# bgmanuel99/Super-Resolution-Images-for-3D-Printing-Defect-Detection

Hardware: AMD Instinct MI355X
Metric: 4x-SR MPix/s on 512x512 LR batch (higher is better)
Workload: dtype bf16

## Files before the change

### include/sr355.h

```cpp
#ifndef SR355_H
#define SR355_H
#include <stdint.h>

#ifdef __cplusplus
extern "C" {
#endif

typedef struct sr_ctx sr_ctx;
typedef struct sr_model sr_model;

typedef enum sr_status {
    SR_OK = 0,
    SR_ERR_INVALID = -1,
    SR_ERR_HIP = -2,
    SR_ERR_OOM = -3,
    SR_ERR_STATE = -4,
    SR_ERR_NAME = -5,
    SR_ERR_CAPACITY = -6
} sr_status;

enum { SR_DTYPE_F32 = 0, SR_DTYPE_BF16 = 1, SR_DTYPE_U8 = 2 };
enum { SR_MODEL_SRCNN = 0, SR_MODEL_EDSR = 1, SR_MODEL_ESRGAN_G = 2, SR_MODEL_VGG16 = 3,
       SR_MODEL_ESRGAN_D = 4,
       SR_MODEL_VGG19_FEATURES = 5 };
enum { SR_ACT_LINEAR = 0, SR_ACT_RELU = 1, SR_ACT_LRELU = 2, SR_ACT_TANH = 3 };
enum { SR_WEIGHT_KERNEL = 0, SR_WEIGHT_BIAS = 1 };
enum { SR_ELT_AXPBY = 0, SR_ELT_RELU_BWD = 1, SR_ELT_LRELU_BWD = 2, SR_ELT_CLIP01_BWD = 3, SR_ELT_MUL = 4, SR_ELT_TANH_BWD = 5, SR_ELT_CLIP01 = 6,
       SR_ELT_SIGN_DIFF = 7 };

typedef struct sr_model_cfg {
    int32_t compute_dtype;
    int32_t scale_factor;
    int32_t channels;
    int32_t num_blocks;
    int32_t num_filters;
    int32_t growth_channels;
    float   res_scaling;
    int32_t num_classes;
    int32_t use_attention;
} sr_model_cfg;

int  sr_init(int device_id, sr_ctx** out);
void sr_destroy(sr_ctx* ctx);
const char* sr_last_error(sr_ctx* ctx);
int  sr_mem_info(sr_ctx* ctx, int64_t* current_bytes, int64_t* peak_bytes);
int  sr_last_forward_ms(sr_ctx* ctx, float* ms);

int  sr_measure_clock(sr_ctx* ctx, float* mhz, void* stream);

int  sr_debug_set_stamp_buffer(sr_ctx* ctx, void* device_u64_buffer, int64_t capacity_bytes);
int  sr_debug_set_chain_stamp_buffer(sr_ctx* ctx, void* device_u64_buffer, int64_t capacity_bytes);
int64_t sr_debug_stamp_bytes_needed(int which, int64_t workgroups);
int  sr_debug_set_fused(sr_ctx* ctx, int mask, int max_workgroups);
enum { SR_FUSE_DENSE_TAIL = 1, SR_FUSE_DENSE_MID = 2, SR_FUSE_RGB_TAIL = 4, SR_FUSE_ATTN_PROJ = 8, SR_FUSE_CELLS = 16, SR_FUSE_CONV1_STREAM = 32,
       SR_FUSE_POOL = 64, SR_FUSE_CONV_STREAM = 128, SR_FUSE_SRCNN_1X1 = 256, SR_FUSE_ALL = 511,
       SR_FUSE_TWO_UP = SR_FUSE_DENSE_TAIL | SR_FUSE_DENSE_MID | SR_FUSE_CONV1_STREAM };
int  sr_debug_set_alloc_cap(sr_ctx* ctx, int64_t bytes);
int  sr_debug_conv_routes(sr_ctx* ctx, int enable, char* text, int64_t cap);
int  sr_profile_begin(sr_ctx* ctx);
int  sr_profile_end(sr_ctx* ctx, char* json, int64_t cap);

int  sr_model_create(sr_ctx* ctx, int kind, const sr_model_cfg* cfg, sr_model** out);
void sr_model_destroy(sr_model* m);
int  sr_model_num_params(sr_model* m);
int  sr_model_param_info(sr_model* m, int index, const char** name, int* which, int64_t shape[4], int* ndim);
int  sr_model_set_weight(sr_model* m, const char* keras_layer_name, int which,
                         const float* host, const int64_t* shape, int ndim);
int  sr_model_finalize(sr_model* m);
int  sr_model_release_workspace(sr_model* m);
int  sr_model_num_ops(sr_model* m);
int  sr_model_op_info(sr_model* m, int index, const char** name, int* channels, int* mul, int* shift, int* ceil_halvings);
int  sr_model_set_tap(sr_model* m, int op_index, float* device_dst, int64_t capacity);
int  sr_model_output_shape(sr_model* m, int B, int H, int W, int C, int64_t out_shape[4]);
int  sr_forward(sr_model* m, const void* x, int io_dtype, int B, int H, int W, int C,
                void* y, int64_t y_capacity, void* stream);

int  sr_conv2d(sr_ctx* ctx, const void* x, int dtype, int B, int H, int W, int Cin,
               const float* w_hwio, const float* bias, int KH, int KW, int Cout, int act,
               float alpha, const void* skip1, float beta1, const void* skip2, float beta2,
               int clip01, int d2s_r, void* y, void* stream);
int  sr_self_attention(sr_ctx* ctx, const void* x, int dtype, int B, int H, int W, int C,
                       const float* wf, const float* bf, const float* wg, const float* bg,
                       const float* wh, const float* bh, const float* wv, const float* bv,
                       void* y, void* stream);
int  sr_bicubic(sr_ctx* ctx, const void* x, int dtype, int B, int H, int W, int C,
                int outH, int outW, void* y, void* stream);
int  sr_resize(sr_ctx* ctx, const void* x, int dtype, int B, int H, int W, int C,
               int outH, int outW, int interpolation, void* y, void* stream);
int  sr_psnr(sr_ctx* ctx, const void* a, const void* b, int B, int H, int W, int C, float max_val,
             float* out_B, void* stream);
int  sr_ssim(sr_ctx* ctx, const void* a, const void* b, int B, int H, int W, int C, float max_val,
             float* out_B, void* stream);
int  sr_mse(sr_ctx* ctx, const void* a, const void* b, int64_t n, float* out1, void* stream);
int  sr_l1(sr_ctx* ctx, const void* a, const void* b, int64_t n, float* out1, void* stream);
int  sr_spectral_l1(sr_ctx* ctx, const void* a, const void* b, int B, int H, int W, int C, float* out1, void* stream);
int  sr_conv2d_wgrad(sr_ctx* ctx, const void* x, const void* dy, int B, int H, int W, int Cin, int Cout, int K,
                     float* dw_hwio, float* db, void* stream);
int  sr_conv2d_dev(sr_ctx* ctx, const void* x, int B, int H, int W, int Cin, const float* d_w, const float* d_bias, int K, int Cout,
                   int rot, int act, float alpha, const void* skip1, float beta1, const void* skip2, float beta2, int clip01,
                   int d2s_r, void* y, void* stream);
typedef struct { const void* p; int64_t cs; int32_t coff; } sr_view;
int  sr_conv2d_dev_views(sr_ctx* ctx, const sr_view* x, int B, int H, int W, int Cin, const float* d_w, const float* d_bias, int K, int Cout, int rot,
                         int act, float alpha, const sr_view* skip1, float beta1, const sr_view* y, void* stream);
int  sr_conv2d_wgrad_views(sr_ctx* ctx, const sr_view* x, const sr_view* dy, int B, int H, int W, int Cin, int Cout, int K,
                           float* dw_hwio, float* db, void* stream);
int  sr_eltwise_views(sr_ctx* ctx, int op, const sr_view* a, const sr_view* b, float alpha, float beta, const sr_view* out, int64_t npix, int C, void* stream);
typedef struct { const float* w; const float* bias; int32_t K, Cin, Cout, rot; } sr_pack_desc;
int  sr_conv_prepack(sr_ctx* ctx, const sr_pack_desc* uses, int n, void* stream);
int  sr_eltwise(sr_ctx* ctx, int op, const void* a, const void* b, float alpha, float beta, void* out, int64_t n, void* stream);
int  sr_adam(sr_ctx* ctx, void* w, const void* g, void* m, void* v, int64_t n, float lr_t, float beta1, float one_minus_beta1, float beta2,
             float one_minus_beta2, float epsilon, float grad_scale, void* stream);
int  sr_space_to_depth(sr_ctx* ctx, const void* x, int B, int H, int W, int C, int r, void* y, void* stream);
enum { SR_SP_MAXPOOL2 = 0, SR_SP_GAP = 1, SR_SP_PICK2 = 2, SR_SP_VGG_PREPROCESS = 3 };
int  sr_spatial_op(sr_ctx* ctx, int op, const void* x, int B, int H, int W, int C, void* y, void* stream);
int  sr_matmul(sr_ctx* ctx, const void* A, const void* B, void* C, int batch, int M, int N, int K, int transA, int transB, float alpha, void* stream);
int  sr_softmax_rows(sr_ctx* ctx, void* s, int64_t rows, int cols, void* stream);
int  sr_softmax_bwd(sr_ctx* ctx, const void* p, const void* dp, void* ds, int64_t rows, int cols, void* stream);
int  sr_maxpool2_bwd(sr_ctx* ctx, const void* x, const void* dy, int B, int H, int W, int C, void* dx, void* stream);
int  sr_zero_insert2(sr_ctx* ctx, const void* dy, int B, int H, int W, int C, void* out, void* stream);
int  sr_spectral_l1_bwd(sr_ctx* ctx, const void* a, const void* b, int B, int H, int W, int C, float scale, void* da, void* stream);
int  sr_extract_patches(sr_ctx* ctx, const float* img, int H, int W, int C, int patch, int stride,
                        float mul, float add, int out_dtype, void* out, int64_t out_capacity,
                        int* n_patches, void* stream);
int  sr_overlap_add(sr_ctx* ctx, const void* patches, int in_dtype, int H, int W, int C, int patch,
                    int stride, int scale, float mul, float add, float* out, void* stream);

int  sr_extract_patches_batch(sr_ctx* ctx, const void* imgs, int in_dtype, int F, int H, int W, int C, int patch, int stride,
                              float mul, float add, int out_dtype, void* out, int64_t out_capacity, int* patches_per_image, void* stream);
int  sr_patch_vote(sr_ctx* ctx, const float* probs, int F, int P, int K, int32_t* cls_F, float* conf_F, int32_t* votes_FxK, void* stream);
int  sr_classification_counts(sr_ctx* ctx, const int32_t* y_true_N, const int32_t* preds_AxN, const float* conf_AxN, int A, int N, int K,
                              int64_t* confusion_AxKxK, double* conf_sums_Ax2, void* stream);

int  sr_back_projection(sr_ctx* ctx, const uint8_t* hr_u8, const uint8_t* lr_u8, int B, int H, int W, int h, int w, int iterations,
                        uint8_t* y_u8, float* y_f32, void* stream);
int  sr_noise_sigma(sr_ctx* ctx, const uint8_t* x_u8, int B, int h, int w, double* sigma_f64, void* stream);
int  sr_nl_means(sr_ctx* ctx, const uint8_t* x_u8, int B, int h, int w, int patch, int distance, const double* sigma_f64,
                 double h_scale, float* y_f32, void* stream);
int  sr_edge_guided(sr_ctx* ctx, const uint8_t* x_u8, int B, int h, int w, int H, int W, float weight, uint8_t* y_u8,
                    float* up_e_f32, void* stream);
// ... 93 lines not shown
```

### super-resolution-images-for-3d-printing-defect-detection_amd/csrc/api.hip

```cpp
#include <math.h>
#include <stdio.h>
#include <stdlib.h>
#include <string.h>

#include <memory>

#include "common.h"

void* sr_ctx::dalloc(size_t bytes) {
    void* p = nullptr;
    if (bytes == 0) bytes = 16;
    if (alloc_cap > 0 && cur_bytes + (int64_t)bytes > alloc_cap) {
        err = "allocation of " + std::to_string(bytes) + " bytes exceeds the debug cap (sr_debug_set_alloc_cap)";
        return nullptr;
    }
    hipError_t e = hipMalloc(&p, bytes);
    if (e != hipSuccess) {
        err = std::string("hipMalloc(") + std::to_string(bytes) + "): " + hipGetErrorString(e);
        return nullptr;
    }
    allocs[p] = bytes;
    cur_bytes += (int64_t)bytes;
    if (cur_bytes > peak_bytes) peak_bytes = cur_bytes;
    return p;
// ... 469 lines not shown
            const std::string why = m->ctx->err;
            (void)hipDeviceSynchronize();
            m->free_bufs();
            return m->ctx->fail(SR_ERR_OOM, "workspace for [" + std::to_string(B) + "," + std::to_string(H) + "," + std::to_string(W) + "]: " + why +
                                                " (all workspaces of this model were released)");
        }
        SR_HIP(m->ctx, hipMemsetAsync(m->bufp[i], 0, bytes, st));
        m->bufcap[i] = bytes;
    }
    return SR_OK;
}

enum Route { RT_CHAIN = OP_PREPROC + 1, RT_CHAIN_SECOND, RT_CONV1_STREAM, RT_RGB_TAIL, RT_PW2, RT_IN_EPILOGUE };

bool tapped(const sr_model* m, size_t oi) { return !m->taps.empty() && m->taps.count((int)oi) != 0; }
bool bare_epilogue(const Op& op) { return op.skip1.buf < 0 && op.skip2.buf < 0 && op.d2s == 1 && !op.clip; }

bool chain_fits(const sr_model* m, size_t oi, int w, bool pack2) {
    const Op& op = m->ops[oi];
    if (op.chain < 0 || op.chain_pos != 0) return false;
    const ChainSpec& ch = m->chains[op.chain];
    return !(ch.tail && tapped(m, oi)) && (m->ctx->chain_mask & (ch.tail ? SR_FUSE_DENSE_TAIL : SR_FUSE_DENSE_MID)) && chain_supported(ch.w, m->view(op.in), pack2 ? 48 : w);
}
bool conv1_stream_fits(const sr_model* m, const Op& op, int w, bool pack2) {
    return (m->ctx->chain_mask & SR_FUSE_CONV1_STREAM) && op.chain < 0 && op.act == SR_ACT_RELU && op.alpha == 1.f && bare_epilogue(op) && op.out.buf == op.in.buf &&
           op.in.coff == 0 && op.out.coff == 64 && conv1_stream_supported(m->convs[op.conv].w, m->view(op.in), pack2 ? 48 : w);
}
bool rgb_tail_fits(const sr_model* m, const Op& op, size_t oi, int B, int h, int w) {
    const ConvWeights& cw = m->convs[op.conv].w;
    return op.rgbtail >= 0 && (m->ctx->chain_mask & SR_FUSE_RGB_TAIL) && !tapped(m, oi) && cw.rows && cw.NT == 4 && cw.Cout == 64 && bare_epilogue(op) &&
           op.act != SR_ACT_TANH && op.out.buf >= 0 && (int64_t)m->bufcap[op.out.buf] >= rgbtail_partial_bytes(B, h, w);
}
bool pw2_fits(const sr_model* m, const Op& op, size_t oi) {
    const ConvWeights& cw = m->convs[op.conv].w;
    return op.pw2 >= 0 && (m->ctx->chain_mask & SR_FUSE_SRCNN_1X1) && !tapped(m, oi) && cw.thin && !cw.few && cw.dtype == SR_DTYPE_F32 && bare_epilogue(op);
}
bool pool_fits(const sr_model* m, const Op& op, size_t oi, int h, int w) {
    if (oi + 1 >= m->ops.size() || op.out.buf < 0) return false;
    const Op& pl = m->ops[oi + 1];
    const ConvWeights& cw = m->convs[op.conv].w;
    return (m->ctx->chain_mask & SR_FUSE_POOL) && m->T == SR_DTYPE_BF16 && pl.kind == OP_POOL && pl.in.buf == op.out.buf && pl.out.buf >= 0 && cw.rows && cw.NT == 4 &&
           cw.CoutP == cw.Cout && bare_epilogue(op) && op.act != SR_ACT_TANH && !tapped(m, oi) && !m->grid_now[op.in.buf].gx && !m->grid_now[op.out.buf].gx &&
           h >= 2 && w >= 2 && m->bufs[pl.out.buf].Cbuf % 8 == 0 && m->bufs[pl.out.buf].Cbuf >= cw.Cout;
}
bool proj_fits(const sr_model* m, const Op& op) {
    const ConvWeights& cw = m->convs[op.conv].w;
    return op.proj >= 0 && (m->ctx->chain_mask & SR_FUSE_ATTN_PROJ) && cw.rows && cw.NT == 4 && cw.Cout / (op.d2s * op.d2s) == 64 && cw.CoutP == cw.Cout &&
           op.out.buf >= 0 && !m->bufs[op.out.buf].blk && op.skip2.buf < 0 && !op.clip && op.act != SR_ACT_TANH && m->bufs[op.out.buf].Cbuf % 4 == 0;
}

void plan_routes(sr_model* m, const Layout& L, int B, int H, int W) {
    std::vector<int>& rt = m->routes;
    rt.resize(m->ops.size());
    for (size_t oi = 0; oi < m->ops.size(); ++oi) rt[oi] = m->ops[oi].kind;
    for (size_t oi = 0; oi < m->ops.size(); ++oi) {
        const Op& op = m->ops[oi];
        if (rt[oi] != OP_CONV) continue;
        int h, w;
        buf_hw(m->bufs[op.in.buf], H, W, &h, &w);
        if (chain_fits(m, oi, w, L.pack2)) { rt[oi] = RT_CHAIN; rt[oi + 1] = RT_CHAIN_SECOND; }
        else if (conv1_stream_fits(m, op, w, L.pack2)) rt[oi] = RT_CONV1_STREAM;
        else if (rgb_tail_fits(m, op, oi, B, h, w)) { rt[oi] = RT_RGB_TAIL; rt[oi + 1] = RT_IN_EPILOGUE; }
        else if (pw2_fits(m, op, oi)) { rt[oi] = RT_PW2; rt[oi + 1] = RT_IN_EPILOGUE; }
        else if (pool_fits(m, op, oi, h, w) || proj_fits(m, op)) rt[oi + 1] = RT_IN_EPILOGUE;
    }
}

}

extern "C" {

int sr_init(int device_id, sr_ctx** out) {
    if (!out) return SR_ERR_INVALID;
    *out = nullptr;
    int n = 0;
    if (hipGetDeviceCount(&n) != hipSuccess || device_id < 0 || device_id >= n) return SR_ERR_HIP;
    if (hipSetDevice(device_id) != hipSuccess) return SR_ERR_HIP;
    sr_ctx* c = new sr_ctx();
    c->device = device_id;
    if (hipEventCreate(&c->ev0) != hipSuccess || hipEventCreate(&c->ev1) != hipSuccess) { delete c; return SR_ERR_HIP; }
    c->zero_page = c->dalloc(sr_ctx::ZERO_PAGE_BYTES);
    if (!c->zero_page) { sr_destroy(c); return SR_ERR_OOM; }
    if (hipMemset(c->zero_page, 0, sr_ctx::ZERO_PAGE_BYTES) != hipSuccess) { sr_destroy(c); return SR_ERR_HIP; }
    *out = c;
    return SR_OK;
}

void sr_destroy(sr_ctx* ctx) {
    DeviceGuard dg_(ctx);
    if (!ctx) return;
    (void)hipDeviceSynchronize();
    lpips_release(ctx);
    std::vector<void*> ps;
    for (auto& kv : ctx->allocs) ps.push_back(kv.first);
    for (void* p : ps) ctx->dfree(p);
    if (ctx->ev0) (void)hipEventDestroy(ctx->ev0);
    if (ctx->ev1) (void)hipEventDestroy(ctx->ev1);
    for (auto& r : ctx->prof_recs) { (void)hipEventDestroy(r.e0); (void)hipEventDestroy(r.e1); }
    for (auto& e : ctx->ev_pool) (void)hipEventDestroy(e);
    delete ctx;
}

const char* sr_last_error(sr_ctx* ctx) { return ctx ? ctx->err.c_str() : "null ctx"; }

int sr_mem_info(sr_ctx* ctx, int64_t* current_bytes, int64_t* peak_bytes) {
    if (!ctx) return SR_ERR_INVALID;
    if (current_bytes) *current_bytes = ctx->cur_bytes;
    if (peak_bytes) *peak_bytes = ctx->peak_bytes;
    return SR_OK;
}

int sr_last_forward_ms(sr_ctx* ctx, float* ms) {
    DeviceGuard dg_(ctx);
    if (!ctx || !ms) return SR_ERR_INVALID;
    if (!ctx->timed) return ctx->fail(SR_ERR_STATE, "no forward has run on this ctx");
    SR_HIP(ctx, hipEventSynchronize(ctx->ev1));
    SR_HIP(ctx, hipEventElapsedTime(ms, ctx->ev0, ctx->ev1));
    return SR_OK;
}

int64_t sr_debug_stamp_bytes_needed(int which, int64_t workgroups) {
    if (which == 0) return workgroups < 0 ? -1 : workgroups * 16 * (int64_t)sizeof(unsigned long long);
    if (which == 1) return (int64_t)64 * 4 * 64 * 4 * (int64_t)sizeof(unsigned long long);
    return -1;
}

int sr_debug_set_stamp_buffer(sr_ctx* ctx, void* device_u64_buffer, int64_t capacity_bytes) {
    if (!ctx) return SR_ERR_INVALID;
    if (device_u64_buffer && capacity_bytes < sr_debug_stamp_bytes_needed(0, 1))
        return ctx->fail(SR_ERR_INVALID, "sr_debug_set_stamp_buffer: the buffer does not hold one workgroup's stamps");
    ctx->stamp_buf = static_cast<unsigned long long*>(device_u64_buffer);
    ctx->stamp_cap = device_u64_buffer ? capacity_bytes : 0;
    return SR_OK;
}

int sr_measure_clock(sr_ctx* ctx, float* mhz, void* stream) {
    if (!ctx || !mhz) return SR_ERR_INVALID;
    DeviceGuard dg_(ctx);
    return clock_probe_launch(ctx, mhz, static_cast<hipStream_t>(stream));
}

int sr_debug_set_chain_stamp_buffer(sr_ctx* ctx, void* device_u64_buffer, int64_t capacity_bytes) {
    if (!ctx) return SR_ERR_INVALID;
    if (device_u64_buffer && capacity_bytes < sr_debug_stamp_bytes_needed(1, 0))
        return ctx->fail(SR_ERR_INVALID, "sr_debug_set_chain_stamp_buffer: the buffer is smaller than the stamped kernels write (sr_debug_stamp_bytes_needed(1, 0))");
    ctx->chain_stamp_buf = static_cast<unsigned long long*>(device_u64_buffer);
    const char* skip = getenv("SR355_CHAIN_STAMP_SKIP");
    ctx->chain_stamp_skip = skip ? atoi(skip) : -1;
    return SR_OK;
}

int sr_debug_set_fused(sr_ctx* ctx, int mask, int max_workgroups) {
    if (!ctx) return SR_ERR_INVALID;
    ctx->chain_mask = mask;
    ctx->chain_max_wgs = max_workgroups > 0 ? max_workgroups : 0;
    return SR_OK;
}

int sr_debug_set_alloc_cap(sr_ctx* ctx, int64_t bytes) {
    if (!ctx) return SR_ERR_INVALID;
    ctx->alloc_cap = bytes > 0 ? bytes : 0;
    return SR_OK;
}

int sr_debug_conv_routes(sr_ctx* ctx, int enable, char* text, int64_t cap) {
    if (!ctx) return SR_ERR_INVALID;
    if (text && cap <= (int64_t)ctx->route_text.size()) return ctx->fail(SR_ERR_CAPACITY, "sr_debug_conv_routes: the text buffer is too small");
    if (text) memcpy(text, ctx->route_text.c_str(), ctx->route_text.size() + 1);
    ctx->route_text.clear();
    ctx->route_log = enable != 0;
    return SR_OK;
}

int sr_profile_begin(sr_ctx* ctx) {
    if (!ctx) return SR_ERR_INVALID;
    for (auto& r : ctx->prof_recs) { ctx->ev_pool.push_back(r.e0); ctx->ev_pool.push_back(r.e1); }
    ctx->prof_recs.clear();
    ctx->prof = true;
    return SR_OK;
}

int sr_profile_end(sr_ctx* ctx, char* json, int64_t cap) {
    DeviceGuard dg_(ctx);
    if (!ctx || !json || cap <= 0) return SR_ERR_INVALID;
    ctx->prof = false;
    SR_HIP(ctx, hipDeviceSynchronize());
    struct Agg { int64_t n = 0; double ms = 0, flops = 0, bytes = 0; };
    std::vector<Agg> agg(ctx->prof_names.size());
    for (auto& r : ctx->prof_recs) {
        float ms = 0.f;
        if (hipEventElapsedTime(&ms, r.e0, r.e1) != hipSuccess) continue;
        Agg& a = agg[r.name];
        a.n += 1; a.ms += ms; a.flops += r.flops; a.bytes += r.bytes;
    }
    std::string s = "[";
    bool first = true;
    for (size_t i = 0; i < agg.size(); ++i) {
        if (!agg[i].n) continue;
        char buf[512];
        snprintf(buf, sizeof buf, "%s{\"kernel\": \"%s\", \"launches\": %lld, \"total_ms\": %.6f, \"flops\": %.6e, \"bytes\": %.6e}",
                 first ? "" : ", ", ctx->prof_names[i].c_str(), (long long)agg[i].n, agg[i].ms, agg[i].flops, agg[i].bytes);
        s += buf;
        first = false;
    }
    s += "]";
    for (auto& r : ctx->prof_recs) { ctx->ev_pool.push_back(r.e0); ctx->ev_pool.push_back(r.e1); }
    ctx->prof_recs.clear();
    if ((int64_t)s.size() + 1 > cap) return ctx->fail(SR_ERR_CAPACITY, "profile buffer too small");
    memcpy(json, s.c_str(), s.size() + 1);
    return SR_OK;
}

int sr_model_create(sr_ctx* ctx, int kind, const sr_model_cfg* cfg, sr_model** out) {
    if (!ctx || !cfg || !out) return SR_ERR_INVALID;
    *out = nullptr;
    if (cfg->compute_dtype != SR_DTYPE_F32 && cfg->compute_dtype != SR_DTYPE_BF16)
        return ctx->fail(SR_ERR_INVALID, "compute_dtype must be SR_DTYPE_F32 or SR_DTYPE_BF16");
    std::unique_ptr<sr_model> m(new sr_model());
    m->ctx = ctx; m->kind = kind; m->cfg = *cfg; m->T = cfg->compute_dtype;
    if (m->cfg.channels <= 0) m->cfg.channels = 3;
    if (m->cfg.channels > 16 / dtype_size(m->T))
        return ctx->fail(SR_ERR_INVALID, "channels must fit one 16-byte slice (<= 4 for f32, <= 8 for bf16)");
    int rc;
    switch (kind) {
        case SR_MODEL_SRCNN: rc = build_srcnn(m.get()); break;
        case SR_MODEL_EDSR: rc = build_edsr(m.get()); break;
        case SR_MODEL_ESRGAN_G: rc = build_esrgan(m.get()); break;
        case SR_MODEL_VGG16: rc = build_vgg16(m.get()); break;
        case SR_MODEL_ESRGAN_D: rc = build_discriminator(m.get()); break;
        case SR_MODEL_VGG19_FEATURES: rc = build_vgg19_features(m.get()); break;
        default: return ctx->fail(SR_ERR_INVALID, "unknown model kind");
    }
    if (rc) return rc;
    m->dense_dev.assign(m->params.size(), nullptr);
    *out = m.release();
    return SR_OK;
}

// ... 115 lines not shown
        std::vector<float> k, bias;
        gather(c, k, bias);
        int rc = conv_pack_weights(ctx, k.data(), bias.data(), c.KS, c.Cin, c.Cout, m->T, &c.w, c.rows_head);
        if (rc) return rc;
    }
    for (auto& ch : m->chains) {
        chain_free_weights(ctx, &ch.w);
        const ConvSpec& a = m->convs[ch.conv_a], &bq = m->convs[ch.conv_b];
        std::vector<float> ka, ba, kb, bb;
        gather(a, ka, ba);
        gather(bq, kb, bb);
        int rc = chain_pack_weights(ctx, ka.data(), ba.data(), kb.data(), bb.data(), a.Cin / 32, a.Cout / 16, bq.Cout / 16, &ch.w);
        if (rc) return rc;
    }
    for (auto& rt : m->rgbtails) {
        rgbtail_free_weights(ctx, &rt.w);
        const ConvSpec& c2 = m->convs[rt.conv_b];
        std::vector<float> k, bias;
        gather(c2, k, bias);
        int rc = rgbtail_pack_weights(ctx, k.data(), bias.data(), c2.Cout, &rt.w);
        if (rc) return rc;
    }
    for (auto& pj : m->projs) {
        proj_free_weights(ctx, &pj.w);
        const ConvSpec& c1 = m->convs[pj.conv];
        std::vector<float> k, bias;
        gather(c1, k, bias);
        int rc = proj_pack_weights(ctx, k.data(), bias.data(), c1.Cout, &pj.w);
        if (rc) return rc;
    }
    for (auto& pw : m->pw2s) {
        pw2_free_weights(ctx, &pw.w);
        const ConvSpec& c1 = m->convs[pw.conv];
        std::vector<float> k, bias;
        gather(c1, k, bias);
        int rc = pw2_pack_weights(ctx, k.data(), bias.data(), c1.Cin, c1.Cout, pw.act, &pw.w);
        if (rc) return rc;
    }
    for (auto& op : m->ops) {
        if (op.kind != OP_DENSE) continue;
        for (int pi : {op.dw, op.db}) {
            if (m->dense_dev[pi]) ctx->dfree(m->dense_dev[pi]);
            const Param& p = m->params[pi];
            m->dense_dev[pi] = static_cast<float*>(ctx->dalloc(sizeof(float) * p.count()));
            if (!m->dense_dev[pi]) return SR_ERR_OOM;
            SR_HIP(ctx, hipMemcpy(m->dense_dev[pi], p.host.data(), sizeof(float) * p.count(), hipMemcpyHostToDevice));
        }
    }
    m->finalized = true;
    return SR_OK;
}

int sr_model_output_shape(sr_model* m, int B, int H, int W, int C, int64_t out_shape[4]) {
    if (!m || !out_shape) return SR_ERR_INVALID;
    (void)C;
    if (m->out_vec) { out_shape[0] = B; out_shape[1] = m->out_C; out_shape[2] = 1; out_shape[3] = 1; }
    else { out_shape[0] = B; out_shape[1] = ((int64_t)H * m->out_mul) >> m->out_shift; out_shape[2] = ((int64_t)W * m->out_mul) >> m->out_shift; out_shape[3] = m->out_C; }
    return SR_OK;
}

int sr_forward(sr_model* m, const void* x, int io_dtype, int B, int H, int W, int C, void* y, int64_t y_capacity, void* stream) {
    DeviceGuard dg_(m ? m->ctx : nullptr);
    if (!m) return SR_ERR_INVALID;
    sr_ctx* ctx = m->ctx;
    hipStream_t st = static_cast<hipStream_t>(stream);
    if (!m->finalized) return ctx->fail(SR_ERR_STATE, "sr_model_finalize has not been called");
    if (!x || !y) return ctx->fail(SR_ERR_INVALID, "null tensor");
    if (io_dtype != SR_DTYPE_F32 && io_dtype != SR_DTYPE_BF16) return ctx->fail(SR_ERR_INVALID, "io dtype must be f32 or bf16");
    if (io_dtype == SR_DTYPE_BF16 && m->T == SR_DTYPE_F32) return ctx->fail(SR_ERR_INVALID, "an fp32 model takes fp32 tensors");
    if (C != m->in_C) return ctx->fail(SR_ERR_INVALID, "channel count does not match the model");
    if (B == 0) return SR_OK;
    if (B < 0 || H <= 0 || W <= 0) return ctx->fail(SR_ERR_INVALID, "bad tensor shape");
    int64_t os[4];
    sr_model_output_shape(m, B, H, W, C, os);
    if (y_capacity < os[0] * os[1] * os[2] * os[3]) return ctx->fail(SR_ERR_CAPACITY, "output buffer too small");
    if (m->kind == SR_MODEL_VGG16 && (H < 32 || W < 32)) return ctx->fail(SR_ERR_INVALID, "VGG16 needs H,W >= 32");
    if (m->kind == SR_MODEL_VGG19_FEATURES && (H < 16 || W < 16)) return ctx->fail(SR_ERR_INVALID, "VGG19 features need H,W >= 16");
    const Layout L = choose_layout(m, B, H, W);
    int rc = ensure_workspace(m, L, H, W, st);
    if (rc) return rc;
    plan_routes(m, L, B, H, W);
    SR_HIP(ctx, hipEventRecord(ctx->ev0, st));
    const int T = m->T;
    for (size_t oi = 0; oi < m->ops.size(); ++oi) {
        const Op& op = m->ops[oi];
        const int route = m->routes[oi];
        const Op* nx = oi + 1 < m->ops.size() && m->routes[oi + 1] == RT_IN_EPILOGUE ? &m->ops[oi + 1] : nullptr;
        int h = H, w = W;
        if (op.in.buf >= 0) buf_hw(m->bufs[op.in.buf], H, W, &h, &w);
        const TensorView vi = m->view(op.in), vo = m->view(op.out);
        void* const po = op.out.buf >= 0 ? m->bufp[op.out.buf] : nullptr;
        switch (route) {
            case RT_CHAIN_SECOND: case RT_IN_EPILOGUE:
                break;
            case RT_CHAIN: {
                const ChainSpec& ch = m->chains[op.chain];
                const Op& ob = m->ops[oi + 1];
                TensorView outv{}, so{};
                float bx = 0.f, bo = 0.f;
                if (ch.tail) {
                    outv = m->view(ob.out);
                    for (int k2 = 0; k2 < 2; ++k2) {
                        const Ref& r = k2 ? ob.skip2 : ob.skip1;
                        const float be = k2 ? ob.beta2 : ob.beta1;
                        if (r.buf < 0) continue;
                        if (r.buf == op.in.buf && r.coff == 0) bx = be; else { so = m->view(r); bo = be; }
                    }
                }
                rc = chain_launch(ctx, ch.w, vi, L.pack2 ? (B + 1) / 2 : B, h, L.pack2 ? 48 : w, outv, so, ob.alpha, bx, bo, st, L.pack2);
                break;
            }
            case RT_CONV1_STREAM:
                rc = conv1_stream_launch(ctx, m->convs[op.conv].w, vi, L.pack2 ? (B + 1) / 2 : B, h, L.pack2 ? 48 : w, st, L.pack2);
                break;
            case RT_RGB_TAIL: case RT_PW2: case OP_CONV: {
                const ConvSpec& cs = m->convs[op.conv];
                int in = op.in.buf;
                TensorView xin = vi;
                if (op.pack_alt >= 0 && (L.pack2 || m->grid_now[in].gx)) {
                    void* d = m->bufp[op.pack_alt];
                    const int64_t dC = m->bufs[op.pack_alt].Cbuf;
                    const CellGrid& g = m->grid_now[in];
                    rc = g.gx ? cell_unpack_launch(ctx, vi.p, vi.cs, vi.coff, B, h, w, 64, d, dC, 0, g, st) : unpack_pairs_launch(ctx, vi.p, vi.cs, vi.coff, B, h, w, 64, d, dC, 0, st);
                    if (rc) return rc;
                    in = op.pack_alt;
                    m->grid_now[in] = CellGrid{};
                    xin = m->view({in, 0});
                } else if (L.pack2 && vi.blk) {
                    return ctx->fail(SR_ERR_STATE, "two-up packed dense blocks: a conv outside the fused kernels would read a packed buffer");
                }
                const CellGrid g = m->grid_now[in];
                bool same = g.gx == 0 || op.d2s == 1;
                for (const Ref& r : {op.out, op.skip1, op.skip2})
                    if (r.buf != -1 && !((r.buf >= 0 ? m->grid_now[r.buf] : CellGrid{}) == g)) same = false;
                if (!same) return ctx->fail(SR_ERR_STATE, "packed small-image layout: producer and consumer disagree");
                const int cB = g.gx ? 1 : B;
                if (g.gx) { h = g.Hv; w = g.Wv; }
                ConvEpilogue ep;
                ep.act = op.act; ep.alpha = op.alpha; ep.clip01 = op.clip; ep.d2s_r = op.d2s; ep.cell_h = g.ch; ep.cell_w = g.cw;
                if (op.skip1.buf >= 0) { ep.skip1 = m->view(op.skip1); ep.beta1 = op.beta1; }
                if (op.skip2.buf >= 0) { ep.skip2 = m->view(op.skip2); ep.beta2 = op.beta2; }
                if (route == RT_RGB_TAIL) {
                    const RgbTailWeights& rt = m->rgbtails[op.rgbtail].w;
                    ep.f2 = &rt; ep.f2_part = static_cast<float*>(po);
                    rc = conv_launch(ctx, cs.w, xin, cB, h, w, TensorView{}, ep, st);
                    if (!rc) rc = rgbtail_finish_launch(ctx, rt, ep.f2_part, cB, h, w, nx->act, nx->alpha, nx->clip, y, m->out_C, 0, io_dtype == SR_DTYPE_F32, st);
                    break;
                }
                if (route == RT_PW2) ep.pw2 = &m->pw2s[op.pw2].w;
                else if (nx && nx->kind == OP_POOL) { ep.pool_out = m->view(nx->out); ep.pool_grid = m->grid_now[nx->out.buf]; }
                else if (nx) { ep.pj = &m->projs[op.proj].w; ep.pj_out = m->view(nx->out); }
                if (op.out.buf == -2) {
                    ep.out_f32 = io_dtype == SR_DTYPE_F32;
                    rc = conv_launch(ctx, cs.w, xin, B, h, w, y, m->out_C, 0, ep, st);
                } else {
                    rc = conv_launch(ctx, cs.w, xin, cB, h, w, route == RT_PW2 ? m->view(nx->out) : vo, ep, st);
                }
                break;
            }
            case OP_CONVERT:
                rc = convert_pad_launch(ctx, x, io_dtype, (int64_t)B * H * W, C, po, T, vo.cs, 1.f, 0.f, st);
                break;
            case OP_PREPROC:
                rc = vgg_preproc_launch(ctx, x, io_dtype, (int64_t)B * H * W, po, T, vo.cs, st);
                break;
            case OP_ATTN:
                rc = attention_launch(ctx, T, vi.p, vi.cs,  8,  0,  16, B, h * w, po, vo.cs, 0, st);
                break;
            case OP_SUBSAMPLE:
                rc = subsample2_launch(ctx, T, vi.p, B, h, w, m->bufs[op.in.buf].C, vi.cs, po, vo.cs, st);
                break;
            case OP_TOBLK: {
                const CellGrid& g = m->grid_now[op.out.buf];
                rc = g.gx ? cell_pack_launch(ctx, vi.p, vi.cs, vi.coff, B, h, w, 64, po, vo.cs, vo.coff, g, st)
                   : L.pack2 ? pack_pairs_launch(ctx, vi.p, vi.cs, vi.coff, B, h, w, 64, po, vo.cs, vo.coff, st)
                             : nhwc_to_blocked_launch(ctx, vi.p, vi.cs, vi.coff, B, h, w, 64, po, vo.cs, vo.coff, st);
                break;
            }
            case OP_POOL:
                rc = maxpool2_launch(ctx, T, vi.p, B, h, w, m->bufs[op.in.buf].C, vi.cs, po, vo.cs, st, m->grid_now[op.in.buf], m->grid_now[op.out.buf]);
                break;
            case OP_GAP:
                rc = gap_launch(ctx, T, vi.p, B, h * w, m->bufs[op.in.buf].C, vi.cs, static_cast<float*>(po), st);
                break;
            case OP_DENSE: {
                const bool f32 = op.out.buf != -2 || io_dtype == SR_DTYPE_F32;
                float* yf = static_cast<float*>(op.out.buf == -2 ? y : po);
                rc = dense_launch(ctx, static_cast<const float*>(vi.p), m->dense_dev[op.dw], m->dense_dev[op.db], B, op.In, op.Out, op.act, f32 ? yf : nullptr,
                                  f32 ? 0 : io_dtype, f32 ? nullptr : y, st);
                break;
            }
        }
        if (rc) return rc;
        if (tapped(m, oi)) {
            int C_, mu, sh, th, tw;
            op_out_view(m, op, &C_, &mu, &sh);
            buf_hw(m->bufs[op.out.buf], H, W, &th, &tw);
            const sr_model::Tap& tp = m->taps.at((int)oi);
            if (tp.cap < (int64_t)B * th * tw * C_) return ctx->fail(SR_ERR_CAPACITY, "tap buffer too small");
            rc = tap_copy_launch(ctx, vo.p, T, vo.blk, vo.cs, vo.coff, B, th, tw, C_, tp.dst, st, L.pack2 && vo.blk);
            if (rc) return rc;
        }
    }
    SR_HIP(ctx, hipEventRecord(ctx->ev1, st));
    ctx->timed = true;
    return SR_OK;
}

static ConvEpilogue single_op_epilogue(int act, float alpha, int clip01, int d2s_r, TensorView skip1, float beta1, TensorView skip2, float beta2) {
    ConvEpilogue ep;
    ep.act = act; ep.alpha = alpha; ep.clip01 = clip01; ep.d2s_r = d2s_r < 1 ? 1 : d2s_r;
    ep.allow_splitk = 1;
    if (skip1.p) { ep.skip1 = skip1; ep.beta1 = beta1; }
    if (skip2.p) { ep.skip2 = skip2; ep.beta2 = beta2; }
    return ep;
}

static int padded_cin(const ConvWeights& cw) { return cw.thin ? cw.CinP : round_up(cw.CinP, 32); }

int sr_conv2d(sr_ctx* ctx, const void* x, int dtype, int B, int H, int W, int Cin, const float* w_hwio, const float* bias, int KH, int KW,
              int Cout, int act, float alpha, const void* skip1, float beta1, const void* skip2, float beta2, int clip01, int d2s_r,
              void* y, void* stream) {
    DeviceGuard dg_(ctx);
    if (!ctx) return SR_ERR_INVALID;
    hipStream_t st = static_cast<hipStream_t>(stream);
    if (!x || !w_hwio || !y) return ctx->fail(SR_ERR_INVALID, "null tensor");
    if (KH != KW) return ctx->fail(SR_ERR_INVALID, "square kernels only");
    if (dtype != SR_DTYPE_F32 && dtype != SR_DTYPE_BF16) return ctx->fail(SR_ERR_INVALID, "dtype must be f32 or bf16");
    if (B <= 0 || H <= 0 || W <= 0 || Cin <= 0 || Cout <= 0) return ctx->fail(SR_ERR_INVALID, "bad tensor shape");
    ConvWeights cw;
    int rc = conv_pack_weights(ctx, w_hwio, bias, KH, Cin, Cout, dtype, &cw);
    if (rc) return rc;
    const int esz = dtype_size(dtype);
    const int Cp = padded_cin(cw);
    void* xp = ctx->dalloc((size_t)B * H * W * Cp * esz + 4096);
    if (!xp) { conv_free_weights(ctx, &cw); return SR_ERR_OOM; }
    rc = convert_pad_launch(ctx, x, dtype, (int64_t)B * H * W, Cin, xp, dtype, Cp, 1.f, 0.f, st);
    if (!rc) {
        auto skip_view = [&](const void* s) { return (s == x && Cout == Cin) ? TensorView{xp, Cp, 0} : TensorView{s, Cout, 0}; };
        const ConvEpilogue ep = single_op_epilogue(act, alpha, clip01, d2s_r, skip_view(skip1), beta1, skip_view(skip2), beta2);
        const int r = ep.d2s_r;
        rc = conv_launch(ctx, cw, TensorView{xp, Cp, 0}, B, H, W, y, Cout / (r * r), 0, ep, st);
    }
    hipError_t e = hipStreamSynchronize(st);
    ctx->dfree(xp);
    conv_free_weights(ctx, &cw);
    if (!rc && e != hipSuccess) return ctx->fail(SR_ERR_HIP, std::string("conv2d: ") + hipGetErrorString(e));
    return rc;
}

// ... 278 lines not shown
```

### super-resolution-images-for-3d-printing-defect-detection_amd/csrc/attention.hip

```cpp
#include "common.h"

#include <cstdlib>

namespace {

constexpr int KV_TILE = 64;

template <typename T> struct AT;
template <> struct AT<float>  { static constexpr int PITCH = KV_TILE * 4 + 4; };

struct AttnParams {
    const char* qkv; int64_t cs; int qoff, koff, voff;
    char* o; int64_t o_cs; int o_coff;
    int N;
    const float* knorm;
};

__device__ __forceinline__ float xhalf(float v) { return __shfl_xor(v, 32); }

__global__ void __launch_bounds__(256, 2) attn_f32_kernel(AttnParams p) {
    constexpr int PITCH = AT<float>::PITCH;
    __shared__ __attribute__((aligned(16))) char vt[32 * PITCH];

    const int tid = threadIdx.x, lane = tid & 63, wave = tid >> 6, r = lane & 31, h = lane >> 5;
    const int b = blockIdx.y;
    const int N = p.N;
    const float* base = reinterpret_cast<const float*>(p.qkv) + (int64_t)b * N * p.cs;
    const int q = blockIdx.x * 128 + wave * 32 + r;
    const int qc = q < N ? q : N - 1;

    float qf[4];
    {
        const float* qp = base + (int64_t)qc * p.cs + p.qoff;
#pragma unroll
        for (int j = 0; j < 4; ++j) qf[j] = qp[2 * j + h];
    }

    f32x16 oacc;
#pragma unroll
    for (int e = 0; e < 16; ++e) oacc[e] = 0.f;
    float m_run = -INFINITY, l_run = 0.f;

    const int skey = tid >> 2, soct = tid & 3;

    for (int k0 = 0; k0 < N; k0 += KV_TILE) {
        __syncthreads();
        {
            const int key = k0 + skey;
            const float* vp = base + (int64_t)(key < N ? key : N - 1) * p.cs + p.voff + soct * 8;
            f32x4 v0 = *reinterpret_cast<const f32x4*>(vp), v1 = *reinterpret_cast<const f32x4*>(vp + 4);
#pragma unroll
            for (int e = 0; e < 4; ++e) {
                *reinterpret_cast<float*>(vt + (soct * 8 + e) * PITCH + skey * 4) = v0[e];
                *reinterpret_cast<float*>(vt + (soct * 8 + 4 + e) * PITCH + skey * 4) = v1[e];
            }
        }
        __syncthreads();
#pragma unroll
        for (int sub = 0; sub < KV_TILE / 32; ++sub) {
            const int kb = k0 + sub * 32;
            if (kb >= N) break;
            f32x16 s;
#pragma unroll
            for (int e = 0; e < 16; ++e) s[e] = 0.f;
            {
                const int key = kb + r;
                const float* kp = base + (int64_t)(key < N ? key : N - 1) * p.cs + p.koff;
#pragma unroll
                for (int j = 0; j < 4; ++j) s = __builtin_amdgcn_mfma_f32_32x32x2f32(kp[2 * j + h], qf[j], s, 0, 0, 0);
            }
            float mx = -INFINITY;
#pragma unroll
            for (int i = 0; i < 16; ++i) {
                const int key = kb + (i & 3) + 8 * (i >> 2) + 4 * h;
                if (key >= N) s[i] = -INFINITY;
                mx = fmaxf(mx, s[i]);
            }
            mx = fmaxf(mx, xhalf(mx));
            const float m_new = fmaxf(m_run, mx);
            const float alpha = __expf(m_run - m_new);
            float psum = 0.f;
#pragma unroll
            for (int i = 0; i < 16; ++i) { s[i] = __expf(s[i] - m_new); psum += s[i]; }
            l_run = l_run * alpha + psum;
            m_run = m_new;
#pragma unroll
            for (int e = 0; e < 16; ++e) oacc[e] *= alpha;
#pragma unroll
            for (int i = 0; i < 16; ++i) {
                const int krow = sub * 32 + (i & 3) + 8 * (i >> 2);
                const float va = *reinterpret_cast<const float*>(vt + r * PITCH + (krow + 4 * h) * 4);
                oacc = __builtin_amdgcn_mfma_f32_32x32x2f32(va, s[i], oacc, 0, 0, 0);
            }
        }
    }
    const float l_tot = l_run + xhalf(l_run);
    const float inv = 1.f / l_tot;
    if (q < N) {
        float* op = reinterpret_cast<float*>(p.o) + ((int64_t)b * N + q) * p.o_cs + p.o_coff;
#pragma unroll
        for (int g = 0; g < 4; ++g) {
            const int d0 = 8 * g + 4 * h;
            f32x4 t = {oacc[4 * g] * inv, oacc[4 * g + 1] * inv, oacc[4 * g + 2] * inv, oacc[4 * g + 3] * inv};
            *reinterpret_cast<f32x4*>(op + d0) = t;
        }
    }
}

constexpr int KT2 = 128;
constexpr int PITCH2 = KT2 * 2 + 8;

__global__ void __launch_bounds__(64) attn_knorm_kernel(const bf16_t* qkv, int64_t cs, int koff, int N, int ngroups, float* out) {
    const int g = blockIdx.x % ngroups, b = blockIdx.x / ngroups, lane = threadIdx.x;
    const bf16_t* base = qkv + (int64_t)b * N * cs + koff;
    float m = 0.f;
#pragma unroll
    for (int t = 0; t < 2; ++t) {
        const int key = g * 128 + t * 64 + lane;
        if (key < N) {
            const bf16x8 k = *reinterpret_cast<const bf16x8*>(base + (int64_t)key * cs);
            float n2 = 0.f;
#pragma unroll
            for (int e = 0; e < 8; ++e) n2 += (float)k[e] * (float)k[e];
            m = fmaxf(m, n2);
        }
    }
#pragma unroll
    for (int o = 32; o > 0; o >>= 1) m = fmaxf(m, __shfl_xor(m, o));
    if (lane == 0) out[(int64_t)b * ngroups + g] = sqrtf(m);
}

template <int QB>
__global__ void __launch_bounds__(256, 3) attn_bf16_kernel(AttnParams p) {
    __shared__ __attribute__((aligned(16))) char vt[32 * PITCH2];
    const int tid = threadIdx.x, lane = tid & 63, wave = tid >> 6, r = lane & 31, h = lane >> 5;
    const int N = p.N;
    constexpr int QW = 64 * QB * 2;
    const int nqt = (N + QW - 1) / QW;
    const int b = blockIdx.x / nqt, qt = blockIdx.x - b * nqt;
    const bf16_t* base = reinterpret_cast<const bf16_t*>(p.qkv) + (int64_t)b * N * p.cs;
    const int cs = (int)p.cs;
    int qi[QB];
    bf16x8 qb[QB];
#pragma unroll
    for (int j = 0; j < QB; ++j) {
        qi[j] = qt * QW + wave * (32 * QB) + j * 32 + r;
        const int qc = qi[j] < N ? qi[j] : N - 1;
        bf16x8 z = {};
        qb[j] = z;
        if (h == 0) qb[j] = *reinterpret_cast<const bf16x8*>(base + (int64_t)qc * cs + p.qoff);
    }
    float qn2 = 0.f;
#pragma unroll
    for (int j = 0; j < QB; ++j) {
        float n2 = 0.f;
#pragma unroll
        for (int e = 0; e < 8; ++e) n2 += (float)qb[j][e] * (float)qb[j][e];
        qn2 = fmaxf(qn2, n2);
    }
#pragma unroll
    for (int o = 32; o > 0; o >>= 1) qn2 = fmaxf(qn2, __shfl_xor(qn2, o));
    const float qmaxv = sqrtf(qn2) * 1.0009765625f;
    const int* knorm_bits = reinterpret_cast<const int*>(p.knorm) + (int64_t)b * ((N + KT2 - 1) / KT2);
    f32x16 oacc[QB];
    bf16x8 sel = {};
    {
        const int m = lane & 15, kg = lane >> 4;
        const bf16_t one = (bf16_t)1.f;
        if ((m == 0 && (kg & 1) == 0) || (m == 1 && (kg & 1) == 1)) sel = bf16x8{one, one, one, one, one, one, one, one};
    }
    f32x4 lacc[QB];
    float m_run[QB];
#pragma unroll
    for (int j = 0; j < QB; ++j) {
        m_run[j] = 0.f; lacc[j] = f32x4{0.f, 0.f, 0.f, 0.f};
#pragma unroll
        for (int e = 0; e < 16; ++e) oacc[j][e] = 0.f;
    }

    const int kp = tid >> 2, oct = tid & 3;
    bf16x8 kneg = {};
    kneg[0] = (bf16_t)-1.f; kneg[1] = (bf16_t)-1.f; kneg[2] = (bf16_t)-1.f;
    auto load_k = [&](int kb) {
        int l;
        asm volatile("v_mbcnt_lo_u32_b32 %0, -1, 0\n\tv_mbcnt_hi_u32_b32 %0, -1, %0" : "=v"(l));
        bf16x8 kf = kneg;
        const int key = kb + (l & 31);
        if (l < 32) kf = *reinterpret_cast<const bf16x8*>(base + (int64_t)(key < N ? key : N - 1) * cs + p.koff);
        return kf;
    };
    bf16x8 knext = load_k(0);
    f32x16 zero16;
#pragma unroll
    for (int e = 0; e < 16; ++e) zero16[e] = 0.f;
    struct { } false_c; struct { int x; } true_c{0};
    auto hmax = [](float v) {
        const unsigned u = __builtin_bit_cast(unsigned, v);
        const auto sw = __builtin_amdgcn_permlane32_swap(u, u, false, false);
        return fmaxf(__builtin_bit_cast(float, (unsigned)sw[0]), __builtin_bit_cast(float, (unsigned)sw[1]));
    };
    auto tile = [&](const bf16x8 kf, const int sub, const int kb, auto ragged_tag, const bool first) {
        constexpr bool RAGGED = sizeof(ragged_tag) > 1;
        f32x16 s[QB];
        float mx[QB];
#pragma unroll
        for (int j = 0; j < QB; ++j) {
            s[j] = __builtin_amdgcn_mfma_f32_32x32x16_bf16(kf, qb[j], zero16, 0, 0, 0);
            if constexpr (RAGGED) {
#pragma unroll
                for (int i = 0; i < 16; ++i)
                    if (kb + (i & 3) + 8 * (i >> 2) + 4 * h >= N) s[j][i] = -INFINITY;
            }
// ... 85 lines not shown
                lacc[j] = __builtin_amdgcn_mfma_f32_16x16x32_bf16(sel, pf, lacc[j], 0, 0, 0);
            }
        }
        return true;
    };
    auto thresh_of_wave = [&]() -> int {
        float m = m_run[0];
#pragma unroll
        for (int j = 1; j < QB; ++j) m = fminf(m, m_run[j]);
#pragma unroll
        for (int o = 32; o > 0; o >>= 1) m = fminf(m, __shfl_xor(m, o));
        const float lim = GROW_OK + m;
        const float th = !(lim >= 0.f) ? -1.f : (qmaxv > 0.f ? lim / qmaxv * 0.9990234375f : INFINITY);
        return __builtin_amdgcn_readfirstlane(__builtin_bit_cast(int, th));
    };
    int thresh_bits = __builtin_amdgcn_readfirstlane(__builtin_bit_cast(int, -1.f));
    auto stage_v = [&](const int k0) {
        __syncthreads();
#pragma unroll
        for (int part = 0; part < KT2 / 128; ++part) {
            const int ka = k0 + part * 128 + 2 * kp, kbb = ka + 1;
            if (ka - 2 * kp >= N) break;
            const bf16x8 va = *reinterpret_cast<const bf16x8*>(base + (int64_t)(ka < N ? ka : N - 1) * cs + p.voff + oct * 8);
            const bf16x8 vb = *reinterpret_cast<const bf16x8*>(base + (int64_t)(kbb < N ? kbb : N - 1) * cs + p.voff + oct * 8);
#pragma unroll
            for (int e = 0; e < 8; ++e) {
                typedef bf16_t bf16x2 __attribute__((ext_vector_type(2)));
                bf16x2 pr = {va[e], vb[e]};
                *reinterpret_cast<bf16x2*>(vt + (oct * 8 + e) * PITCH2 + (part * 64 + kp) * 4) = pr;
            }
        }
        __syncthreads();
    };
    auto slow_tiles = [&](const int k0, const int sub0, bf16x8 kf) {
        for (int sub = sub0; sub < KT2 / 32; ++sub) {
            const int kb = k0 + sub * 32;
            if (kb >= N) break;
            if (sub != sub0) { kf = knext; knext = load_k(kb + 32); }
            if (kb + 32 <= N) tile(kf, sub, kb, false_c, kb == 0);
            else tile(kf, sub, kb, true_c, kb == 0);
        }
    };

    for (int k0 = 0; k0 < N; k0 += KT2) {
        stage_v(k0);
        int sub = 0;
        bf16x8 kf = knext;
        const bool full = k0 != 0 && k0 + KT2 <= N;
        if (full) {
            const bool guard = !(knorm_bits[k0 / KT2] <= thresh_bits);
#pragma unroll
            for (; sub < KT2 / 32; ++sub) {
                kf = knext;
                knext = load_k(k0 + sub * 32 + 32);
                if (!tile_fast(kf, sub, guard)) break;
            }
        } else {
            knext = load_k(k0 + 32);
        }
        if (sub < KT2 / 32) {
            slow_tiles(k0, sub, kf);
            thresh_bits = thresh_of_wave();
        }
    }
#pragma unroll
    for (int j = 0; j < QB; ++j) {
        const float l0 = __shfl(lacc[j][0], r & 15), l1 = __shfl(lacc[j][1], r & 15);
        const float inv = 1.f / ((r >> 4) ? l1 : l0);
        if (qi[j] < N) {
            bf16_t* op = reinterpret_cast<bf16_t*>(p.o) + ((int64_t)b * N + qi[j]) * p.o_cs + p.o_coff;
#pragma unroll
            for (int g = 0; g < 4; ++g) {
                bf16x4 t = {(bf16_t)(oacc[j][4 * g] * inv), (bf16_t)(oacc[j][4 * g + 1] * inv), (bf16_t)(oacc[j][4 * g + 2] * inv),
                            (bf16_t)(oacc[j][4 * g + 3] * inv)};
                *reinterpret_cast<bf16x4*>(op + 8 * g + 4 * h) = t;
            }
        }
    }
}

}

int attention_launch(sr_ctx* ctx, int dtype, const void* qkv, int64_t cs, int qoff, int koff, int voff, int B, int N,
                     void* o, int64_t o_cs, int o_coff, hipStream_t st) {
    if (B <= 0 || N <= 0) return ctx->fail(SR_ERR_INVALID, "attention: empty tensor");
    const int esz = dtype_size(dtype);
    if ((cs * esz) % 16 || (qoff * esz) % 16 || (koff * esz) % 16 || (voff * esz) % 16 || (o_cs * esz) % 16 || (o_coff * esz) % 16)
        return ctx->fail(SR_ERR_INVALID, "attention: views must be 16-byte aligned");
    AttnParams p{static_cast<const char*>(qkv), cs, qoff, koff, voff, static_cast<char*>(o), o_cs, o_coff, N, nullptr};
    dim3 grid((unsigned)((N + 127) / 128), (unsigned)B);
    if (dtype != SR_DTYPE_BF16 && dtype != SR_DTYPE_F32) return ctx->fail(SR_ERR_INVALID, "attention: dtype must be f32 or bf16");
    const int rec = ctx->prof_open(dtype == SR_DTYPE_BF16 ? "attn<bf16>" : "attn<f32>", 2.0 * B * (double)N * N * 40.0,
                                   (double)B * N * 80.0 * esz, st);
    if (dtype == SR_DTYPE_BF16) {
        constexpr int QBr = 2;
        const int64_t nwg = (int64_t)B * ((N + 128 * QBr - 1) / (128 * QBr));
        const int ngroups = (N + KT2 - 1) / KT2;
        if (nwg >= (1ll << 31) || (int64_t)B * ngroups >= (1ll << 31)) { ctx->prof_close(rec, st); return ctx->fail(SR_ERR_INVALID, "attention: too many workgroups for one launch"); }
        float* kn = static_cast<float*>(ctx->arena(ctx->attn_kn, sizeof(float) * (size_t)B * ngroups, st));
        if (!kn) { ctx->prof_close(rec, st); return SR_ERR_OOM; }
        p.knorm = kn;
        hipLaunchKernelGGL(attn_knorm_kernel, dim3((unsigned)((int64_t)B * ngroups)), dim3(64), 0, st, reinterpret_cast<const bf16_t*>(qkv) + 0, cs, koff, N, ngroups, kn);
        hipLaunchKernelGGL(attn_bf16_kernel<QBr>, dim3((unsigned)nwg), dim3(256), 0, st, p);
    }
    else hipLaunchKernelGGL(attn_f32_kernel, grid, dim3(256), 0, st, p);
    ctx->prof_close(rec, st);
    SR_HIP(ctx, hipGetLastError());
    return SR_OK;
}
```

### super-resolution-images-for-3d-printing-defect-detection_amd/csrc/common.h

```cpp
#pragma once
#include <hip/hip_runtime.h>
#include <stdint.h>
#include <string.h>
#include <string>
#include <unordered_map>
#include <unordered_set>
#include <vector>

#include "../../include/sr355.h"

typedef __bf16 bf16_t;
typedef __bf16 bf16x8 __attribute__((ext_vector_type(8)));
typedef __bf16 bf16x4 __attribute__((ext_vector_type(4)));
typedef float f32x4 __attribute__((ext_vector_type(4)));
typedef float f32x16 __attribute__((ext_vector_type(16)));

struct sr_ctx {
    int device = 0;
    std::string err;
    int64_t cur_bytes = 0, peak_bytes = 0;
    std::unordered_map<void*, size_t> allocs;
    hipEvent_t ev0 = nullptr, ev1 = nullptr;
    bool timed = false;

    void* scratch_buf = nullptr;
    size_t scratch_cap = 0;
    unsigned long long* stamp_buf = nullptr;
    int64_t stamp_cap = 0;
    int chain_stamp_skip = -1;
    unsigned long long* chain_stamp_buf = nullptr;

    struct ProfRec { int name; hipEvent_t e0, e1; double flops, bytes; };
    bool prof = false;
    std::vector<std::string> prof_names;
    std::vector<ProfRec> prof_recs;
    std::vector<hipEvent_t> ev_pool;
    int prof_open(const std::string& name, double flops, double bytes, hipStream_t st);
    void prof_close(int rec, hipStream_t st);

    static constexpr int MAX_LDS_BYTES = 160 * 1024;
    std::unordered_map<const void*, int> lds_attr_done;
    int ensure_dyn_lds(const void* kernel, int bytes);
    void* tab_buf = nullptr; size_t tab_cap = 0;
    struct Arena { void* p = nullptr; size_t cap = 0; };
    Arena attn_kn;
    Arena dev_w, dev_b, dev_x;
    Arena cls_tab, cls_work, cls_fft;
    std::unordered_map<int64_t, double*> dft_ops;
    Arena met_work, met_fft;
    Arena eda_work, eda_dct;
    Arena deg_work;
    Arena crop_work;
    Arena sn_work, sn_tab, dhead_work;
    std::vector<char> sn_tab_host;
    void* sn_tab_dev = nullptr;
    struct LpipsState* lpips = nullptr;
    Arena lpips_work;
    int* deg_status = nullptr;
    void* arena(Arena& a, size_t bytes, hipStream_t st);
    struct PackKey {
        const void* w; const void* b; int K, Cin, Cout, rot;
        bool operator==(const PackKey& o) const { return w == o.w && b == o.b && K == o.K && Cin == o.Cin && Cout == o.Cout && rot == o.rot; }
    };
    struct PackKeyHash {
        size_t operator()(const PackKey& k) const {
            return std::hash<const void*>()(k.w) ^ (std::hash<const void*>()(k.b) * 31u) ^ ((size_t)k.rot << 1) ^ ((size_t)k.Cin << 20) ^ ((size_t)k.Cout << 36) ^ ((size_t)k.K << 52);
        }
    };
    std::unordered_map<PackKey, std::pair<void*, float*>, PackKeyHash> pack_cache;
    Arena pack_w, pack_b, pack_tab;
    std::vector<char> pack_tab_host;
    void* pack_tab_dev = nullptr;
    static constexpr int ZERO_PAGE_BYTES = 32768;
    void* zero_page = nullptr;
    int num_cus = 0;
    int cu_count();
    int chain_mask = 511;
    int chain_max_wgs = 0;
    int64_t alloc_cap = 0;
    bool route_log = false;
    std::string route_text;

    void* dalloc(size_t bytes);
    void dfree(void* p);
    void* scratch(size_t bytes);
    int fail(int code, const std::string& msg) { err = msg; return code; }
};
static_assert(511 == SR_FUSE_ALL && SR_FUSE_ALL == (SR_FUSE_DENSE_TAIL | SR_FUSE_DENSE_MID | SR_FUSE_RGB_TAIL | SR_FUSE_ATTN_PROJ | SR_FUSE_CELLS | SR_FUSE_CONV1_STREAM |
                                             SR_FUSE_POOL | SR_FUSE_CONV_STREAM | SR_FUSE_SRCNN_1X1), "sr_ctx::chain_mask's default is every SR_FUSE_* bit");

struct DeviceGuard {
    int prev = -1; bool switched = false;
    explicit DeviceGuard(const sr_ctx* c) {
        if (c && hipGetDevice(&prev) == hipSuccess && prev != c->device) switched = hipSetDevice(c->device) == hipSuccess;
    }
    ~DeviceGuard() { if (switched) (void)hipSetDevice(prev); }
    DeviceGuard(const DeviceGuard&) = delete;
    DeviceGuard& operator=(const DeviceGuard&) = delete;
};

#define SR_HIP(ctx, call)                                                                        \
    do {                                                                                         \
        hipError_t e_ = (call);                                                                  \
        if (e_ != hipSuccess)                                                                    \
            return (ctx)->fail(SR_ERR_HIP, std::string(#call) + ": " + hipGetErrorString(e_));   \
    } while (0)

void lpips_release(sr_ctx* ctx);

__device__ inline int gray_bgr(int b, int g, int r) { return (1868 * b + 9617 * g + 4899 * r + 8192) >> 14; }

static inline int dtype_size(int dt) { return dt == SR_DTYPE_F32 ? 4 : (dt == SR_DTYPE_BF16 ? 2 : 1); }
static inline int round_up(int a, int b) { return (a + b - 1) / b * b; }
static inline uint16_t f32_to_bf16_host(float f) {
    uint32_t u;
    memcpy(&u, &f, 4);
    if ((u & 0x7fffffffu) > 0x7f800000u) return (uint16_t)((u >> 16) | 0x40);
    u += 0x7fffu + ((u >> 16) & 1u);
    return (uint16_t)(u >> 16);
}

int weights_upload(sr_ctx* ctx, const void* packed, size_t bytes, const float* bias, int n, int npad, void** d_w, float** d_bias);
template <typename P> static inline void weights_free(sr_ctx* ctx, P*& w, float*& bias) {
    if (w) ctx->dfree(w);
    if (bias) ctx->dfree(bias);
    w = nullptr; bias = nullptr;
}

struct ConvWeights {
    void* w = nullptr;
    float* bias = nullptr;
    int dtype = SR_DTYPE_BF16;
    int KS = 3, Cin = 0, Cout = 0;
    int CinP = 0, CoutP = 0;
    int thin = 0;
    int KGPT = 2;
    int NT = 1;
    int rows = 0;
    int few = 0;
    int pw = 0;
    int nchunks = 1;
    size_t bytes = 0;
};

struct TensorView {
    const void* p = nullptr;
    int64_t cs = 0;
    int coff = 0;
    int blk = 0;
};

struct RgbTailWeights {
    void* a = nullptr;
    float* bias = nullptr;
    int c2 = 0;
};

struct ProjWeights {
    void* a = nullptr;
    float* bias = nullptr;
    int nblk = 0;
};

struct Pw2Weights {
    float* a = nullptr;
    float* bias = nullptr;
    int cin = 0, cout = 0, act = 0;
};

struct CellGrid {
    int gx = 0, ch = 0, cw = 0, Hv = 0, Wv = 0;
    bool operator==(const CellGrid& o) const { return gx == o.gx && ch == o.ch && cw == o.cw && Hv == o.Hv && Wv == o.Wv; }
};

struct ConvEpilogue {
    TensorView pool_out;
    CellGrid pool_grid;
    int cell_h = 0, cell_w = 0;
    const ProjWeights* pj = nullptr;
    TensorView pj_out;
    const Pw2Weights* pw2 = nullptr;
    const RgbTailWeights* f2 = nullptr;
    float* f2_part = nullptr;
    int act = SR_ACT_LINEAR;
    float alpha = 1.f;
    TensorView skip1, skip2;
    float beta1 = 0.f, beta2 = 0.f;
    int clip01 = 0;
    int d2s_r = 1;
    int out_f32 = 0;
    int allow_splitk = 0;
};

int conv_pack_weights_dev(sr_ctx* ctx, const float* d_hwio, const float* d_bias, int KS, int Cin, int Cout, int rot, ConvWeights* out, hipStream_t st);
int conv_prepack_dev(sr_ctx* ctx, const sr_pack_desc* descs, int n, hipStream_t st);
int conv_pack_weights(sr_ctx* ctx, const float* hwio, const float* bias, int KS, int Cin, int Cout,
                      int dtype, ConvWeights* out, int rows_head = 0);
static inline void conv_free_weights(sr_ctx* ctx, ConvWeights* w) { weights_free(ctx, w->w, w->bias); }
int conv_launch(sr_ctx* ctx, const ConvWeights& w, TensorView x, int B, int H, int W,
                void* y, int64_t y_cs, int y_coff, const ConvEpilogue& ep, hipStream_t st);
int conv_launch(sr_ctx* ctx, const ConvWeights& w, TensorView x, int B, int H, int W, TensorView y, const ConvEpilogue& ep, hipStream_t st);

int proj_pack_weights(sr_ctx* ctx, const float* w_hwio, const float* bias, int cout, ProjWeights* out);
int pw2_pack_weights(sr_ctx* ctx, const float* w_hwio, const float* bias, int cin, int cout, int act, Pw2Weights* out);
static inline void pw2_free_weights(sr_ctx* ctx, Pw2Weights* w) { weights_free(ctx, w->a, w->bias); *w = Pw2Weights{}; }
static inline void proj_free_weights(sr_ctx* ctx, ProjWeights* w) { weights_free(ctx, w->a, w->bias); }
int rgbtail_pack_weights(sr_ctx* ctx, const float* w2_hwio, const float* bias2, int c2, RgbTailWeights* out);
static inline void rgbtail_free_weights(sr_ctx* ctx, RgbTailWeights* w) { weights_free(ctx, w->a, w->bias); }
int64_t rgbtail_partial_bytes(int B, int H, int W);
int rgbtail_finish_launch(sr_ctx* ctx, const RgbTailWeights& w, const float* part, int B, int H, int W, int act, float alpha, int clip01, void* y,
                          int64_t y_cs, int y_coff, int out_f32, hipStream_t st);

struct ChainWeights {
    void* w = nullptr; float* bias = nullptr;
    int ext = 0, nb0 = 0, nb1 = 0;
    size_t bytes = 0;
};
int chain_pack_weights(sr_ctx* ctx, const float* wa_hwio, const float* ba, const float* wb_hwio, const float* bb, int ext, int nb0, int nb1, ChainWeights* out);
static inline void chain_free_weights(sr_ctx* ctx, ChainWeights* w) { weights_free(ctx, w->w, w->bias); }
bool chain_supported(const ChainWeights& w, const TensorView& in, int W);
bool conv1_stream_supported(const ConvWeights& w, const TensorView& in, int W);
int conv1_stream_launch(sr_ctx* ctx, const ConvWeights& w, TensorView in, int B, int H, int W, hipStream_t st, bool seam = false);
int pack_pairs_launch(sr_ctx* ctx, const void* src, int64_t src_cs, int src_coff, int B, int H, int W, int C, void* dst, int64_t dst_C, int dst_coff, hipStream_t st);
int unpack_pairs_launch(sr_ctx* ctx, const void* src, int64_t src_C, int src_coff, int B, int H, int W, int C, void* dst, int64_t dst_C, int dst_coff, hipStream_t st);
int cell_pack_launch(sr_ctx* ctx, const void* src, int64_t src_cs, int src_coff, int B, int H, int W, int C, void* dst, int64_t dst_C, int dst_coff, const CellGrid& g, hipStream_t st);
int cell_unpack_launch(sr_ctx* ctx, const void* src, int64_t src_C, int src_coff, int B, int H, int W, int C, void* dst, int64_t dst_C, int dst_coff, const CellGrid& g, hipStream_t st);
int chain_launch(sr_ctx* ctx, const ChainWeights& w, TensorView in, int B, int H, int W, TensorView out, TensorView skip_o, float alpha, float beta_x,
                 float beta_o, hipStream_t st, bool seam = false);

int attention_launch(sr_ctx* ctx, int dtype, const void* qkv, int64_t cs, int qoff, int koff, int voff,
                     int B, int N, void* o, int64_t o_cs, int o_coff, hipStream_t st);

int nhwc_to_blocked_launch(sr_ctx* ctx, const void* src, int64_t src_cs, int src_coff, int B, int H, int W, int C, void* dst, int64_t dst_C,
                           int dst_coff, hipStream_t st);
int clock_probe_launch(sr_ctx* ctx, float* mhz_out, hipStream_t st);
int tap_copy_launch(sr_ctx* ctx, const void* src, int dtype, int blk, int64_t cs, int coff, int B, int H, int W, int C, float* dst, hipStream_t st, bool pairs = false);
int convert_pad_launch(sr_ctx* ctx, const void* x, int in_dtype, int64_t npix, int C, void* y, int out_dtype,
                       int Cp, float mul, float add, hipStream_t st);
int maxpool2_launch(sr_ctx* ctx, int dtype, const void* x, int B, int H, int W, int C, int64_t x_cs, void* y,
                    int64_t y_cs, hipStream_t st, CellGrid in_grid = CellGrid{}, CellGrid out_grid = CellGrid{});
int gap_launch(sr_ctx* ctx, int dtype, const void* x, int B, int HW, int C, int64_t x_cs, float* y, hipStream_t st);
int dense_launch(sr_ctx* ctx, const float* x, const float* w, const float* bias, int B, int In, int Out, int act,
                 float* y, int y_dtype, void* y_typed, hipStream_t st);
int bicubic_launch(sr_ctx* ctx, const void* x, int dtype, int B, int H, int W, int C, int outH, int outW,
                   void* y, int out_dtype, int64_t y_cs, hipStream_t st);
int subsample2_launch(sr_ctx* ctx, int dtype, const void* x, int B, int H, int W, int C, int64_t x_cs, void* y, int64_t y_cs, hipStream_t st);
int vgg_preproc_launch(sr_ctx* ctx, const void* x, int in_dtype, int64_t npix, void* y, int out_dtype, int Cp, hipStream_t st);
int l1_launch(sr_ctx* ctx, const float* a, const float* b, int64_t n, float* out, hipStream_t st);
int spectral_l1_launch(sr_ctx* ctx, const float* a, const float* b, int B, int H, int W, int C, float* out, hipStream_t st);
int wgrad_launch(sr_ctx* ctx, const float* x, const float* dy, int B, int H, int W, int Cin, int Cout, int KS, float* dw, float* db, hipStream_t st);
int wgrad_launch_views(sr_ctx* ctx, const float* x, int64_t x_cs, const float* dy, int64_t dy_cs, int B, int H, int W, int Cin, int Cout, int KS, float* dw, float* db,
                       hipStream_t st);
int eltwise_views_launch(sr_ctx* ctx, int op, const float* a, int64_t a_cs, const float* b, int64_t b_cs, float alpha, float beta, float* out, int64_t o_cs, int64_t npix, int C,
                         hipStream_t st);
int adam_launch(sr_ctx* ctx, float* w, const float* g, float* m, float* v, int64_t n, float lr_t, float b1, float omb1, float b2, float omb2, float eps,
                float gscale, hipStream_t st);
int eltwise_launch(sr_ctx* ctx, int op, const float* a, const float* b, float alpha, float beta, float* out, int64_t n, hipStream_t st);
int space_to_depth_launch(sr_ctx* ctx, const float* x, int B, int H, int W, int C, int r, float* y, hipStream_t st);
int matmul_launch(sr_ctx* ctx, const float* A, const float* B, float* C, int batch, int M, int N, int K, int tA, int tB, float alpha, hipStream_t st);
int softmax_rows_launch(sr_ctx* ctx, float* s, int64_t rows, int cols, hipStream_t st);
int softmax_bwd_launch(sr_ctx* ctx, const float* p, const float* dp, float* ds, int64_t rows, int cols, hipStream_t st);
int maxpool2_bwd_launch(sr_ctx* ctx, const float* x, const float* dy, int B, int H, int W, int C, float* dx, hipStream_t st);
int zero_insert2_launch(sr_ctx* ctx, const float* dy, int B, int H, int W, int C, float* out, hipStream_t st);
int spectral_l1_bwd_launch(sr_ctx* ctx, const float* a, const float* b, int B, int H, int W, int C, float scale, float* da, hipStream_t st);
int resize_launch(sr_ctx* ctx, const void* x, int dtype, int B, int H, int W, int C, int outH, int outW, int interp, void* y, hipStream_t st);
int psnr_launch(sr_ctx* ctx, const float* a, const float* b, int B, int64_t n_per_image, float max_val, float* out,
                hipStream_t st);
int ssim_launch(sr_ctx* ctx, const float* a, const float* b, int B, int H, int W, int C, float max_val, float* out,
                hipStream_t st);
int mse_launch(sr_ctx* ctx, const float* a, const float* b, int64_t n, float* out, hipStream_t st);
int extract_patches_launch(sr_ctx* ctx, const float* img, int H, int W, int C, int patch, int stride, float mul,
                           float add, int out_dtype, void* out, int ny, int nx, hipStream_t st);
int overlap_add_launch(sr_ctx* ctx, const void* patches, int in_dtype, int H, int W, int C, int patch, int stride,
                       int scale, float mul, float add, int ny, int nx, float* out, hipStream_t st);

static inline int pad_amount(int n, int patch, int stride) {
    int pad = (n % stride != 0) ? (patch - (n % stride)) % stride : 0;
    int extra = patch - stride;
    return pad > extra ? pad : extra;
}
```

### super-resolution-images-for-3d-printing-defect-detection_amd/csrc/conv.hip

```cpp
#include <type_traits>

#include "conv_common.h"
#include "conv_pack.h"

#include <cstdio>
#include <cstdlib>
#include <cstring>

namespace {

using namespace convk;

template <typename T> struct TT;
template <> struct TT<bf16_t> { static constexpr int E = 8; typedef bf16x8 frag; };
template <> struct TT<float>  { static constexpr int E = 4; typedef f32x4 frag; };

__device__ __forceinline__ f32x16 mma(bf16x8 a, bf16x8 b, f32x16 c) {
    return __builtin_amdgcn_mfma_f32_32x32x16_bf16(a, b, c, 0, 0, 0);
}
__device__ __forceinline__ f32x16 mma(f32x4 a, f32x4 b, f32x16 c) {
#pragma unroll
    for (int j = 0; j < 4; ++j) c = __builtin_amdgcn_mfma_f32_32x32x2f32(a[j], b[j], c, 0, 0, 0);
    return c;
}
// ... 718 lines not shown
    std::vector<PackJob> jobs((size_t)n);
    std::vector<sr_ctx::PackKey> keys((size_t)n);
    size_t wbytes = 0, bbytes = 0;
    int64_t blocks = 0;
    std::vector<size_t> woff((size_t)n), boff((size_t)n);
    for (int i = 0; i < n; ++i) {
        const sr_pack_desc& d = descs[i];
        if (!d.w || d.Cin <= 0 || d.Cout <= 0) return ctx->fail(SR_ERR_INVALID, "conv prepack: null kernel or bad shape");
        ConvWeights w;
        PackJob& jb = jobs[(size_t)i];
        const int rc = conv_plan(ctx, SR_DTYPE_F32, d.K, d.Cin, d.Cout, 0, d.rot ? 1 : 0, &w, &jb.q, &jb.n);
        if (rc) return rc;
        jb.src = d.w; jb.bias = d.bias; jb.blk0 = (int)blocks;
        blocks += (jb.n + PACK_JOB_ELEMS - 1) / PACK_JOB_ELEMS;
        woff[(size_t)i] = wbytes; boff[(size_t)i] = bbytes;
        wbytes += (w.bytes + 255) & ~(size_t)255;
        bbytes += (sizeof(float) * (size_t)round_up(w.CoutP, 64) + 255) & ~(size_t)255;
        keys[(size_t)i] = sr_ctx::PackKey{d.w, d.bias, d.K, d.Cin, d.Cout, d.rot ? 1 : 0};
    }
    if (blocks > 0x7fffffff) return ctx->fail(SR_ERR_INVALID, "conv prepack: too many elements for one launch");
    char* wb = static_cast<char*>(ctx->arena(ctx->pack_w, wbytes, st));
    char* bb = static_cast<char*>(ctx->arena(ctx->pack_b, bbytes, st));
    const size_t tbytes = sizeof(PackJob) * (size_t)n;
    void* tab = ctx->arena(ctx->pack_tab, tbytes, st);
    if (!wb || !bb || !tab) return SR_ERR_OOM;
    for (int i = 0; i < n; ++i) {
        jobs[(size_t)i].dst = reinterpret_cast<float*>(wb + woff[(size_t)i]);
        jobs[(size_t)i].bias_out = reinterpret_cast<float*>(bb + boff[(size_t)i]);
    }
    if (ctx->pack_tab_host.size() != tbytes || ctx->pack_tab_dev != tab || memcmp(ctx->pack_tab_host.data(), jobs.data(), tbytes) != 0) {
        SR_HIP(ctx, hipStreamSynchronize(st));
        SR_HIP(ctx, hipMemcpy(tab, jobs.data(), tbytes, hipMemcpyHostToDevice));
        ctx->pack_tab_host.assign(reinterpret_cast<const char*>(jobs.data()), reinterpret_cast<const char*>(jobs.data()) + tbytes);
        ctx->pack_tab_dev = tab;
    }
    hipLaunchKernelGGL(pack_weights_f32_many_kernel, dim3((unsigned)blocks), dim3(256), 0, st, static_cast<const PackJob*>(tab), n);
    SR_HIP(ctx, hipGetLastError());
    for (int i = 0; i < n; ++i) ctx->pack_cache[keys[(size_t)i]] = {jobs[(size_t)i].dst, jobs[(size_t)i].bias_out};
    return SR_OK;
}

int conv_launch(sr_ctx* ctx, const ConvWeights& w, TensorView x, int B, int H, int W, void* y, int64_t y_cs, int y_coff,
                const ConvEpilogue& ep, hipStream_t st) {
    return conv_launch(ctx, w, x, B, H, W, TensorView{y, y_cs, y_coff}, ep, st);
}

int conv_launch(sr_ctx* ctx, const ConvWeights& w, TensorView x, int B, int H, int W, TensorView yv, const ConvEpilogue& ep, hipStream_t st) {
    void* y = const_cast<void*>(yv.p);
    const int64_t y_cs = yv.cs;
    const int y_coff = yv.coff;
    if (B <= 0 || H <= 0 || W <= 0) return ctx->fail(SR_ERR_INVALID, "conv: empty tensor");
    const int esz = dtype_size(w.dtype);
    if ((x.cs * esz) % 16 != 0 || (x.coff * esz) % 16 != 0 || ((uintptr_t)x.p % 16) != 0)
        return ctx->fail(SR_ERR_INVALID, "conv: input view must be 16-byte aligned per pixel");
    if (x.cs - x.coff < w.CinP) return ctx->fail(SR_ERR_INVALID, "conv: input view exposes fewer channels than the packed Cin");
    if ((int64_t)H * W * x.cs >= (int64_t)1 << 31) return ctx->fail(SR_ERR_INVALID, "conv: image too large for 32-bit offsets");
    const int r = ep.d2s_r < 1 ? 1 : ep.d2s_r;
    if (w.Cout % (r * r) != 0) return ctx->fail(SR_ERR_INVALID, "conv: Cout not divisible by d2s block^2");
    auto strides = [&](const TensorView& v, int width, int64_t* cs, int* ps, int* rs) {
        if (v.blk) { *cs = 32; *ps = width * 32; *rs = (int)(width * v.cs); }
        else { *cs = v.cs; *ps = 32; *rs = (int)(width * v.cs); }
    };
    for (const TensorView* v : {(const TensorView*)&x, (const TensorView*)&yv, &ep.skip1, &ep.skip2})
        if (v->p && v->blk && (v->cs % 32 != 0 || v->coff % (v == &yv ? 4 : 32) != 0))
            return ctx->fail(SR_ERR_INVALID, "conv: a row-blocked view needs 32-channel granularity (4 for the output's first channel)");
    const bool any_blk = x.blk || yv.blk || (ep.skip1.p && ep.skip1.blk) || (ep.skip2.p && ep.skip2.blk);
    if (w.pw && r > 1) return ctx->fail(SR_ERR_INVALID, "conv: 1x1 with depth_to_space is not built");
    if (any_blk && !w.rows) return ctx->fail(SR_ERR_INVALID, "conv: only the bf16 3x3 kernel handles row-blocked views");
    if (yv.blk && r > 1) return ctx->fail(SR_ERR_INVALID, "conv: depth_to_space writes NHWC only");
    ConvParams p;
    p.in = static_cast<const char*>(x.p); p.in_coff = x.coff; strides(x, W, &p.in_cs, &p.in_ps, &p.in_rs);
    p.w = static_cast<const char*>(w.w); p.bias = w.bias;
    p.out = static_cast<char*>(y); p.out_coff = y_coff; strides(yv, W * r, &p.out_cs, &p.out_ps, &p.out_rs);
    p.out_f32 = (ep.out_f32 || w.dtype == SR_DTYPE_F32) ? 1 : 0;
    p.s1 = static_cast<const char*>(ep.skip1.p); p.s1_coff = ep.skip1.coff; p.beta1 = ep.beta1; strides(ep.skip1, W, &p.s1_cs, &p.s1_ps, &p.s1_rs);
    p.s2 = static_cast<const char*>(ep.skip2.p); p.s2_coff = ep.skip2.coff; p.beta2 = ep.beta2; strides(ep.skip2, W, &p.s2_cs, &p.s2_ps, &p.s2_rs);
    if (!p.s1 && p.s2) {
        p.s1 = p.s2; p.s1_cs = p.s2_cs; p.s1_coff = p.s2_coff; p.s1_ps = p.s2_ps; p.s1_rs = p.s2_rs; p.beta1 = p.beta2; p.s2 = nullptr;
    }
    p.alpha = ep.alpha; p.act = ep.act; p.clip = ep.clip01; p.r = r; p.Cd = w.Cout / (r * r);
    p.B = B; p.H = H; p.W = W; p.Cout = w.Cout; p.nchunks = w.nchunks; p.tilesX = p.tilesY = 0;
    p.dbg = ctx->stamp_buf;
    p.f2w = nullptr; p.f2part = nullptr; p.f2c = 0;
    p.pjw = nullptr; p.pjbias = nullptr; p.pjout = nullptr; p.pj_cs = 0; p.pj_coff = 0; p.pj_rs = 0; p.pj_nblk = 0;
    p.cell_h = ep.cell_h; p.cell_w = ep.cell_w;
    p.splitk_ok = ep.allow_splitk;
    p.pw2w = nullptr; p.pw2bias = nullptr; p.pw2_cout = 0; p.pw2_act = 0;
    p.plout = nullptr; p.pl_cs = 0; p.pl_coff = 0; p.pl_gx = p.pl_ch = p.pl_cw = p.pl_Wv = 0;
    const int osz = p.out_f32 ? 4 : esz;
    bool vec = (y_cs % 4 == 0) && (y_coff % 4 == 0) && ((uintptr_t)y % (4 * osz) == 0) && (p.Cd % 4 == 0);
    if (p.s1) vec = vec && (p.s1_cs % 4 == 0) && (p.s1_coff % 4 == 0) && ((uintptr_t)p.s1 % (4 * esz) == 0);
    if (p.s2) vec = vec && (p.s2_cs % 4 == 0) && (p.s2_coff % 4 == 0) && ((uintptr_t)p.s2 % (4 * esz) == 0);
    p.vec = vec ? 1 : 0;
    if (any_blk && !(vec && w.Cout % 4 == 0 && ep.act != SR_ACT_TANH))
        return ctx->fail(SR_ERR_INVALID, "conv: row-blocked views need the vector epilogue (aligned views, Cout % 4 == 0, no tanh)");
    p.skip_lds = 0; p.skip_scale = 0.f;
    if (w.rows && w.NT == 4 && w.Cout % 16 == 0 && w.Cin >= w.Cout && ep.act == SR_ACT_LINEAR && ep.alpha != 0.f && r == 1 && vec) {
        if (p.s2 && p.s2 == p.in && p.s2_cs == p.in_cs && p.s2_ps == p.in_ps && p.s2_coff == p.in_coff) { p.skip_lds = 2; p.skip_scale = p.beta2 / p.alpha; }
        else if (p.s1 && p.s1 == p.in && p.s1_cs == p.in_cs && p.s1_ps == p.in_ps && p.s1_coff == p.in_coff) { p.skip_lds = 1; p.skip_scale = p.beta1 / p.alpha; }
    }
    if ((ep.cell_h || ep.cell_w) && !(w.rows && vec && w.Cout % 4 == 0 && ep.act != SR_ACT_TANH && r == 1 && !ep.pj && !ep.f2 && ep.cell_h >= 2 && ep.cell_w >= 2))
        return ctx->fail(SR_ERR_INVALID, "conv: separator masks need the bf16 3x3 kernel's vector epilogue");
    if (ep.pool_out.p) {
        if (!(w.rows && w.NT == 4 && w.CoutP == w.Cout && r == 1 && !p.s1 && !p.s2 && !ep.clip01 && ep.act != SR_ACT_TANH && !ep.pj && !ep.f2 && !ep.cell_h && !ep.cell_w && !ep.pool_out.blk &&
              ep.pool_out.cs % 8 == 0 && ep.pool_out.coff % 8 == 0 && ((uintptr_t)ep.pool_out.p % 16) == 0 && ep.pool_out.cs - ep.pool_out.coff >= w.Cout && H >= 2 && W >= 2))
            return ctx->fail(SR_ERR_INVALID, "conv: the fused max-pool follows a bf16 3x3 conv in 64-cout tiles without skips");
        p.plout = static_cast<char*>(const_cast<void*>(ep.pool_out.p)); p.pl_cs = ep.pool_out.cs; p.pl_coff = ep.pool_out.coff;
        p.pl_gx = ep.pool_grid.gx; p.pl_ch = ep.pool_grid.ch; p.pl_cw = ep.pool_grid.cw; p.pl_Wv = ep.pool_grid.Wv;
    }
    if (ep.pj) {
        if (!(w.rows && w.NT == 4 && p.Cd == 64 && w.CoutP == w.Cout && !yv.blk && !p.s2 && !ep.clip01 && ep.act != SR_ACT_TANH && vec && !ep.f2 && ep.pj->a &&
              ep.pj->nblk >= 1 && ep.pj->nblk <= 3 && ep.pj_out.p && !ep.pj_out.blk && ep.pj_out.cs - ep.pj_out.coff >= 16 * ep.pj->nblk && ep.pj_out.cs % 4 == 0 &&
              ep.pj_out.coff % 4 == 0 && (int64_t)H * r * W * r * ep.pj_out.cs < ((int64_t)1 << 31)))
            return ctx->fail(SR_ERR_INVALID, "conv: the fused 1x1 projection follows a bf16 3x3 conv whose output pixels have 64 channels (NHWC, at most one skip)");
        p.pjw = static_cast<const char*>(ep.pj->a); p.pjbias = ep.pj->bias; p.pj_nblk = ep.pj->nblk;
        p.skip_lds = 0; p.skip_scale = 0.f;
        p.pjout = static_cast<char*>(const_cast<void*>(ep.pj_out.p)); p.pj_cs = ep.pj_out.cs; p.pj_coff = ep.pj_out.coff; p.pj_rs = (int)(W * r * ep.pj_out.cs);
    }
    if (ep.pw2) {
        if (!(w.dtype == SR_DTYPE_F32 && w.thin && !w.few && w.NT == 1 && w.CoutP == 96 && ep.pw2->a && ep.pw2->cin == w.Cout && ep.pw2->cout >= 1 && ep.pw2->cout <= 32 && r == 1 &&
              !p.s1 && !p.s2 && !ep.clip01 && !ep.pj && !ep.f2 && !ep.pool_out.p && !yv.blk && yv.cs - yv.coff >= ep.pw2->cout))
            return ctx->fail(SR_ERR_INVALID, "conv: the fused 1x1 follows an fp32 thin conv that owns all its couts in one workgroup, without skips");
        p.pw2w = ep.pw2->a; p.pw2bias = ep.pw2->bias; p.pw2_cout = ep.pw2->cout; p.pw2_act = ep.pw2->act;
        p.Cd = ep.pw2->cout;
    }
    if (ep.f2) {
        if (!(w.rows && w.NT == 4 && w.Cout == 64 && w.CoutP == 64 && r == 1 && !p.s1 && !p.s2 && !ep.clip01 && ep.act != SR_ACT_TANH && ep.f2->a && ep.f2_part))
            return ctx->fail(SR_ERR_INVALID, "conv: the fused RGB tail follows a bf16 3x3 conv to 64 channels without skips");
        p.f2w = static_cast<const char*>(ep.f2->a); p.f2part = ep.f2_part; p.f2c = ep.f2->c2;
    }
    const int nct = w.CoutP / 32 / w.NT;
    const ConvRoute rt = conv_route(ctx, w, p, nct);
    const bool stream = rt.fam == CF_STREAM;
    if (ctx->route_log) ctx->route_text += conv_route_name(rt) + "\n";
    int rec = -1;
    if (ctx->prof && ep.f2) {
        const double px = (double)B * H * W;
        rec = ctx->prof_open("conv_rows_rgbtail<bf16,64->64->rgb>", 2.0 * px * 9 * w.Cin * (w.Cout + ep.f2->c2),
                             px * w.Cin * esz + (double)rgbtail_partial_bytes(B, H, W), st);
    } else if (ctx->prof && ep.pool_out.p) {
        const double px = (double)B * H * W;
        rec = ctx->prof_open("conv_rows_pool<bf16,k3,nt4+maxpool2>", 2.0 * px * 9.0 * w.Cin * w.Cout, px * ((double)w.Cin * esz + 0.25 * w.Cout * esz), st);
    } else if (ctx->prof && ep.pj) {
        const double px = (double)B * H * W;
        rec = ctx->prof_open("conv_rows_proj<bf16,k3,nt4+1x1>", 2.0 * px * (9.0 * w.Cin * w.Cout + (double)w.Cout * 16 * ep.pj->nblk),
                             px * ((double)w.Cin * esz + (double)w.Cout * osz + (p.s1 ? (double)w.Cout * esz : 0.0) + (double)r * r * 16 * ep.pj->nblk * esz), st);
    } else if (ctx->prof && ep.pw2) {
        const double px = (double)B * H * W;
        rec = ctx->prof_open("conv_thin_pw2<f32,k9,3->96->32>", 2.0 * px * ((double)w.KS * w.KS * w.Cin * w.Cout + (double)w.Cout * ep.pw2->cout),
                             px * ((double)w.CinP * esz + (double)ep.pw2->cout * osz), st);
    } else if (ctx->prof) {
        char nm[96];
        snprintf(nm, sizeof nm, "conv_%s<%s,k%d,kg%d,nt%d>", w.few ? "few" : stream ? "stream" : w.rows ? "rows" : (w.pw ? "pw" : (w.thin ? "thin" : "wide")),
                 w.dtype == SR_DTYPE_BF16 ? "bf16" : "f32", w.KS, w.KGPT, w.NT);
        const double px = (double)B * H * W;
        double bytes = px * ((double)w.Cin * esz + (double)w.Cout * osz);
        if (p.s1) bytes += px * w.Cout * esz;
        if (p.s2) bytes += px * w.Cout * esz;
        rec = ctx->prof_open(nm, 2.0 * px * w.KS * w.KS * w.Cin * w.Cout, bytes, st);
    }
    int rc;
    switch (rt.fam) {
        case CF_FEW: rc = w.KS == 3 ? launch_fewcout<3>(ctx, p, rt.sub, st) : launch_fewcout<5>(ctx, p, rt.sub, st); break;
        case CF_STREAM: rc = conv_stream_launch(ctx, w, p, st); break;
        case CF_ROWS: rc = conv_rows_launch(ctx, w, p, st); break;
        case CF_PW: rc = conv_pw_launch(ctx, w, p, st); break;
        default: rc = (w.dtype == SR_DTYPE_BF16) ? dispatch<bf16_t>(ctx, rt, p, nct, st) : dispatch<float>(ctx, rt, p, nct, st); break;
    }
    ctx->prof_close(rec, st);
    return rc;
}

int pw2_pack_weights(sr_ctx* ctx, const float* w, const float* bias, int cin, int cout, int act, Pw2Weights* out) {
    if (cin < 32 || cin % 32 != 0 || cin > 96 || cout < 1 || cout > 32) return ctx->fail(SR_ERR_INVALID, "fused 1x1: 32, 64 or 96 input and 1..32 output channels");
    const int NT = cin / 32;
    std::vector<float> host((size_t)NT * 16 * 64, 0.f);
    for (int n = 0; n < NT; ++n)
        for (int i = 0; i < 16; ++i)
            for (int l = 0; l < 64; ++l) {
                const int c = 32 * n + 8 * (i >> 2) + 4 * (l >> 5) + (i & 3), co = l & 31;
                if (co < cout) host[((size_t)n * 16 + i) * 64 + l] = w[(size_t)c * cout + co];
            }
    Pw2Weights pw;
    pw.cin = cin; pw.cout = cout; pw.act = act;
    void* a = nullptr;
    if (int rc = weights_upload(ctx, host.data(), host.size() * sizeof(float), bias, cout, 32, &a, &pw.bias)) return rc;
    pw.a = static_cast<float*>(a);
    *out = pw;
    return SR_OK;
}
```

### super-resolution-images-for-3d-printing-defect-detection_amd/csrc/conv_common.h

```cpp
#pragma once
#include "common.h"

namespace convk {

struct ConvParams {
    const char* in; int64_t in_cs; int in_coff; int in_ps; int in_rs;
    const char* w; const float* bias;
    char* out; int64_t out_cs; int out_coff; int out_ps; int out_rs; int out_f32;
    const char* s1; int64_t s1_cs; int s1_coff; int s1_ps; int s1_rs; float beta1;
    const char* s2; int64_t s2_cs; int s2_coff; int s2_ps; int s2_rs; float beta2;
    float alpha; int act; int clip; int r; int Cd;
    int B, H, W, Cout;
    int nchunks;
    int tilesX, tilesY;
    int vec;
    int skip_lds;
    float skip_scale;
    unsigned long long* dbg;
    const char* f2w;
    float* f2part;
    int f2c;
    const char* pjw;
    const float* pjbias;
    char* pjout; int64_t pj_cs; int pj_coff; int pj_rs; int pj_nblk;
    const float* pw2w; const float* pw2bias; int pw2_cout, pw2_act;
    int splitk_ok;
    int cell_h, cell_w;
    char* plout; int64_t pl_cs; int pl_coff; int pl_gx, pl_ch, pl_cw, pl_Wv;
};

__device__ __forceinline__ int choff(int c, int ps) { return (c >> 5) * ps + (c & 31); }
__device__ __forceinline__ float act_apply(float v, int act) {
    switch (act) {
        case SR_ACT_RELU: return fmaxf(v, 0.f);
        case SR_ACT_LRELU: return v > 0.f ? v : 0.2f * v;
        case SR_ACT_TANH: return tanhf(v);
        default: return v;
    }
}

template <typename T> __device__ __forceinline__ void load4(const char* base, int64_t eoff, bool vec, int n, float v[4]);
template <> __device__ __forceinline__ void load4<float>(const char* base, int64_t eoff, bool vec, int n, float v[4]) {
    const float* p = reinterpret_cast<const float*>(base) + eoff;
    if (vec) { f32x4 t = *reinterpret_cast<const f32x4*>(p); v[0] = t[0]; v[1] = t[1]; v[2] = t[2]; v[3] = t[3]; }
    else { for (int e = 0; e < 4; ++e) v[e] = e < n ? p[e] : 0.f; }
}
template <> __device__ __forceinline__ void load4<bf16_t>(const char* base, int64_t eoff, bool vec, int n, float v[4]) {
    const bf16_t* p = reinterpret_cast<const bf16_t*>(base) + eoff;
    if (vec) { bf16x4 t = *reinterpret_cast<const bf16x4*>(p); for (int e = 0; e < 4; ++e) v[e] = (float)t[e]; }
    else { for (int e = 0; e < 4; ++e) v[e] = e < n ? (float)p[e] : 0.f; }
}
template <typename T> __device__ __forceinline__ void store4(char* base, int64_t eoff, bool vec, int n, const float v[4], bool f32);
template <> __device__ __forceinline__ void store4<float>(char* base, int64_t eoff, bool vec, int n, const float v[4], bool) {
    float* p = reinterpret_cast<float*>(base) + eoff;
    if (vec) { f32x4 t = {v[0], v[1], v[2], v[3]}; *reinterpret_cast<f32x4*>(p) = t; }
    else { for (int e = 0; e < n; ++e) p[e] = v[e]; }
}
template <> __device__ __forceinline__ void store4<bf16_t>(char* base, int64_t eoff, bool vec, int n, const float v[4], bool f32) {
    if (f32) { store4<float>(base, eoff, vec, n, v, true); return; }
    bf16_t* p = reinterpret_cast<bf16_t*>(base) + eoff;
    if (vec) { bf16x4 t = {(bf16_t)v[0], (bf16_t)v[1], (bf16_t)v[2], (bf16_t)v[3]}; *reinterpret_cast<bf16x4*>(p) = t; }
    else { for (int e = 0; e < n; ++e) p[e] = (bf16_t)v[e]; }
}


template <typename T>
__device__ __forceinline__ void epilogue4(const ConvParams& p, int b, int oy, int ox, int c0, const float a[4]) {
    if (c0 >= p.Cout) return;
    const bool vec = p.vec != 0;
    const int64_t pix = ((int64_t)b * p.H + oy) * p.W + ox;
    const int nv = min(4, p.Cout - c0);
    const bool v4 = vec && nv == 4;
    float v[4];
#pragma unroll
    for (int e = 0; e < 4; ++e) v[e] = act_apply(a[e] + p.bias[c0 + e], p.act) * p.alpha;
    if (p.s1) {
        float s[4];
        load4<T>(p.s1, pix * p.s1_cs + p.s1_coff + c0, v4, nv, s);
#pragma unroll
        for (int e = 0; e < 4; ++e) v[e] += p.beta1 * s[e];
    }
    if (p.s2) {
        float s[4];
        load4<T>(p.s2, pix * p.s2_cs + p.s2_coff + c0, v4, nv, s);
#pragma unroll
        for (int e = 0; e < 4; ++e) v[e] += p.beta2 * s[e];
    }
    if (p.clip) {
#pragma unroll
        for (int e = 0; e < 4; ++e) v[e] = fminf(fmaxf(v[e], 0.f), 1.f);
    }
    if (p.r <= 1) {
        store4<T>(p.out, pix * p.out_cs + p.out_coff + c0, v4, nv, v, p.out_f32 != 0);
    } else if (v4) {
        const int sub = c0 / p.Cd, c = c0 - sub * p.Cd;
        const int i = sub / p.r, j = sub - i * p.r;
        const int64_t dst = (((int64_t)b * p.H * p.r + (int64_t)oy * p.r + i) * ((int64_t)p.W * p.r) + (int64_t)ox * p.r + j) * p.out_cs + p.out_coff + c;
        store4<T>(p.out, dst, true, 4, v, p.out_f32 != 0);
    } else {
        for (int e = 0; e < nv; ++e) {
            const int co = c0 + e, sub = co / p.Cd, c = co - sub * p.Cd;
            const int i = sub / p.r, j = sub - i * p.r;
            const int64_t dst = (((int64_t)b * p.H * p.r + (int64_t)oy * p.r + i) * ((int64_t)p.W * p.r) + (int64_t)ox * p.r + j) * p.out_cs + p.out_coff + c;
            store4<T>(p.out, dst, false, 1, v + e, p.out_f32 != 0);
        }
    }
}
// ... 8 lines not shown
```

### super-resolution-images-for-3d-printing-defect-detection_amd/csrc/conv_rows.hip

```cpp
#include <stdlib.h>
#include <string.h>

#include <vector>

#include "conv_rows_epi.h"

namespace {

using namespace convk;

__device__ __forceinline__ f32x4 mma16(bf16x8 a, bf16x8 b, f32x4 c) {
    return __builtin_amdgcn_mfma_f32_16x16x32_bf16(a, b, c, 0, 0, 0);
}

#define STAMP_AT(i) do { if (STAMP && tid == 0) p.dbg[(size_t)blockIdx.x * 16 + (i)] = __builtin_amdgcn_s_memtime(); } while (0)

template <int R>
__device__ __forceinline__ void rows_fuse2(const ConvParams& p, f32x4 (&acc)[R][4], const f32x4 (&biasv)[4], char* smem, int64_t tile, int y0, int x0,
                                           int wave, int lane, int px, int q, int tid) {
    constexpr int TH = 4 * R, RW = 18, ZS = 36;
    const float slope = p.act == SR_ACT_RELU ? 0.f : (p.act == SR_ACT_LRELU ? 0.2f : 1.f);
    const float alpha = p.alpha;
    bf16x8 wa[2][2];
#pragma unroll
    for (int tb = 0; tb < 2; ++tb)
#pragma unroll
        for (int hf = 0; hf < 2; ++hf) wa[tb][hf] = *reinterpret_cast<const bf16x8*>(p.f2w + ((tb * 2 + hf) * 64 + lane) * 16);
    const int ox = x0 + px;
    f32x4 z[R][2];
#pragma unroll
    for (int r = 0; r < R; ++r) {
        const bool live = y0 + wave * R + r < p.H && ox < p.W;
        bf16x8 hb[2], lb[2];
#pragma unroll
        for (int hf = 0; hf < 2; ++hf)
#pragma unroll
            for (int u = 0; u < 2; ++u)
#pragma unroll
                for (int e = 0; e < 4; ++e) {
                    float v = acc[r][2 * hf + u][e] + biasv[2 * hf + u][e];
                    v = fmaxf(v, v * slope) * alpha;
                    const bf16_t hi = (bf16_t)v;
                    hb[hf][4 * u + e] = live ? hi : (bf16_t)0.f;
                    lb[hf][4 * u + e] = live ? (bf16_t)(v - (float)hi) : (bf16_t)0.f;
                }
#pragma unroll
        for (int tb = 0; tb < 2; ++tb) {
            z[r][tb] = mma16(wa[tb][0], lb[0], f32x4{0.f, 0.f, 0.f, 0.f});
            z[r][tb] = mma16(wa[tb][1], lb[1], z[r][tb]);
            z[r][tb] = mma16(wa[tb][0], hb[0], z[r][tb]);
            z[r][tb] = mma16(wa[tb][1], hb[1], z[r][tb]);
        }
    }
    __syncthreads();
    float* zl = reinterpret_cast<float*>(smem);
#pragma unroll
    for (int r = 0; r < R; ++r)
#pragma unroll
        for (int tb = 0; tb < 2; ++tb) *reinterpret_cast<f32x4*>(zl + ((wave * R + r) * 16 + px) * ZS + 16 * tb + 4 * q) = z[r][tb];
    __syncthreads();
    if (tid < (TH + 2) * RW) {
        const int ry = tid / RW, rx = tid - ry * RW, c2 = p.f2c;
        float s[3] = {0.f, 0.f, 0.f};
#pragma unroll
        for (int ky = 0; ky < 3; ++ky) {
            const int sy = ry + ky - 2;
#pragma unroll
            for (int kx = 0; kx < 3; ++kx) {
                const int sx = rx + kx - 2;
                if ((unsigned)sy < (unsigned)TH && (unsigned)sx < 16u) {
                    const float* zp = zl + (sy * 16 + sx) * ZS + (ky * 3 + kx) * c2;
#pragma unroll
                    for (int co = 0; co < 3; ++co)
                        if (co < c2) s[co] += zp[co];
                }
            }
        }
        float* dst = p.f2part + (tile * ((TH + 2) * RW) + tid) * 3;
        dst[0] = s[0]; dst[1] = s[1]; dst[2] = s[2];
    }
}

template <int R, bool HAS1>
__device__ __forceinline__ void rows_epilogue_proj(const ConvParams& p, f32x4 (&acc)[R][4], const f32x4 (&biasv)[4], int b, int y0, int x0, int ct,
                                                   int wave, int lane, int px, int q) {
    typedef unsigned u32x2 __attribute__((ext_vector_type(2)));
    typedef unsigned u32x4 __attribute__((ext_vector_type(4)));
    const int H = p.H, W = p.W, ox = x0 + px, oyw = y0 + wave * R;
    const int rows = min(R, H - oyw);
    if (rows <= 0) return;
    const bool col_ok = ox < W;
    const int oxc = col_ok ? ox : 0;
    const float slope = p.act == SR_ACT_RELU ? 0.f : (p.act == SR_ACT_LRELU ? 0.2f : 1.f);
    const float alpha = p.alpha, beta1 = p.beta1;
    const int rr = p.r, nblk = p.pj_nblk;
    const int si = rr > 1 ? ct / rr : 0, sj = rr > 1 ? ct - si * rr : 0;
    const int lane_c = (q & 1) * 16 + 4 * (q & ~1);
    const int64_t orow0 = ((int64_t)b * H + oyw) * rr + si;
    const int ooff = (ox * rr + sj) * (int)p.out_cs + p.out_coff + (rr > 1 ? 0 : ct * 64) + lane_c;
    const int poff = (ox * rr + sj) * (int)p.pj_cs + p.pj_coff + 4 * q;
    bf16x4 k1[HAS1 ? R : 1][4];
    if (HAS1) {
#pragma unroll
        for (int r = 0; r < R; ++r) {
            const int64_t row = (int64_t)b * H + (oyw + (r < rows ? r : 0));
#pragma unroll
            for (int n = 0; n < 4; ++n)
                k1[r][n] = *reinterpret_cast<const bf16x4*>(reinterpret_cast<const bf16_t*>(p.s1) + row * p.s1_rs + (oxc * (int)p.s1_cs + choff(p.s1_coff + ct * 64 + n * 16 + 4 * q, p.s1_ps)));
        }
    }
    bf16x8 wa[3][2];
    f32x4 pjb[3];
#pragma unroll
    for (int nb = 0; nb < 3; ++nb) {
        const int nbc = nb < nblk ? nb : 0;
#pragma unroll
        for (int hf = 0; hf < 2; ++hf) wa[nb][hf] = *reinterpret_cast<const bf16x8*>(p.pjw + ((nbc * 2 + hf) * 64 + lane) * 16);
        pjb[nb] = *reinterpret_cast<const f32x4*>(p.pjbias + nbc * 16 + 4 * q);
    }
#pragma unroll
    for (int r = 0; r < R; ++r) {
        if (r >= rows) break;
        bf16x4 o[4];
#pragma unroll
        for (int n = 0; n < 4; ++n) {
            f32x4 v = acc[r][n] + biasv[n];
#pragma unroll
            for (int e = 0; e < 4; ++e) v[e] = fmaxf(v[e], v[e] * slope) * alpha;
            if (HAS1) {
#pragma unroll
                for (int e = 0; e < 4; ++e) v[e] += beta1 * (float)k1[r][n][e];
            }
            o[n] = bf16x4{(bf16_t)v[0], (bf16_t)v[1], (bf16_t)v[2], (bf16_t)v[3]};
        }
        bf16_t* const orow = reinterpret_cast<bf16_t*>(p.out) + (orow0 + (int64_t)r * rr) * p.out_rs;
#pragma unroll
        for (int s = 0; s < 2; ++s) {
            const u32x2 au = __builtin_bit_cast(u32x2, o[2 * s]), cu = __builtin_bit_cast(u32x2, o[2 * s + 1]);
            const auto s0 = __builtin_amdgcn_permlane16_swap(au[0], cu[0], false, false);
            const auto s1 = __builtin_amdgcn_permlane16_swap(au[1], cu[1], false, false);
            const u32x4 ov = {(unsigned)s0[0], (unsigned)s1[0], (unsigned)s0[1], (unsigned)s1[1]};
            if (col_ok) *reinterpret_cast<u32x4*>(orow + ooff + 32 * s) = ov;
        }
        bf16x8 hb[2];
#pragma unroll
        for (int hf = 0; hf < 2; ++hf)
#pragma unroll
            for (int e = 0; e < 4; ++e) { hb[hf][e] = o[2 * hf][e]; hb[hf][4 + e] = o[2 * hf + 1][e]; }
        bf16_t* const prow = reinterpret_cast<bf16_t*>(p.pjout) + (orow0 + (int64_t)r * rr) * p.pj_rs;
#pragma unroll
        for (int nb = 0; nb < 3; ++nb) {
            if (nb >= nblk) break;
            f32x4 z = mma16(wa[nb][0], hb[0], pjb[nb]);
            z = mma16(wa[nb][1], hb[1], z);
            const bf16x4 zo = {(bf16_t)z[0], (bf16_t)z[1], (bf16_t)z[2], (bf16_t)z[3]};
            if (col_ok) *reinterpret_cast<bf16x4*>(prow + poff + 16 * nb) = zo;
        }
        __builtin_amdgcn_sched_barrier(0);
    }
}

template <int R>
__device__ __forceinline__ void rows_pool2(const ConvParams& p, f32x4 (&acc)[R][4], const f32x4 (&biasv)[4], char* smem, int b, int y0, int x0, int ct, int wave,
                                           int px, int q, int tid) {
    constexpr int TH = 4 * R, PB = 128 + 16;
    const float slope = p.act == SR_ACT_RELU ? 0.f : (p.act == SR_ACT_LRELU ? 0.2f : 1.f);
    const float alpha = p.alpha;
    __syncthreads();
#pragma unroll
    for (int r = 0; r < R; ++r)
#pragma unroll
        for (int n = 0; n < 4; ++n) {
            f32x4 v = acc[r][n] + biasv[n];
#pragma unroll
            for (int e = 0; e < 4; ++e) v[e] = fmaxf(v[e], v[e] * slope) * alpha;
            *reinterpret_cast<bf16x4*>(smem + ((wave * R + r) * 16 + px) * PB + (16 * n + 4 * q) * 2) = bf16x4{(bf16_t)v[0], (bf16_t)v[1], (bf16_t)v[2], (bf16_t)v[3]};
        }
    __syncthreads();
    const int Ho = p.H >> 1, Wo = p.W >> 1;
#pragma unroll
    for (int it = 0; it < 2; ++it) {
        const int v = tid + 256 * it;
        if (v >= (TH / 2) * 8 * 8) break;
        const int cv = v & 7, ppx = (v >> 3) & 7, pr = v >> 6;
        const int oy = (y0 >> 1) + pr, ox = (x0 >> 1) + ppx;
        if (oy >= Ho || ox >= Wo) continue;
        const char* s = smem + ((2 * pr) * 16 + 2 * ppx) * PB + cv * 16;
        const bf16x8 v00 = *reinterpret_cast<const bf16x8*>(s), v01 = *reinterpret_cast<const bf16x8*>(s + PB);
        const bf16x8 v10 = *reinterpret_cast<const bf16x8*>(s + 16 * PB), v11 = *reinterpret_cast<const bf16x8*>(s + 17 * PB);
        bf16x8 o;
#pragma unroll
        for (int e = 0; e < 8; ++e) o[e] = (bf16_t)fmaxf(fmaxf((float)v00[e], (float)v01[e]), fmaxf((float)v10[e], (float)v11[e]));
        const int64_t pix = p.pl_gx == 0 ? ((int64_t)b * Ho + oy) * Wo + ox : ((int64_t)(b / p.pl_gx) * p.pl_ch + oy) * p.pl_Wv + (b % p.pl_gx) * p.pl_cw + ox;
        *reinterpret_cast<bf16x8*>(reinterpret_cast<bf16_t*>(p.plout) + pix * p.pl_cs + p.pl_coff + ct * 64 + cv * 8) = o;
    }
}

template <int NB16, int R, bool STAMP, int FUSE2 = 0>
__global__ void __launch_bounds__(256, NB16 == 4 ? (R > 3 ? 2 : 3) : 4) conv3_rows_kernel(ConvParams p) {
    constexpr int TH = 4 * R, TW = 16, PH = TH + 2, PW = TW + 2;
    constexpr int NPIX = PH * PW;
    constexpr int NIN = NPIX * 4;
    constexpr int NINT = (NIN + 255) / 256;
    constexpr int LIN_BYTES = NPIX * 64;
    constexpr int WUNITS = 9 * NB16 * 64;
    constexpr int NWT = (WUNITS + 255) / 256;
    constexpr bool WPRE = NB16 <= 1;
    extern __shared__ __attribute__((aligned(16))) char smem[];
    char* lin = smem;
    char* lw = smem + LIN_BYTES;
    float* lbias = reinterpret_cast<float*>(smem + LIN_BYTES + WUNITS * 16);

    const int tid = threadIdx.x, lane = tid & 63, wave = tid >> 6, px = lane & 15, q = lane >> 4;
    STAMP_AT(0);
    int t;
    {
        const int total = gridDim.x, xcd = blockIdx.x & 7, k = blockIdx.x >> 3;
        const int qn = total >> 3, rn = total & 7;
        t = (xcd < rn ? xcd * (qn + 1) : rn * (qn + 1) + (xcd - rn) * qn) + k;
    }
    const int nct = p.tilesX >> 16;
    const int tilesX = p.tilesX & 0xffff;
    const int ct = t % nct; t /= nct;
    const int tx = t % tilesX; t /= tilesX;
    const int ty = t % p.tilesY;
    const int b = t / p.tilesY;
    const int y0 = ty * TH, x0 = tx * TW;
    const int H = p.H, W = p.W, in_cs = (int)p.in_cs, in_rs = p.in_rs, in_ps = p.in_ps;
    const bf16_t* inb = reinterpret_cast<const bf16_t*>(p.in) + (int64_t)b * H * in_rs + choff(p.in_coff, in_ps);

    int soff[NINT], doff[NINT];
#pragma unroll
    for (int i = 0; i < NINT; ++i) {
        const int u = tid + 256 * i;
        const int pix = u >> 2, sl = u & 3;
        const int py = pix / PW, pxx = pix - py * PW;
        const int gy = y0 + py - 1, gx = x0 + pxx - 1;
        const bool live = u < NIN;
        const bool inside = live && (unsigned)gy < (unsigned)H && (unsigned)gx < (unsigned)W;
        doff[i] = live ? pix * 64 + ((sl * 16) ^ ((pix & 4) << 3)) : -1;
        soff[i] = inside ? gy * in_rs + gx * in_cs + sl * 8 : -1;
// ... 73 lines not shown
        if constexpr (WDMA) {
            dma_w(chunk);
            asm volatile("s_waitcnt vmcnt(%0)" ::"n"(DMA_PER_WAVE) : "memory");
#pragma unroll
            for (int i = 0; i < NINT; ++i) asm volatile("" : "+v"(pre[i]));
        } else {
            land_all();
        }
#pragma unroll
        for (int i = 0; i < NINT; ++i)
            if (doff[i] >= 0) {
                bf16x8 z = {};
                *reinterpret_cast<bf16x8*>(lin + doff[i]) = soff[i] >= 0 ? pre[i] : z;
            }
        if constexpr (WDMA) asm volatile("s_waitcnt vmcnt(0)" ::: "memory");
        else write_w();
        __syncthreads();
        if (chunk < 6) STAMP_AT(3 + 2 * chunk);
        if (chunk + 1 < nch) {
            issue(chunk + 1);
            if (WPRE) issue_w(chunk + 1);
        }
        bf16x8 xcur = *reinterpret_cast<const bf16x8*>(lin + xaddr(0, 0));
#pragma unroll
        for (int kx = 0; kx < 3; ++kx) {
            bf16x8 wf[3][NB16];
#pragma unroll
            for (int ky = 0; ky < 3; ++ky)
#pragma unroll
                for (int n = 0; n < NB16; ++n)
                    wf[ky][n] = *reinterpret_cast<const bf16x8*>(lw + ((ky * 3 + kx) * NB16 + n) * 1024 + lane * 16);
#pragma unroll
            for (int yi = 0; yi < R + 2; ++yi) {
                const bf16x8 xf = xcur;
                if (yi + 1 < R + 2) xcur = *reinterpret_cast<const bf16x8*>(lin + xaddr(yi + 1, kx));
                else if (kx + 1 < 3) xcur = *reinterpret_cast<const bf16x8*>(lin + xaddr(0, kx + 1));
#pragma unroll
                for (int ky = 0; ky < 3; ++ky) {
                    const int yo = yi - ky;
                    if (yo >= 0 && yo < R) {
#pragma unroll
                        for (int n = 0; n < NB16; ++n) acc[yo][n] = mma16(wf[ky][n], xf, acc[yo][n]);
                    }
                }
            }
        }
        if constexpr (SKIP_LDS_OK) if (skip_lds) {
            const float sc = p.skip_scale;
#pragma unroll
            for (int n = 0; n < NB16; ++n) {
                const int g = ct * NB16 + n;
                if ((g >> 1) != chunk) continue;
                const int slice = (g & 1) * 2 + (q >> 1);
#pragma unroll
                for (int r = 0; r < R; ++r) {
                    const int tt = (wave * R + r + 1) * PW + px + 1;
                    const bf16x4 xk = *reinterpret_cast<const bf16x4*>(lin + tt * 64 + ((slice * 16) ^ ((tt & 4) << 3)) + (q & 1) * 8);
#pragma unroll
                    for (int e = 0; e < 4; ++e) acc[r][n][e] += sc * (float)xk[e];
                }
            }
        }
    }
    asm volatile("s_waitcnt vmcnt(0)" ::: "memory");
    STAMP_AT(14);

    f32x4 biasv[NB16];
#pragma unroll
    for (int n = 0; n < NB16; ++n) biasv[n] = *reinterpret_cast<const f32x4*>(lbias + n * 16 + 4 * q);
    if constexpr (FUSE2 == 2) {
        static_assert(FUSE2 != 2 || NB16 == 4, "the fused max-pool is built for 64-cout workgroups");
        rows_pool2<R>(p, acc, biasv, smem, b, y0, x0, ct, wave, px, q, tid);
        STAMP_AT(15);
        return;
    }
    if constexpr (FUSE2 == 1) {
        static_assert(FUSE2 != 1 || NB16 == 4, "the fused RGB tail needs all 64 channels of a pixel in one workgroup");
        rows_fuse2<R>(p, acc, biasv, smem, ((int64_t)b * p.tilesY + ty) * tilesX + tx, y0, x0, wave, lane, px, q, tid);
        STAMP_AT(15);
        return;
    }
    if constexpr (NB16 == 4) {
        if (p.pjw) {
            if (p.s1) rows_epilogue_proj<R, true>(p, acc, biasv, b, y0, x0, ct, wave, lane, px, q);
            else rows_epilogue_proj<R, false>(p, acc, biasv, b, y0, x0, ct, wave, lane, px, q);
            STAMP_AT(15);
            return;
        }
    }
    if constexpr (SKIP_LDS_OK) if (skip_lds) {
        ConvParams pe = p;
        if (p.skip_lds == 1) { pe.s1 = p.s2; pe.s1_cs = p.s2_cs; pe.s1_coff = p.s2_coff; pe.s1_ps = p.s2_ps; pe.s1_rs = p.s2_rs; pe.beta1 = p.beta2; }
        pe.s2 = nullptr;
        rows_epilogue<NB16, R>(pe, acc, biasv, b, y0, x0, ct, wave, px, q);
        STAMP_AT(15);
        return;
    }
    rows_epilogue<NB16, R>(p, acc, biasv, b, y0, x0, ct, wave, px, q);
    STAMP_AT(15);
}

template <int NB16, int R = (NB16 == 4 ? 3 : 4)>
int launch_rows(sr_ctx* ctx, const ConvParams& p0, int nct, hipStream_t st) {
    constexpr int lds = (4 * R + 2) * 18 * 64 + 9 * NB16 * 1024 + NB16 * 64;
    static_assert(NB16 != 4 || 4 * R * 16 * 36 * 4 <= lds, "rows_fuse2 parks its tap channels in the tile's LDS");
    ConvParams p = p0;
    const int tilesX = (p.W + 15) / 16;
    p.tilesY = (p.H + 4 * R - 1) / (4 * R);
    if (tilesX > 0xffff || nct > 0x7fff) return ctx->fail(SR_ERR_INVALID, "conv_rows: image too wide / too many cout tiles");
    const int64_t nwg = (int64_t)tilesX * p.tilesY * p.B * nct;
    if (nwg >= (1ll << 31)) return ctx->fail(SR_ERR_INVALID, "conv_rows: too many workgroups for one launch");
    p.tilesX = (nct << 16) | tilesX;
    dim3 grid((unsigned)nwg, 1u);
    if (p.dbg && !p.f2w && !p.plout) {
        if (nwg * 16 * (int64_t)sizeof(unsigned long long) > ctx->stamp_cap)
            return ctx->fail(SR_ERR_INVALID, "conv_rows: the stamp buffer is too small for this launch (sr_debug_stamp_bytes_needed(0, workgroups))");
        auto kd = conv3_rows_kernel<NB16, R, true>;
        if (int rc = ctx->ensure_dyn_lds(reinterpret_cast<const void*>(kd), lds)) return rc;
        hipLaunchKernelGGL(kd, grid, dim3(256), lds, st, p);
        SR_HIP(ctx, hipGetLastError());
        return SR_OK;
    }
    if constexpr (NB16 == 4 && R == 3) {
        if (p.f2w) {
            if (nct != 1) return ctx->fail(SR_ERR_INVALID, "conv_rows: the fused RGB tail needs a 64-cout conv");
            auto kf = conv3_rows_kernel<NB16, R, false, 1>;
            if (int rc = ctx->ensure_dyn_lds(reinterpret_cast<const void*>(kf), lds)) return rc;
            hipLaunchKernelGGL(kf, grid, dim3(256), lds, st, p);
            SR_HIP(ctx, hipGetLastError());
            return SR_OK;
        }
    }
    if (p.f2w) return ctx->fail(SR_ERR_INVALID, "conv_rows: the fused RGB tail needs a 64-cout conv");
    if constexpr (NB16 == 4 && R == 3) {
        if (p.plout) {
            static_assert(NB16 != 4 || 12 * 16 * 144 <= lds, "rows_pool2 parks the tile's outputs in its LDS");
            auto kp = conv3_rows_kernel<NB16, R, false, 2>;
            if (int rc = ctx->ensure_dyn_lds(reinterpret_cast<const void*>(kp), lds)) return rc;
            hipLaunchKernelGGL(kp, grid, dim3(256), lds, st, p);
            SR_HIP(ctx, hipGetLastError());
            return SR_OK;
        }
    }
    if (p.plout) return ctx->fail(SR_ERR_INVALID, "conv_rows: the fused max-pool needs 64-cout workgroups");
    auto kern = conv3_rows_kernel<NB16, R, false>;
    if (int rc = ctx->ensure_dyn_lds(reinterpret_cast<const void*>(kern), lds)) return rc;
    hipLaunchKernelGGL(kern, grid, dim3(256), lds, st, p);
    SR_HIP(ctx, hipGetLastError());
    return SR_OK;
}

}

namespace {

constexpr int F2_TH = 12, F2_TW = 16, F2_REGION = (F2_TH + 2) * (F2_TW + 2);

__global__ void __launch_bounds__(256) rgbtail_finish_kernel(const float* __restrict__ part, int64_t npix, int H, int W, int tilesY, int tilesX,
                                                             const float* __restrict__ bias, int c2, int act, float alpha, int clip, char* out,
                                                             int64_t out_cs, int out_coff, int out_f32) {
    const int64_t i = (int64_t)blockIdx.x * 256 + threadIdx.x;
    if (i >= npix) return;
    const int x = (int)(i % W);
    const int64_t row = i / W;
    const int y = (int)(row % H);
    const int64_t b = row / H;
    const int ty = y / F2_TH, ry = y - ty * F2_TH + 1, tx = x / F2_TW, rx = x - tx * F2_TW + 1;
    float s[3] = {0.f, 0.f, 0.f};
// ... 89 lines not shown
```

### super-resolution-images-for-3d-printing-defect-detection_amd/csrc/conv_rows_epi.h

```cpp
#pragma once
#include "conv_common.h"

namespace convk {

template <int NB16, int R, bool HAS1, bool HAS2, bool PAIR>
__device__ __forceinline__ void rows_epilogue_fast(const ConvParams& p, f32x4 (&acc)[R][NB16], const f32x4 (&biasv)[NB16], int b, int y0,
                                                   int x0, int ct, int wave, int px, int q) {
    typedef unsigned u32x2 __attribute__((ext_vector_type(2)));
    typedef unsigned u32x4 __attribute__((ext_vector_type(4)));
    const int H = p.H, W = p.W;
    const int ox = x0 + px;
    const int oyw = y0 + wave * R;
    const int rows = min(R, H - oyw);
    if (rows <= 0) return;
    const int cell_h = p.cell_h, cell_w = p.cell_w;
    const bool col_ok = ox < W && (cell_w == 0 || ox % cell_w != cell_w - 1);
    const int oxc = ox < W ? ox : 0;
    const float slope = p.act == SR_ACT_RELU ? 0.f : (p.act == SR_ACT_LRELU ? 0.2f : 1.f);
    const float alpha = p.alpha, beta1 = p.beta1, beta2 = p.beta2;
    const bool clip = p.clip != 0, of32 = p.out_f32 != 0;

    constexpr int RG = (HAS1 && HAS2 && NB16 <= 2 && R >= 2) ? R / 2 : R;
    int cc[NB16];
#pragma unroll
// ... 4 lines not shown
    int loff[NS];
    int64_t rb[NS];
    bool live[NS];
    const int64_t rstep = rr_ <= 1 ? (int64_t)p.out_rs : (int64_t)rr_ * p.out_rs;
#pragma unroll
    for (int s = 0; s < NS; ++s) {
        const int blk = (ct * NB16 + (PAIR ? 2 * s : s)) * 16;
        const int lane_c = PAIR ? (q & 1) * 16 + 4 * (q & ~1) : 4 * q;
        live[s] = col_ok && (PAIR || blk + lane_c < p.Cout);
        if (rr_ <= 1) {
            rb[s] = ((int64_t)b * H + oyw) * p.out_rs;
            loff[s] = ox * (int)p.out_cs + choff(p.out_coff + blk + lane_c, p.out_ps);
        } else {
            const int sub = blk / Cd, cb = blk - sub * Cd;
            const int i = sub / rr_, j = sub - i * rr_;
            rb[s] = (((int64_t)b * H + oyw) * rr_ + i) * p.out_rs;
            loff[s] = (ox * rr_ + j) * (int)p.out_cs + p.out_coff + cb + lane_c;
        }
    }

#pragma unroll
    for (int r0 = 0; r0 < R; r0 += RG) {
    if (r0 >= rows) break;
    bf16x4 k1[HAS1 ? RG : 1][NB16], k2[HAS2 ? RG : 1][NB16];
    if (HAS1 || HAS2) {
#pragma unroll
        for (int g = 0; g < RG; ++g) {
            const int64_t row = (int64_t)b * H + (oyw + (r0 + g < rows ? r0 + g : 0));
#pragma unroll
            for (int n = 0; n < NB16; ++n) {
                if (HAS1) k1[g][n] = *reinterpret_cast<const bf16x4*>(reinterpret_cast<const bf16_t*>(p.s1) + row * p.s1_rs + (oxc * (int)p.s1_cs + choff(p.s1_coff + cc[n], p.s1_ps)));
                if (HAS2) k2[g][n] = *reinterpret_cast<const bf16x4*>(reinterpret_cast<const bf16_t*>(p.s2) + row * p.s2_rs + (oxc * (int)p.s2_cs + choff(p.s2_coff + cc[n], p.s2_ps)));
            }
        }
    }
#pragma unroll
    for (int g = 0; g < RG; ++g) {
        const int r = r0 + g;
        if (r >= rows) break;
        const bool row_ok = cell_h == 0 || (oyw + r) % cell_h != cell_h - 1;
        f32x4 v[NB16];
#pragma unroll
        for (int n = 0; n < NB16; ++n) {
            v[n] = acc[r][n] + biasv[n];
#pragma unroll
            for (int e = 0; e < 4; ++e) v[n][e] = fmaxf(v[n][e], v[n][e] * slope) * alpha;
            if (HAS1) {
#pragma unroll
                for (int e = 0; e < 4; ++e) v[n][e] += beta1 * (float)k1[g][n][e];
            }
            if (HAS2) {
#pragma unroll
                for (int e = 0; e < 4; ++e) v[n][e] += beta2 * (float)k2[g][n][e];
            }
            if (clip) {
#pragma unroll
                for (int e = 0; e < 4; ++e) v[n][e] = fminf(fmaxf(v[n][e], 0.f), 1.f);
            }
        }
#pragma unroll
        for (int s = 0; s < NS; ++s) {
            const int64_t base = rb[s] + r * rstep;
            if (PAIR) {
                const int n = 2 * s;
                const bf16x4 a = {(bf16_t)v[n][0], (bf16_t)v[n][1], (bf16_t)v[n][2], (bf16_t)v[n][3]};
                const bf16x4 c = {(bf16_t)v[n + 1][0], (bf16_t)v[n + 1][1], (bf16_t)v[n + 1][2], (bf16_t)v[n + 1][3]};
                const u32x2 au = __builtin_bit_cast(u32x2, a), cu = __builtin_bit_cast(u32x2, c);
                const auto s0 = __builtin_amdgcn_permlane16_swap(au[0], cu[0], false, false);
                const auto s1 = __builtin_amdgcn_permlane16_swap(au[1], cu[1], false, false);
                const u32x4 o = {(unsigned)s0[0], (unsigned)s1[0], (unsigned)s0[1], (unsigned)s1[1]};
                if (live[s] && row_ok) *reinterpret_cast<u32x4*>(reinterpret_cast<bf16_t*>(p.out) + base + loff[s]) = o;
            } else if (of32) {
                if (live[s] && row_ok) *reinterpret_cast<f32x4*>(reinterpret_cast<float*>(p.out) + base + loff[s]) = v[s];
            } else {
                const bf16x4 o = {(bf16_t)v[s][0], (bf16_t)v[s][1], (bf16_t)v[s][2], (bf16_t)v[s][3]};
                if (live[s] && row_ok) *reinterpret_cast<bf16x4*>(reinterpret_cast<bf16_t*>(p.out) + base + loff[s]) = o;
            }
        }
        __builtin_amdgcn_sched_barrier(0);
    }
    }
}

template <int NB16>
__device__ __forceinline__ int rows_epilogue_kind(const ConvParams& p) {
    const int Cd = p.Cd, rr_ = p.r;
    const bool has1 = p.s1 != nullptr, has2 = p.s2 != nullptr;
    const bool fast = p.vec != 0 && (p.Cout & 3) == 0 && p.act != SR_ACT_TANH && (rr_ <= 1 || (Cd & 15) == 0) && (has1 || !has2);
    if (!fast) return -1;
    const bool pair_ok = NB16 >= 2 && p.out_f32 == 0 && (rr_ <= 1 || (Cd & 31) == 0) && (p.Cout & 31) == 0;
    return 2 * (has2 ? 2 : (has1 ? 1 : 0)) + (pair_ok ? 1 : 0);
}

template <int NB16, int R, int KIND>
__device__ __forceinline__ void rows_epilogue_as(const ConvParams& p, f32x4 (&acc)[R][NB16], const f32x4 (&biasv)[NB16], int b, int y0, int x0,
                                                 int ct, int wave, int px, int q) {
    if constexpr (KIND < 0) {
        const int H = p.H, W = p.W;
        const int ox = x0 + px;
        const int oyw = y0 + wave * R;
        if (ox < W) {
#pragma unroll
            for (int r = 0; r < R; ++r) {
                const int oy = oyw + r;
                if (oy >= H) continue;
#pragma unroll
                for (int n = 0; n < NB16; ++n) {
                    const float a[4] = {acc[r][n][0], acc[r][n][1], acc[r][n][2], acc[r][n][3]};
                    epilogue4<bf16_t>(p, b, oy, ox, (ct * NB16 + n) * 16 + 4 * q, a);
                }
            }
        }
    } else {
        constexpr bool PAIR = (KIND & 1) != 0 && NB16 >= 2;
        rows_epilogue_fast<NB16, R, (KIND >> 1) >= 1, (KIND >> 1) >= 2, PAIR>(p, acc, biasv, b, y0, x0, ct, wave, px, q);
    }
}

template <int NB16, int R>
__device__ __forceinline__ void rows_epilogue(const ConvParams& p, f32x4 (&acc)[R][NB16], const f32x4 (&biasv)[NB16], int b, int y0, int x0,
                                              int ct, int wave, int px, int q) {
    switch (rows_epilogue_kind<NB16>(p)) {
        case -1: rows_epilogue_as<NB16, R, -1>(p, acc, biasv, b, y0, x0, ct, wave, px, q); break;
        case 0: rows_epilogue_as<NB16, R, 0>(p, acc, biasv, b, y0, x0, ct, wave, px, q); break;
        case 1: rows_epilogue_as<NB16, R, 1>(p, acc, biasv, b, y0, x0, ct, wave, px, q); break;
        case 2: rows_epilogue_as<NB16, R, 2>(p, acc, biasv, b, y0, x0, ct, wave, px, q); break;
        case 3: rows_epilogue_as<NB16, R, 3>(p, acc, biasv, b, y0, x0, ct, wave, px, q); break;
        case 4: rows_epilogue_as<NB16, R, 4>(p, acc, biasv, b, y0, x0, ct, wave, px, q); break;
        default: rows_epilogue_as<NB16, R, 5>(p, acc, biasv, b, y0, x0, ct, wave, px, q); break;
    }
}

}
```

### super-resolution-images-for-3d-printing-defect-detection_amd/csrc/conv_stream.hip

```cpp
#include <stdlib.h>

#include <algorithm>
#include <type_traits>

#include "conv_rows_epi.h"

namespace {

using namespace convk;

__device__ __forceinline__ f32x4 mma16s(bf16x8 a, bf16x8 b, f32x4 c) { return __builtin_amdgcn_mfma_f32_16x16x32_bf16(a, b, c, 0, 0, 0); }

constexpr int S_NCOMP = 8, S_NLOAD = 4, S_R = 3;
constexpr int S_TH = S_NCOMP * S_R, S_TW = 16, S_PH = S_TH + 2, S_PW = S_TW + 2, S_NPIX = S_PH * S_PW;
constexpr int S_BUF = S_NPIX * 64;
constexpr int S_NBUF = 3;
constexpr int S_WB = 2 * 9 * 4 * 1024;
constexpr int S_LDS = S_WB + S_NBUF * S_BUF + 64 * 4;
constexpr int S_PIECES = (S_NPIX + 15) / 16;
static_assert(S_LDS <= 160 * 1024, "LDS budget");

template <int N> __device__ __forceinline__ void wait_vm() {
    static_assert(N >= 0 && N < 64, "vmcnt is a 6-bit counter");
    asm volatile("s_waitcnt vmcnt(%0)" ::"n"(N) : "memory");
}

struct StreamParams {
    ConvParams c;
    const char* zero;
    int nct, tilesX, tilesY;
    int tiles_per_wg;
    int ntiles;
};

__global__ void __launch_bounds__((S_NCOMP + S_NLOAD) * 64, (S_NCOMP + S_NLOAD + 3) / 4) conv64_stream_kernel(StreamParams sp) {
    extern __shared__ __attribute__((aligned(16))) char smem[];
    char* const lw = smem;
    char* const stg = smem + S_WB;
    float* const lbias = reinterpret_cast<float*>(stg + S_NBUF * S_BUF);
    constexpr int NTHR = (S_NCOMP + S_NLOAD) * 64;
    const ConvParams& p = sp.c;
    const int tid = threadIdx.x, lane = tid & 63, px = lane & 15, q = lane >> 4;
    const int wave = __builtin_amdgcn_readfirstlane(tid >> 6);
    const int ct = blockIdx.x % sp.nct, wgs = blockIdx.x / sp.nct;
    const int t0 = wgs * sp.tiles_per_wg, t1 = min(sp.ntiles, t0 + sp.tiles_per_wg);
    if (t0 >= t1) return;
    const int nunits = 2 * (t1 - t0);
    const int H = p.H, W = p.W;

    {
        const char* wsrc = p.w + (int64_t)ct * S_WB;
        for (int u = tid; u < S_WB / 16; u += NTHR) *reinterpret_cast<f32x4*>(lw + u * 16) = *reinterpret_cast<const f32x4*>(wsrc + u * 16);
        if (tid < 64) lbias[tid] = p.bias[ct * 64 + tid];
    }
    auto tile_of = [&](int tt, int& b, int& y0, int& x0) {
        const int tx = tt % sp.tilesX;
        const int r = tt / sp.tilesX;
        const int ty = r % sp.tilesY;
        b = r / sp.tilesY;
        y0 = ty * S_TH; x0 = tx * S_TW;
    };
    if (wave >= S_NCOMP) {
        asm volatile("s_waitcnt vmcnt(0) lgkmcnt(0)" ::: "memory");
        const int lwr = wave - S_NCOMP;
        auto loader = [&](auto LWc) {
            constexpr int LW = decltype(LWc)::value;
            constexpr int NP = (S_PIECES - LW + 3) / 4;
            int rel[NP];
#pragma unroll
            for (int i = 0; i < NP; ++i) {
                const int t = 16 * (LW + 4 * i) + (lane >> 2);
                rel[i] = t < S_NPIX ? ((t / S_PW) << 16) | (t % S_PW) : -1;
            }
            const int slot = lane & 3;
            auto stage_unit = [&](int k) {
                const int c = k & 1;
                int b, y0, x0;
                tile_of(min(t0 + (k >> 1), t1 - 1), b, y0, x0);
                const char* const img = p.in + ((int64_t)b * H * W * p.in_cs + p.in_coff) * 2 + c * 64;
                char* const dst = stg + (k % S_NBUF) * S_BUF;
#pragma unroll
                for (int i = 0; i < NP; ++i) {
                    const int t = 16 * (LW + 4 * i) + (lane >> 2);
                    const int gy = y0 + (rel[i] >> 16) - 1, gx = x0 + (rel[i] & 0xffff) - 1;
                    const bool inside = rel[i] >= 0 && (unsigned)gy < (unsigned)H && (unsigned)gx < (unsigned)W;
                    const int sl = slot ^ ((t & 4) >> 1);
                    const char* src = inside ? img + ((int64_t)gy * W + gx) * (p.in_cs * 2) + sl * 16 : sp.zero + sl * 16;
                    if (rel[i] >= 0)
                        __builtin_amdgcn_global_load_lds((const __attribute__((address_space(1))) void*)src,
                                                         (__attribute__((address_space(3))) void*)(dst + (LW + 4 * i) * 1024), 16, 0, 0);
                }
            };
            stage_unit(0); stage_unit(1);
            for (int k = 0; k < nunits; ++k) {
                if (k == 0) wait_vm<NP>();
                __builtin_amdgcn_s_barrier();
                stage_unit(k + 2);
                wait_vm<NP>();
            }
            asm volatile("s_waitcnt vmcnt(0)" ::: "memory");
        };
        if (lwr == 0) loader(std::integral_constant<int, 0>{});
        else if (lwr == 1) loader(std::integral_constant<int, 1>{});
        else if (lwr == 2) loader(std::integral_constant<int, 2>{});
        else loader(std::integral_constant<int, 3>{});
        return;
    }
    asm volatile("s_waitcnt vmcnt(0) lgkmcnt(0)" ::: "memory");
    const int tbase = wave * S_R * S_PW + px;
    auto xaddr = [&](int yi, int kx) {
        const int tt = tbase + yi * S_PW + kx;
        return tt * 64 + ((q * 16) ^ ((tt & 4) << 3));
    };
    auto tiles = [&](auto KINDc) {
    constexpr int KIND = decltype(KINDc)::value;
    for (int ti = t0; ti < t1; ++ti) {
        f32x4 acc[S_R][4];
#pragma unroll
        for (int r = 0; r < S_R; ++r)
#pragma unroll
            for (int n = 0; n < 4; ++n) acc[r][n] = f32x4{0.f, 0.f, 0.f, 0.f};
#pragma unroll
        for (int c = 0; c < 2; ++c) {
            const int k = 2 * (ti - t0) + c;
            asm volatile("s_waitcnt lgkmcnt(0)" ::: "memory");
            __builtin_amdgcn_s_barrier();
            const char* const lin = stg + (k % S_NBUF) * S_BUF;
            const char* const lwc = lw + c * (9 * 4 * 1024);
            bf16x8 xcur = *reinterpret_cast<const bf16x8*>(lin + xaddr(0, 0));
#pragma unroll
            for (int kx = 0; kx < 3; ++kx) {
                bf16x8 wf[3][4];
#pragma unroll
                for (int ky = 0; ky < 3; ++ky)
#pragma unroll
                    for (int n = 0; n < 4; ++n) wf[ky][n] = *reinterpret_cast<const bf16x8*>(lwc + ((ky * 3 + kx) * 4 + n) * 1024 + lane * 16);
#pragma unroll
                for (int yi = 0; yi < S_R + 2; ++yi) {
                    const bf16x8 xf = xcur;
                    if (yi + 1 < S_R + 2) xcur = *reinterpret_cast<const bf16x8*>(lin + xaddr(yi + 1, kx));
                    else if (kx + 1 < 3) xcur = *reinterpret_cast<const bf16x8*>(lin + xaddr(0, kx + 1));
#pragma unroll
                    for (int ky = 0; ky < 3; ++ky) {
                        const int yo = yi - ky;
                        if (yo >= 0 && yo < S_R) {
#pragma unroll
                            for (int n = 0; n < 4; ++n) acc[yo][n] = mma16s(wf[ky][n], xf, acc[yo][n]);
                        }
                    }
                }
            }
        }
        int b, y0, x0;
        tile_of(ti, b, y0, x0);
        f32x4 biasv[4];
#pragma unroll
        for (int n = 0; n < 4; ++n) biasv[n] = *reinterpret_cast<const f32x4*>(lbias + n * 16 + 4 * q);
        rows_epilogue_as<4, S_R, KIND>(p, acc, biasv, b, y0, x0, ct, wave, px, q);
    }
    };
    switch (rows_epilogue_kind<4>(p)) {
        case 0: tiles(std::integral_constant<int, 0>{}); break;
        case 1: tiles(std::integral_constant<int, 1>{}); break;
        case 2: tiles(std::integral_constant<int, 2>{}); break;
        default: tiles(std::integral_constant<int, 3>{}); break;
    }
}

}

bool conv_stream_supported(const ConvWeights& w, const convk::ConvParams& p) {
    return w.rows && w.dtype == SR_DTYPE_BF16 && w.NT == 4 && w.nchunks == 2 && w.Cin == 64 && w.CoutP == w.Cout && p.in_ps == 32 && p.in_cs >= 64 && p.in_cs % 8 == 0 &&
           p.in_coff % 8 == 0 && p.H % S_TH == 0 && p.W % S_TW == 0 && p.skip_lds == 0 && !p.f2w && !p.pjw && !p.plout && !p.dbg && p.cell_h == 0 && p.cell_w == 0 &&
           p.vec != 0 && (p.Cout & 3) == 0 && p.act != SR_ACT_TANH && (p.r <= 1 || (p.Cd & 15) == 0) && !p.s2;
}

int conv_stream_launch(sr_ctx* ctx, const ConvWeights& w, const convk::ConvParams& p0, hipStream_t st) {
    if (!ctx->zero_page) return ctx->fail(SR_ERR_STATE, "context has no zero page");
    StreamParams sp;
    sp.c = p0;
    sp.zero = static_cast<const char*>(ctx->zero_page);
    sp.nct = w.CoutP / 64;
    sp.tilesX = p0.W / S_TW; sp.tilesY = p0.H / S_TH;
    sp.c.tilesX = sp.tilesX; sp.c.tilesY = sp.tilesY;
    const int64_t ntiles = (int64_t)p0.B * sp.tilesX * sp.tilesY;
    if (ntiles >= (1ll << 30)) return ctx->fail(SR_ERR_INVALID, "conv_stream: too many tiles for one launch");
    sp.ntiles = (int)ntiles;
    const int ncu = ctx->cu_count();
    const int groups = (int)std::max<int64_t>(1, std::min<int64_t>(ntiles, ncu / sp.nct > 0 ? ncu / sp.nct : 1));
    sp.tiles_per_wg = (int)((ntiles + groups - 1) / groups);
    const int ngroups = (int)((ntiles + sp.tiles_per_wg - 1) / sp.tiles_per_wg);
    auto k = conv64_stream_kernel;
    if (int rc = ctx->ensure_dyn_lds(reinterpret_cast<const void*>(k), S_LDS)) return rc;
    hipLaunchKernelGGL(k, dim3(ngroups * sp.nct), dim3((S_NCOMP + S_NLOAD) * 64), S_LDS, st, sp);
    SR_HIP(ctx, hipGetLastError());
    return SR_OK;
}
```

### super-resolution-images-for-3d-printing-defect-detection_amd/sr355/_lib.py

```python
import ctypes as C
import os

_HERE = os.path.dirname(os.path.abspath(__file__))
LIB_PATH = os.path.join(_HERE, "libsr355.so")

SR_OK = 0
SR_ERR_INVALID, SR_ERR_HIP, SR_ERR_OOM, SR_ERR_STATE, SR_ERR_NAME, SR_ERR_CAPACITY = -1, -2, -3, -4, -5, -6
DTYPE_F32, DTYPE_BF16, DTYPE_U8 = 0, 1, 2
MODEL_SRCNN, MODEL_EDSR, MODEL_ESRGAN_G, MODEL_VGG16, MODEL_ESRGAN_D, MODEL_VGG19_FEATURES = 0, 1, 2, 3, 4, 5
ACT_LINEAR, ACT_RELU, ACT_LRELU, ACT_TANH = 0, 1, 2, 3
WEIGHT_KERNEL, WEIGHT_BIAS = 0, 1
SP_MAXPOOL2, SP_GAP, SP_PICK2, SP_VGG_PREPROCESS = 0, 1, 2, 3
ELT_AXPBY, ELT_RELU_BWD, ELT_LRELU_BWD, ELT_CLIP01_BWD, ELT_MUL, ELT_TANH_BWD, ELT_CLIP01, ELT_SIGN_DIFF = 0, 1, 2, 3, 4, 5, 6, 7
FUSE_DENSE_TAIL, FUSE_DENSE_MID, FUSE_RGB_TAIL, FUSE_ATTN_PROJ, FUSE_CELLS, FUSE_CONV1_STREAM, FUSE_POOL, FUSE_CONV_STREAM, FUSE_SRCNN_1X1 = \
    1, 2, 4, 8, 16, 32, 64, 128, 256
FUSE_ALL = 511
FUSE_TWO_UP = FUSE_DENSE_TAIL | FUSE_DENSE_MID | FUSE_CONV1_STREAM


class ModelCfg(C.Structure):
    _fields_ = [("compute_dtype", C.c_int32), ("scale_factor", C.c_int32), ("channels", C.c_int32),
                ("num_blocks", C.c_int32), ("num_filters", C.c_int32), ("growth_channels", C.c_int32),
                ("res_scaling", C.c_float), ("num_classes", C.c_int32), ("use_attention", C.c_int32)]


class View(C.Structure):
    _fields_ = [("p", C.c_void_p), ("cs", C.c_int64), ("coff", C.c_int32)]


class PackDesc(C.Structure):
    _fields_ = [("w", C.c_void_p), ("bias", C.c_void_p), ("K", C.c_int32), ("Cin", C.c_int32), ("Cout", C.c_int32), ("rot", C.c_int32)]


class SnDesc(C.Structure):
    _fields_ = [("koff", C.c_int64), ("K", C.c_int32), ("Cout", C.c_int32), ("uoff", C.c_int64)]


class PatchSide(C.Structure):
    _fields_ = [("src", C.c_void_p), ("out", C.c_void_p), ("dtype", C.c_int32), ("N", C.c_int32), ("H", C.c_int32), ("W", C.c_int32),
                ("pad_h", C.c_int32), ("pad_w", C.c_int32), ("swap_rb", C.c_int32), ("mul", C.c_float), ("add", C.c_float)]


_vp, _i, _f, _i64 = C.c_void_p, C.c_int, C.c_float, C.c_int64
_vw = C.POINTER(View)
_fp = C.POINTER(C.c_float)
_i64p = C.POINTER(C.c_int64)

SIGNATURES = {
    "sr_init": (_i, [_i, C.POINTER(_vp)]),
    "sr_destroy": (None, [_vp]),
    "sr_last_error": (C.c_char_p, [_vp]),
    "sr_mem_info": (_i, [_vp, _i64p, _i64p]),
    "sr_last_forward_ms": (_i, [_vp, _fp]),
    "sr_debug_set_stamp_buffer": (_i, [_vp, _vp, _i64]),
    "sr_debug_stamp_bytes_needed": (_i64, [_i, _i64]),
    "sr_measure_clock": (_i, [_vp, _fp, _vp]),
    "sr_debug_set_chain_stamp_buffer": (_i, [_vp, _vp, _i64]),
    "sr_debug_set_fused": (_i, [_vp, _i, _i]),
    "sr_debug_set_alloc_cap": (_i, [_vp, _i64]),
    "sr_debug_conv_routes": (_i, [_vp, _i, C.c_char_p, _i64]),
    "sr_profile_begin": (_i, [_vp]),
    "sr_profile_end": (_i, [_vp, C.c_char_p, _i64]),
    "sr_model_create": (_i, [_vp, _i, C.POINTER(ModelCfg), C.POINTER(_vp)]),
    "sr_model_destroy": (None, [_vp]),
    "sr_model_release_workspace": (_i, [_vp]),
    "sr_model_num_ops": (_i, [_vp]),
    "sr_model_op_info": (_i, [_vp, _i, C.POINTER(C.c_char_p), C.POINTER(_i), C.POINTER(_i), C.POINTER(_i), C.POINTER(_i)]),
    "sr_model_set_tap": (_i, [_vp, _i, _vp, _i64]),
    "sr_model_num_params": (_i, [_vp]),
    "sr_model_param_info": (_i, [_vp, _i, C.POINTER(C.c_char_p), C.POINTER(_i), _i64p, C.POINTER(_i)]),
    "sr_model_set_weight": (_i, [_vp, C.c_char_p, _i, _fp, _i64p, _i]),
    "sr_model_finalize": (_i, [_vp]),
    "sr_model_output_shape": (_i, [_vp, _i, _i, _i, _i, _i64p]),
    "sr_forward": (_i, [_vp, _vp, _i, _i, _i, _i, _i, _vp, _i64, _vp]),
    "sr_conv2d": (_i, [_vp, _vp, _i, _i, _i, _i, _i, _fp, _fp, _i, _i, _i, _i, _f, _vp, _f, _vp, _f, _i, _i, _vp, _vp]),
    "sr_self_attention": (_i, [_vp, _vp, _i, _i, _i, _i, _i, _fp, _fp, _fp, _fp, _fp, _fp, _fp, _fp, _vp, _vp]),
    "sr_bicubic": (_i, [_vp, _vp, _i, _i, _i, _i, _i, _i, _i, _vp, _vp]),
    "sr_resize": (_i, [_vp, _vp, _i, _i, _i, _i, _i, _i, _i, _i, _vp, _vp]),
    "sr_psnr": (_i, [_vp, _vp, _vp, _i, _i, _i, _i, _f, _vp, _vp]),
    "sr_ssim": (_i, [_vp, _vp, _vp, _i, _i, _i, _i, _f, _vp, _vp]),
    "sr_mse": (_i, [_vp, _vp, _vp, _i64, _vp, _vp]),
    "sr_conv2d_dev": (_i, [_vp, _vp, _i, _i, _i, _i, _vp, _vp, _i, _i, _i, _i, _f, _vp, _f, _vp, _f, _i, _i, _vp, _vp]),
    "sr_conv2d_wgrad": (_i, [_vp, _vp, _vp, _i, _i, _i, _i, _i, _i, _vp, _vp, _vp]),
    "sr_conv2d_dev_views": (_i, [_vp, _vw, _i, _i, _i, _i, _vp, _vp, _i, _i, _i, _i, _f, _vw, _f, _vw, _vp]),
    "sr_conv_prepack": (_i, [_vp, C.POINTER(PackDesc), _i, _vp]),
    "sr_conv2d_wgrad_views": (_i, [_vp, _vw, _vw, _i, _i, _i, _i, _i, _i, _vp, _vp, _vp]),
    "sr_eltwise_views": (_i, [_vp, _i, _vw, _vw, _f, _f, _vw, _i64, _i, _vp]),
    "sr_eltwise": (_i, [_vp, _i, _vp, _vp, _f, _f, _vp, _i64, _vp]),
    "sr_adam": (_i, [_vp, _vp, _vp, _vp, _vp, _i64, _f, _f, _f, _f, _f, _f, _f, _vp]),
    "sr_space_to_depth": (_i, [_vp, _vp, _i, _i, _i, _i, _i, _vp, _vp]),
    "sr_spatial_op": (_i, [_vp, _i, _vp, _i, _i, _i, _i, _vp, _vp]),
    "sr_matmul": (_i, [_vp, _vp, _vp, _vp, _i, _i, _i, _i, _i, _i, _f, _vp]),
    "sr_softmax_rows": (_i, [_vp, _vp, _i64, _i, _vp]),
    "sr_softmax_bwd": (_i, [_vp, _vp, _vp, _vp, _i64, _i, _vp]),
    "sr_maxpool2_bwd": (_i, [_vp, _vp, _vp, _i, _i, _i, _i, _vp, _vp]),
    "sr_zero_insert2": (_i, [_vp, _vp, _i, _i, _i, _i, _vp, _vp]),
    "sr_spectral_l1_bwd": (_i, [_vp, _vp, _vp, _i, _i, _i, _i, _f, _vp, _vp]),
    "sr_l1": (_i, [_vp, _vp, _vp, _i64, _vp, _vp]),
    "sr_spectral_l1": (_i, [_vp, _vp, _vp, _i, _i, _i, _i, _vp, _vp]),
    "sr_extract_patches": (_i, [_vp, _vp, _i, _i, _i, _i, _i, _f, _f, _i, _vp, _i64, C.POINTER(_i), _vp]),
    "sr_overlap_add": (_i, [_vp, _vp, _i, _i, _i, _i, _i, _i, _i, _f, _f, _vp, _vp]),
    "sr_extract_patches_batch": (_i, [_vp, _vp, _i, _i, _i, _i, _i, _i, _i, _f, _f, _i, _vp, _i64, C.POINTER(_i), _vp]),
    "sr_patch_vote": (_i, [_vp, _vp, _i, _i, _i, _vp, _vp, _vp, _vp]),
    "sr_classification_counts": (_i, [_vp, _vp, _vp, _vp, _i, _i, _i, _vp, _vp, _vp]),
    "sr_back_projection": (_i, [_vp, _vp, _vp, _i, _i, _i, _i, _i, _i, _vp, _vp, _vp]),
    "sr_noise_sigma": (_i, [_vp, _vp, _i, _i, _i, _vp, _vp]),
    "sr_nl_means": (_i, [_vp, _vp, _i, _i, _i, _i, _i, _vp, C.c_double, _vp, _vp]),
    "sr_edge_guided": (_i, [_vp, _vp, _i, _i, _i, _i, _i, _f, _vp, _vp, _vp]),
    "sr_freq_extrapolate": (_i, [_vp, _vp, _i, _i, _i, _i, _i, _vp, _vp]),
    "sr_classic_scores": (_i, [_vp, _vp, _i, _vp, _i, _i, _i, _i, _i, _vp, C.c_double, _vp, _vp, _vp, _vp, _vp, _vp]),
    "sr_rgb2gray_u8": (_i, [_vp, _vp, _i, _i, _i, _vp, _vp]),
    "sr_freq_to_u8": (_i, [_vp, _vp, _i, _i, _i, _vp, _vp, _vp]),
    "sr_ssim_map": (_i, [_vp, _vp, _i, _vp, _i, _i, _i, _i, _i, _vp, _vp, _vp, _vp]),
    "sr_eda_pair_stats": (_i, [_vp, _vp, _vp, _i, _i, _i, _i, _i, _vp, _vp, _vp, _vp, _vp, _vp, _vp, _vp, _vp, _vp]),
    "sr_eda_accumulate": (_i, [_vp, _vp, _vp, _i, _i, _i, _vp, _vp, _vp, _vp, _vp, _vp]),
    "sr_eda_pair_panels": (_i, [_vp, _vp, _vp, _i, _i, _i, _vp, _vp, _vp, _vp, _vp, _vp, _vp, _vp, _vp]),
    "sr_degrade_gauss": (_i, [_vp, _vp, _i, _i, _i, _vp, _vp, _vp]),
    "sr_degrade_motion": (_i, [_vp, _vp, _i, _i, _i, _vp, _vp, _vp]),
    "sr_degrade_noise": (_i, [_vp, _vp, _i, _i, _i, _vp, _vp, C.c_uint64, _vp, _vp, _vp]),
    "sr_degrade_jpeg": (_i, [_vp, _vp, _i, _i, _i, _vp, _vp, _vp, _vp, _vp, _vp, _vp, _vp, _vp]),
    "sr_degrade_status": (_i, [_vp, _vp]),
    "sr_object_boxes": (_i, [_vp, _vp, _i, _i, _i, _vp, _vp, _vp, _vp, _vp]),
    "sr_square_crop": (_i, [_vp, _vp, _i, _i, _i, _vp, _vp, _vp]),
    "sr_affine_warp": (_i, [_vp, _vp, _i, _i, _i, _i, _vp, _i, _vp, _vp, _vp]),
    "sr_dense_head_workspace_bytes": (_i64, [_i, _i]),
    "sr_dense_head_step": (_i, [_vp, _vp, _i, _i, _i, _i, _vp, _vp, _vp, _f, _vp, _f, _vp, _vp, _vp, _i64, _vp]),
    "sr_spectral_norm_bucket": (_i, [_vp, _vp, _i64, _vp, _i64, C.POINTER(SnDesc), _i, _vp]),
    "sr_disc_head_step": (_i, [_vp, _vp, _i, _i, _i, _i, _i, _i, _vp, _f, _vp, _vp, _vp, _vp, _i, _vp]),
    "sr_lpips_shapes": (_i, [_i, _i, C.POINTER(_i)]),
    "sr_lpips_input_table": (_i, [_fp]),
    "sr_lpips_set_weights": (_i, [_vp, C.POINTER(_fp), C.POINTER(_fp), C.POINTER(_fp)]),
    "sr_lpips": (_i, [_vp, _vp, _vp, _i, _i, _i, _i, _vp, _vp, C.POINTER(_vp), _vp]),
    "sr_gather_patch_pairs": (_i, [_vp, C.POINTER(PatchSide), C.POINTER(PatchSide), _vp, _i, _vp, _i64, _i64, _i, _i, _i, _i, _vp]),
    "sr_gather_warp_patches": (_i, [_vp, _vp, _i, _i, _i, _i, _vp, _i, _vp, _i64, _i64, _i, _i, _i, _i, _vp, _vp, _vp]),
    "sr_clip_by_norm_bucket": (_i, [_vp, _vp, _i64, _vp, _i, C.c_double, _vp, _vp]),
}

SCORE_NAMES = ("psnr", "ssim", "mae", "rmse", "grad_mse", "epi", "hf_ratio", "kl_luma", "kl_color")

EDA_STAT_NAMES = (("psnr", "ssim", "glcm_contrast", "glcm_homogeneity", "glcm_correlation")
                  + tuple(f"{k}_{s}" for k in ("rms_noise", "lap_var", "blocking", "color_noise", "ringing", "saturation_mean", "brightness_mean")
                          for s in ("lr", "hr"))
# ... 42 lines not shown
```

### super-resolution-images-for-3d-printing-defect-detection_amd/sr355/runtime.py

```python
import ctypes as C

import numpy as np
import torch

from . import _lib as L


class Sr355Error(RuntimeError):
    pass


_EXC = {L.SR_ERR_INVALID: ValueError, L.SR_ERR_HIP: Sr355Error, L.SR_ERR_OOM: MemoryError,
        L.SR_ERR_STATE: RuntimeError, L.SR_ERR_NAME: KeyError, L.SR_ERR_CAPACITY: ValueError}

_TORCH2DT = {torch.float32: L.DTYPE_F32, torch.bfloat16: L.DTYPE_BF16, torch.uint8: L.DTYPE_U8}
_DT2TORCH = {v: k for k, v in _TORCH2DT.items()}


def dtype_code(dt):
    if isinstance(dt, str):
        dt = {"f32": torch.float32, "float32": torch.float32, "bf16": torch.bfloat16, "bfloat16": torch.bfloat16,
              "u8": torch.uint8}[dt]
    return _TORCH2DT[dt]

# ... 16 lines not shown
    if not t.is_contiguous():
        raise ValueError(f"{name}: tensor must be contiguous")
    return t


def gauss_taps(ksize, sigma):
    if ksize not in (3, 5, 7) or not sigma > 0:
        raise ValueError(f"gauss_taps: ksize must be 3, 5 or 7 and sigma positive, got {ksize!r}, {sigma!r}")
    r = ksize // 2
    g = np.exp(-((np.arange(ksize, dtype=np.float64) - r) ** 2) / (2.0 * float(sigma) ** 2))
    t = np.floor(256.0 * g / g.sum() + 0.5).astype(np.int64)
    t[r] += 256 - int(t.sum())
    return t.astype(np.int32)


class Context:
    _instances = {}

    @classmethod
    def get(cls, device=None):
        if device is None:
            if not torch.cuda.is_available():
                raise RuntimeError("sr355 needs an MI355X: torch.cuda.is_available() is False and there is no CPU path")
            device = torch.cuda.current_device()
        if isinstance(device, torch.device):
            device = device.index if device.index is not None else torch.cuda.current_device()
        if device not in cls._instances:
            cls._instances[device] = cls(device)
        return cls._instances[device]

    def __init__(self, device):
        self.lib = L.load()
        self.device = int(device)
        h = C.c_void_p()
        rc = self.lib.sr_init(self.device, C.byref(h))
        if rc != L.SR_OK:
            raise Sr355Error(f"sr_init(device={device}) failed with {rc} (no usable GPU?)")
        self.h = h
        self.torch_device = torch.device("cuda", self.device)

    def check(self, rc):
        if rc != L.SR_OK:
            msg = self.lib.sr_last_error(self.h).decode("utf-8", "replace")
            raise _EXC.get(rc, Sr355Error)(msg)

    def stream(self):
        return C.c_void_p(torch.cuda.current_stream(self.torch_device).cuda_stream)

    def to_device(self, a, dtype=None):
        t = a if isinstance(a, torch.Tensor) else torch.from_numpy(np.ascontiguousarray(a))
        if dtype is not None and t.dtype != dtype:
            t = t.to(dtype)
        return t.to(self.torch_device, non_blocking=False).contiguous()

    def empty(self, shape, dtype=torch.float32):
        return torch.empty(tuple(int(s) for s in shape), dtype=dtype, device=self.torch_device)

    def mem_info(self):
        cur, peak = C.c_int64(), C.c_int64()
        self.check(self.lib.sr_mem_info(self.h, C.byref(cur), C.byref(peak)))
        return {"current": cur.value, "peak": peak.value}

    def last_forward_ms(self):
        ms = C.c_float()
        self.check(self.lib.sr_last_forward_ms(self.h, C.byref(ms)))
        return ms.value

    def measure_clock_mhz(self):
        mhz = C.c_float()
        self.check(self.lib.sr_measure_clock(self.h, C.byref(mhz), self.stream()))
        return mhz.value

    FUSED_ALL = 511
    FUSED_DENSE_TAIL, FUSED_DENSE_MID, FUSED_RGB_TAIL = L.FUSE_DENSE_TAIL, L.FUSE_DENSE_MID, L.FUSE_RGB_TAIL
    FUSED_ATTN_PROJ, FUSED_CELLS, FUSED_CONV1_STREAM = L.FUSE_ATTN_PROJ, L.FUSE_CELLS, L.FUSE_CONV1_STREAM
    FUSED_POOL, FUSED_CONV_STREAM, FUSED_SRCNN_1X1 = L.FUSE_POOL, L.FUSE_CONV_STREAM, L.FUSE_SRCNN_1X1
    FUSED_TWO_UP = L.FUSE_TWO_UP

    def set_fused(self, mask=511, max_workgroups=0):
        self.check(self.lib.sr_debug_set_fused(self.h, int(mask), int(max_workgroups)))

    def set_alloc_cap(self, nbytes):
        self.check(self.lib.sr_debug_set_alloc_cap(self.h, int(nbytes)))

    def conv_routes(self, enable=True):
        buf = C.create_string_buffer(1 << 16)
        self.check(self.lib.sr_debug_conv_routes(self.h, int(bool(enable)), buf, len(buf)))
        return buf.value.decode().split()

    def profile_begin(self):
        self.check(self.lib.sr_profile_begin(self.h))

    def profile_end(self):
        import json
        buf = C.create_string_buffer(1 << 16)
        self.check(self.lib.sr_profile_end(self.h, buf, len(buf)))
        return json.loads(buf.value.decode())

    def conv2d(self, x, w, b=None, act="linear", alpha=1.0, skip1=None, beta1=0.0, skip2=None, beta2=0.0,
               clip01=False, d2s=1):
        w = _np32(w)
        b = _np32(b)
        kh, kw, cin, cout = w.shape
        _check_tensor(self, x, "conv2d input", (torch.float32, torch.bfloat16))
        for nm, sk in (("skip1", skip1), ("skip2", skip2)):
            if sk is not None:
                _check_tensor(self, sk, f"conv2d {nm}", (x.dtype,))
        B, H, W, Cx = x.shape
        if Cx != cin:
            raise ValueError("conv2d: input channels do not match the kernel")
        r = max(1, int(d2s))
        y = self.empty((B, H * r, W * r, cout // (r * r)), x.dtype)
        actc = {"linear": L.ACT_LINEAR, None: L.ACT_LINEAR, "relu": L.ACT_RELU, "lrelu": L.ACT_LRELU, "tanh": L.ACT_TANH}[act]
        self.check(self.lib.sr_conv2d(self.h, x.data_ptr(), dtype_code(x.dtype), B, H, W, cin, _fptr(w), _fptr(b), kh, kw, cout,
                                      actc, float(alpha), None if skip1 is None else skip1.data_ptr(), float(beta1),
                                      None if skip2 is None else skip2.data_ptr(), float(beta2), int(bool(clip01)), r,
                                      y.data_ptr(), self.stream()))
        return y

    def conv2d_dev(self, x, w_dev, b_dev, cout, rot=False, act="linear", d2s=1, alpha=1.0, skip1=None, beta1=0.0):
        _check_tensor(self, x, "conv2d_dev input")
        _check_tensor(self, w_dev, "conv2d_dev kernel")
        if b_dev is not None:
            _check_tensor(self, b_dev, "conv2d_dev bias")
        if skip1 is not None:
            _check_tensor(self, skip1, "conv2d_dev skip1")
        B, H, W, Cx = x.shape
        k = w_dev.shape[0]
        want = (k, k, cout, Cx) if rot else (k, k, Cx, cout)
        if tuple(w_dev.shape) != want:
            raise ValueError(f"conv2d_dev: kernel shape {tuple(w_dev.shape)} does not match {want}")
        r = max(1, int(d2s))
        y = self.empty((B, H * r, W * r, cout // (r * r)), torch.float32)
        actc = {"linear": L.ACT_LINEAR, None: L.ACT_LINEAR, "relu": L.ACT_RELU, "lrelu": L.ACT_LRELU, "tanh": L.ACT_TANH}[act]
        self.check(self.lib.sr_conv2d_dev(self.h, x.data_ptr(), B, H, W, Cx, w_dev.data_ptr(), None if b_dev is None else b_dev.data_ptr(), k,
                                          int(cout), int(bool(rot)), actc, float(alpha), None if skip1 is None else skip1.data_ptr(), float(beta1),
                                          None, 0.0, 0, r, y.data_ptr(), self.stream()))
        return y

    def self_attention(self, x, wf, bf, wg, bg, wh, bh, wv, bv):
        _check_tensor(self, x, "self_attention input", (torch.float32, torch.bfloat16))
        B, H, W, Cx = x.shape
        arrs = [_np32(a) for a in (wf, bf, wg, bg, wh, bh, wv, bv)]
        y = torch.empty_like(x)
        self.check(self.lib.sr_self_attention(self.h, x.data_ptr(), dtype_code(x.dtype), B, H, W, Cx, *[_fptr(a) for a in arrs],
                                              y.data_ptr(), self.stream()))
        return y

    def bicubic(self, x, out_h, out_w):
        _check_tensor(self, x, "bicubic input", (torch.float32, torch.uint8))
        B, H, W, Cx = x.shape
        y = self.empty((B, out_h, out_w, Cx), x.dtype)
        self.check(self.lib.sr_bicubic(self.h, x.data_ptr(), dtype_code(x.dtype), B, H, W, Cx, int(out_h), int(out_w), y.data_ptr(),
                                       self.stream()))
        return y

    INTERPOLATIONS = {"INTER_NEAREST": 0, "INTER_LINEAR": 1, "INTER_CUBIC": 2, "INTER_AREA": 3, "INTER_LANCZOS4": 4, "INTER_LINEAR_EXACT": 5}

    def resize(self, x, out_h, out_w, interpolation="INTER_CUBIC"):
        code = self.INTERPOLATIONS.get(interpolation, interpolation)
        _check_tensor(self, x, "resize input", (torch.float32, torch.uint8))
        if code == 5 and x.dtype == torch.float32:
            code = 1
        if isinstance(code, bool) or not isinstance(code, (int, np.integer)) or int(code) not in (0, 1, 2, 3, 4):
            raise ValueError(f"unsupported interpolation {interpolation!r}")
        B, H, W, Cx = x.shape
# ... 977 lines not shown
```

Measured before the change: 112.5.

## Fuse attention key-norm computation into conv projection epilogue and stream kernel

The conv epilogue that computes the fused QKV projection now also writes each pixel's squared key norm to a side buffer. The attention launch can then reduce those per-key values into group max norms with a light kernel, instead of rereading the key channels of the QKV tensor. The projection epilogue is moved into a shared header so the streaming conv kernel can use it, and that kernel gains a grouped workgroup-to-tile mapping and support for planar-blocked inputs. The cost is extra epilogue arithmetic and stores, plus a new arena buffer and a debug API.

```diff
diff --git a/include/sr355.h b/include/sr355.h
--- a/include/sr355.h
+++ b/include/sr355.h
@@ -55,6 +55,7 @@
 enum { SR_FUSE_DENSE_TAIL = 1, SR_FUSE_DENSE_MID = 2, SR_FUSE_RGB_TAIL = 4, SR_FUSE_ATTN_PROJ = 8, SR_FUSE_CELLS = 16, SR_FUSE_CONV1_STREAM = 32,
        SR_FUSE_POOL = 64, SR_FUSE_CONV_STREAM = 128, SR_FUSE_SRCNN_1X1 = 256, SR_FUSE_ALL = 511,
        SR_FUSE_TWO_UP = SR_FUSE_DENSE_TAIL | SR_FUSE_DENSE_MID | SR_FUSE_CONV1_STREAM };
+int  sr_debug_attn_key_norms(sr_ctx* ctx, float* device_dst, int64_t capacity, int64_t* count);
 int  sr_debug_set_alloc_cap(sr_ctx* ctx, int64_t bytes);
 int  sr_debug_conv_routes(sr_ctx* ctx, int enable, char* text, int64_t cap);
 int  sr_profile_begin(sr_ctx* ctx);
diff --git a/super-resolution-images-for-3d-printing-defect-detection_amd/csrc/api.hip b/super-resolution-images-for-3d-printing-defect-detection_amd/csrc/api.hip
--- a/super-resolution-images-for-3d-printing-defect-detection_amd/csrc/api.hip
+++ b/super-resolution-images-for-3d-printing-defect-detection_amd/csrc/api.hip
@@ -575,6 +575,8 @@
     c->zero_page = c->dalloc(sr_ctx::ZERO_PAGE_BYTES);
     if (!c->zero_page) { sr_destroy(c); return SR_ERR_OOM; }
     if (hipMemset(c->zero_page, 0, sr_ctx::ZERO_PAGE_BYTES) != hipSuccess) { sr_destroy(c); return SR_ERR_HIP; }
+    const char* kp = getenv("SR355_KNORM_PASS");
+    c->knorm_pass = kp && atoi(kp) != 0;
     *out = c;
     return SR_OK;
 }
@@ -647,6 +649,17 @@
     if (!ctx) return SR_ERR_INVALID;
     ctx->chain_mask = mask;
     ctx->chain_max_wgs = max_workgroups > 0 ? max_workgroups : 0;
+    return SR_OK;
+}
+
+int sr_debug_attn_key_norms(sr_ctx* ctx, float* device_dst, int64_t capacity, int64_t* count) {
+    DeviceGuard dg_(ctx);
+    if (!ctx || !count) return SR_ERR_INVALID;
+    *count = ctx->attn_key_n2.p ? ctx->attn_key_n2_count : 0;
+    if (*count == 0 || !device_dst) return SR_OK;
+    if (capacity < *count) return ctx->fail(SR_ERR_CAPACITY, "sr_debug_attn_key_norms: destination too small");
+    SR_HIP(ctx, hipDeviceSynchronize());
+    SR_HIP(ctx, hipMemcpy(device_dst, ctx->attn_key_n2.p, sizeof(float) * (size_t)*count, hipMemcpyDeviceToDevice));
     return SR_OK;
 }
 
@@ -928,6 +941,8 @@
     plan_routes(m, L, B, H, W);
     SR_HIP(ctx, hipEventRecord(ctx->ev0, st));
     const int T = m->T;
+    const void* kn_qkv = nullptr;
+    const float* kn_n2 = nullptr;
     for (size_t oi = 0; oi < m->ops.size(); ++oi) {
         const Op& op = m->ops[oi];
         const int route = m->routes[oi];
@@ -995,7 +1010,16 @@
                 }
                 if (route == RT_PW2) ep.pw2 = &m->pw2s[op.pw2].w;
                 else if (nx && nx->kind == OP_POOL) { ep.pool_out = m->view(nx->out); ep.pool_grid = m->grid_now[nx->out.buf]; }
-                else if (nx) { ep.pj = &m->projs[op.proj].w; ep.pj_out = m->view(nx->out); }
+                else if (nx) {
+                    ep.pj = &m->projs[op.proj].w; ep.pj_out = m->view(nx->out);
+                    const Op* at = oi + 2 < m->ops.size() ? &m->ops[oi + 2] : nullptr;
+                    if (at && at->kind == OP_ATTN && at->in.buf == nx->out.buf && at->in.coff == 0 && T == SR_DTYPE_BF16 && !g.gx && !ctx->knorm_pass) {
+                        const size_t nkey = (size_t)cB * h * op.d2s * w * op.d2s;
+                        float* kn = static_cast<float*>(ctx->arena(ctx->attn_key_n2, nkey * sizeof(float), st));
+                        if (!kn) return SR_ERR_OOM;
+                        ep.pj_kn = kn; kn_qkv = ep.pj_out.p; kn_n2 = kn; ctx->attn_key_n2_count = (int64_t)nkey;
+                    }
+                }
                 if (op.out.buf == -2) {
                     ep.out_f32 = io_dtype == SR_DTYPE_F32;
                     rc = conv_launch(ctx, cs.w, xin, B, h, w, y, m->out_C, 0, ep, st);
@@ -1011,7 +1035,8 @@
                 rc = vgg_preproc_launch(ctx, x, io_dtype, (int64_t)B * H * W, po, T, vo.cs, st);
                 break;
             case OP_ATTN:
-                rc = attention_launch(ctx, T, vi.p, vi.cs,  8,  0,  16, B, h * w, po, vo.cs, 0, st);
+                rc = attention_launch(ctx, T, vi.p, vi.cs,  8,  0,  16, B, h * w, po, vo.cs, 0, st, kn_qkv == vi.p ? kn_n2 : nullptr);
+                kn_qkv = nullptr;
                 break;
             case OP_SUBSAMPLE:
                 rc = subsample2_launch(ctx, T, vi.p, B, h, w, m->bufs[op.in.buf].C, vi.cs, po, vo.cs, st);
diff --git a/super-resolution-images-for-3d-printing-defect-detection_amd/csrc/attention.hip b/super-resolution-images-for-3d-printing-defect-detection_amd/csrc/attention.hip
--- a/super-resolution-images-for-3d-printing-defect-detection_amd/csrc/attention.hip
+++ b/super-resolution-images-for-3d-printing-defect-detection_amd/csrc/attention.hip
@@ -1,5 +1,6 @@
 #include "common.h"
 
+#include <algorithm>
 #include <cstdlib>
 
 namespace {
@@ -128,6 +129,22 @@
 #pragma unroll
     for (int o = 32; o > 0; o >>= 1) m = fmaxf(m, __shfl_xor(m, o));
     if (lane == 0) out[(int64_t)b * ngroups + g] = sqrtf(m);
+}
+
+__global__ void __launch_bounds__(256) attn_knorm_reduce_kernel(const float* __restrict__ n2, int N, int ngroups, int64_t total, float* __restrict__ out) {
+    const int lane = threadIdx.x & 63;
+    for (int64_t i = (int64_t)blockIdx.x * 4 + (threadIdx.x >> 6); i < total; i += (int64_t)gridDim.x * 4) {
+        const int g = (int)(i % ngroups);
+        const int64_t b = i / ngroups;
+        const int key = g * 128 + 2 * lane;
+        const float* src = n2 + b * N + key;
+        float m = 0.f;
+        if (key + 1 < N && (N & 1) == 0) { const float2 v = *reinterpret_cast<const float2*>(src); m = fmaxf(v.x, v.y); }
+        else { if (key < N) m = src[0]; if (key + 1 < N) m = fmaxf(m, src[1]); }
+#pragma unroll
+        for (int o = 32; o > 0; o >>= 1) m = fmaxf(m, __shfl_xor(m, o));
+        if (lane == 0) out[i] = sqrtf(m);
+    }
 }
 
 template <int QB>
@@ -379,7 +396,7 @@
 }
 
 int attention_launch(sr_ctx* ctx, int dtype, const void* qkv, int64_t cs, int qoff, int koff, int voff, int B, int N,
-                     void* o, int64_t o_cs, int o_coff, hipStream_t st) {
+                     void* o, int64_t o_cs, int o_coff, hipStream_t st, const float* key_n2) {
     if (B <= 0 || N <= 0) return ctx->fail(SR_ERR_INVALID, "attention: empty tensor");
     const int esz = dtype_size(dtype);
     if ((cs * esz) % 16 || (qoff * esz) % 16 || (koff * esz) % 16 || (voff * esz) % 16 || (o_cs * esz) % 16 || (o_coff * esz) % 16)
@@ -397,7 +414,12 @@
         float* kn = static_cast<float*>(ctx->arena(ctx->attn_kn, sizeof(float) * (size_t)B * ngroups, st));
         if (!kn) { ctx->prof_close(rec, st); return SR_ERR_OOM; }
         p.knorm = kn;
-        hipLaunchKernelGGL(attn_knorm_kernel, dim3((unsigned)((int64_t)B * ngroups)), dim3(64), 0, st, reinterpret_cast<const bf16_t*>(qkv) + 0, cs, koff, N, ngroups, kn);
+        if (key_n2) {
+            const int64_t total = (int64_t)B * ngroups;
+            hipLaunchKernelGGL(attn_knorm_reduce_kernel, dim3((unsigned)std::min<int64_t>((total + 3) / 4, 4096)), dim3(256), 0, st, key_n2, N, ngroups, total, kn);
+        } else {
+            hipLaunchKernelGGL(attn_knorm_kernel, dim3((unsigned)((int64_t)B * ngroups)), dim3(64), 0, st, reinterpret_cast<const bf16_t*>(qkv) + 0, cs, koff, N, ngroups, kn);
+        }
         hipLaunchKernelGGL(attn_bf16_kernel<QBr>, dim3((unsigned)nwg), dim3(256), 0, st, p);
     }
     else hipLaunchKernelGGL(attn_f32_kernel, grid, dim3(256), 0, st, p);
diff --git a/super-resolution-images-for-3d-printing-defect-detection_amd/csrc/common.h b/super-resolution-images-for-3d-printing-defect-detection_amd/csrc/common.h
--- a/super-resolution-images-for-3d-printing-defect-detection_amd/csrc/common.h
+++ b/super-resolution-images-for-3d-printing-defect-detection_amd/csrc/common.h
@@ -44,6 +44,9 @@
     void* tab_buf = nullptr; size_t tab_cap = 0;
     struct Arena { void* p = nullptr; size_t cap = 0; };
     Arena attn_kn;
+    Arena attn_key_n2;
+    int64_t attn_key_n2_count = 0;
+    bool knorm_pass = false;
     Arena dev_w, dev_b, dev_x;
     Arena cls_tab, cls_work, cls_fft;
     std::unordered_map<int64_t, double*> dft_ops;
@@ -179,6 +182,7 @@
     int cell_h = 0, cell_w = 0;
     const ProjWeights* pj = nullptr;
     TensorView pj_out;
+    float* pj_kn = nullptr;
     const Pw2Weights* pw2 = nullptr;
     const RgbTailWeights* f2 = nullptr;
     float* f2_part = nullptr;
@@ -229,7 +233,7 @@
                  float beta_o, hipStream_t st, bool seam = false);
 
 int attention_launch(sr_ctx* ctx, int dtype, const void* qkv, int64_t cs, int qoff, int koff, int voff,
-                     int B, int N, void* o, int64_t o_cs, int o_coff, hipStream_t st);
+                     int B, int N, void* o, int64_t o_cs, int o_coff, hipStream_t st, const float* key_n2 = nullptr);
 
 int nhwc_to_blocked_launch(sr_ctx* ctx, const void* src, int64_t src_cs, int src_coff, int B, int H, int W, int C, void* dst, int64_t dst_C,
                            int dst_coff, hipStream_t st);
diff --git a/super-resolution-images-for-3d-printing-defect-detection_amd/csrc/conv.hip b/super-resolution-images-for-3d-printing-defect-detection_amd/csrc/conv.hip
--- a/super-resolution-images-for-3d-printing-defect-detection_amd/csrc/conv.hip
+++ b/super-resolution-images-for-3d-printing-defect-detection_amd/csrc/conv.hip
@@ -824,7 +824,7 @@
     p.B = B; p.H = H; p.W = W; p.Cout = w.Cout; p.nchunks = w.nchunks; p.tilesX = p.tilesY = 0;
     p.dbg = ctx->stamp_buf;
     p.f2w = nullptr; p.f2part = nullptr; p.f2c = 0;
-    p.pjw = nullptr; p.pjbias = nullptr; p.pjout = nullptr; p.pj_cs = 0; p.pj_coff = 0; p.pj_rs = 0; p.pj_nblk = 0;
+    p.pjw = nullptr; p.pjbias = nullptr; p.pjout = nullptr; p.pj_cs = 0; p.pj_coff = 0; p.pj_rs = 0; p.pj_nblk = 0; p.pjkn = nullptr;
     p.cell_h = ep.cell_h; p.cell_w = ep.cell_w;
     p.splitk_ok = ep.allow_splitk;
     p.pw2w = nullptr; p.pw2bias = nullptr; p.pw2_cout = 0; p.pw2_act = 0;
@@ -858,6 +858,7 @@
         p.pjw = static_cast<const char*>(ep.pj->a); p.pjbias = ep.pj->bias; p.pj_nblk = ep.pj->nblk;
         p.skip_lds = 0; p.skip_scale = 0.f;
         p.pjout = static_cast<char*>(const_cast<void*>(ep.pj_out.p)); p.pj_cs = ep.pj_out.cs; p.pj_coff = ep.pj_out.coff; p.pj_rs = (int)(W * r * ep.pj_out.cs);
+        p.pjkn = ep.pj_kn;
     }
     if (ep.pw2) {
         if (!(w.dtype == SR_DTYPE_F32 && w.thin && !w.few && w.NT == 1 && w.CoutP == 96 && ep.pw2->a && ep.pw2->cin == w.Cout && ep.pw2->cout >= 1 && ep.pw2->cout <= 32 && r == 1 &&
diff --git a/super-resolution-images-for-3d-printing-defect-detection_amd/csrc/conv_common.h b/super-resolution-images-for-3d-printing-defect-detection_amd/csrc/conv_common.h
--- a/super-resolution-images-for-3d-printing-defect-detection_amd/csrc/conv_common.h
+++ b/super-resolution-images-for-3d-printing-defect-detection_amd/csrc/conv_common.h
@@ -23,6 +23,7 @@
     const char* pjw;
     const float* pjbias;
     char* pjout; int64_t pj_cs; int pj_coff; int pj_rs; int pj_nblk;
+    float* pjkn;
     const float* pw2w; const float* pw2bias; int pw2_cout, pw2_act;
     int splitk_ok;
     int cell_h, cell_w;
diff --git a/super-resolution-images-for-3d-printing-defect-detection_amd/csrc/conv_rows.hip b/super-resolution-images-for-3d-printing-defect-detection_amd/csrc/conv_rows.hip
--- a/super-resolution-images-for-3d-printing-defect-detection_amd/csrc/conv_rows.hip
+++ b/super-resolution-images-for-3d-printing-defect-detection_amd/csrc/conv_rows.hip
@@ -78,85 +78,6 @@
         }
         float* dst = p.f2part + (tile * ((TH + 2) * RW) + tid) * 3;
         dst[0] = s[0]; dst[1] = s[1]; dst[2] = s[2];
-    }
-}
-
-template <int R, bool HAS1>
-__device__ __forceinline__ void rows_epilogue_proj(const ConvParams& p, f32x4 (&acc)[R][4], const f32x4 (&biasv)[4], int b, int y0, int x0, int ct,
-                                                   int wave, int lane, int px, int q) {
-    typedef unsigned u32x2 __attribute__((ext_vector_type(2)));
-    typedef unsigned u32x4 __attribute__((ext_vector_type(4)));
-    const int H = p.H, W = p.W, ox = x0 + px, oyw = y0 + wave * R;
-    const int rows = min(R, H - oyw);
-    if (rows <= 0) return;
-    const bool col_ok = ox < W;
-    const int oxc = col_ok ? ox : 0;
-    const float slope = p.act == SR_ACT_RELU ? 0.f : (p.act == SR_ACT_LRELU ? 0.2f : 1.f);
-    const float alpha = p.alpha, beta1 = p.beta1;
-    const int rr = p.r, nblk = p.pj_nblk;
-    const int si = rr > 1 ? ct / rr : 0, sj = rr > 1 ? ct - si * rr : 0;
-    const int lane_c = (q & 1) * 16 + 4 * (q & ~1);
-    const int64_t orow0 = ((int64_t)b * H + oyw) * rr + si;
-    const int ooff = (ox * rr + sj) * (int)p.out_cs + p.out_coff + (rr > 1 ? 0 : ct * 64) + lane_c;
-    const int poff = (ox * rr + sj) * (int)p.pj_cs + p.pj_coff + 4 * q;
-    bf16x4 k1[HAS1 ? R : 1][4];
-    if (HAS1) {
-#pragma unroll
-        for (int r = 0; r < R; ++r) {
-            const int64_t row = (int64_t)b * H + (oyw + (r < rows ? r : 0));
-#pragma unroll
-            for (int n = 0; n < 4; ++n)
-                k1[r][n] = *reinterpret_cast<const bf16x4*>(reinterpret_cast<const bf16_t*>(p.s1) + row * p.s1_rs + (oxc * (int)p.s1_cs + choff(p.s1_coff + ct * 64 + n * 16 + 4 * q, p.s1_ps)));
-        }
-    }
-    bf16x8 wa[3][2];
-    f32x4 pjb[3];
-#pragma unroll
-    for (int nb = 0; nb < 3; ++nb) {
-        const int nbc = nb < nblk ? nb : 0;
-#pragma unroll
-        for (int hf = 0; hf < 2; ++hf) wa[nb][hf] = *reinterpret_cast<const bf16x8*>(p.pjw + ((nbc * 2 + hf) * 64 + lane) * 16);
-        pjb[nb] = *reinterpret_cast<const f32x4*>(p.pjbias + nbc * 16 + 4 * q);
-    }
-#pragma unroll
-    for (int r = 0; r < R; ++r) {
-        if (r >= rows) break;
-        bf16x4 o[4];
-#pragma unroll
-        for (int n = 0; n < 4; ++n) {
-            f32x4 v = acc[r][n] + biasv[n];
-#pragma unroll
-            for (int e = 0; e < 4; ++e) v[e] = fmaxf(v[e], v[e] * slope) * alpha;
-            if (HAS1) {
-#pragma unroll
-                for (int e = 0; e < 4; ++e) v[e] += beta1 * (float)k1[r][n][e];
-            }
-            o[n] = bf16x4{(bf16_t)v[0], (bf16_t)v[1], (bf16_t)v[2], (bf16_t)v[3]};
-        }
-        bf16_t* const orow = reinterpret_cast<bf16_t*>(p.out) + (orow0 + (int64_t)r * rr) * p.out_rs;
-#pragma unroll
-        for (int s = 0; s < 2; ++s) {
-            const u32x2 au = __builtin_bit_cast(u32x2, o[2 * s]), cu = __builtin_bit_cast(u32x2, o[2 * s + 1]);
-            const auto s0 = __builtin_amdgcn_permlane16_swap(au[0], cu[0], false, false);
-            const auto s1 = __builtin_amdgcn_permlane16_swap(au[1], cu[1], false, false);
-            const u32x4 ov = {(unsigned)s0[0], (unsigned)s1[0], (unsigned)s0[1], (unsigned)s1[1]};
-            if (col_ok) *reinterpret_cast<u32x4*>(orow + ooff + 32 * s) = ov;
-        }
-        bf16x8 hb[2];
-#pragma unroll
-        for (int hf = 0; hf < 2; ++hf)
-#pragma unroll
-            for (int e = 0; e < 4; ++e) { hb[hf][e] = o[2 * hf][e]; hb[hf][4 + e] = o[2 * hf + 1][e]; }
-        bf16_t* const prow = reinterpret_cast<bf16_t*>(p.pjout) + (orow0 + (int64_t)r * rr) * p.pj_rs;
-#pragma unroll
-        for (int nb = 0; nb < 3; ++nb) {
-            if (nb >= nblk) break;
-            f32x4 z = mma16(wa[nb][0], hb[0], pjb[nb]);
-            z = mma16(wa[nb][1], hb[1], z);
-            const bf16x4 zo = {(bf16_t)z[0], (bf16_t)z[1], (bf16_t)z[2], (bf16_t)z[3]};
-            if (col_ok) *reinterpret_cast<bf16x4*>(prow + poff + 16 * nb) = zo;
-        }
-        __builtin_amdgcn_sched_barrier(0);
     }
 }
 
@@ -396,8 +317,8 @@
     }
     if constexpr (NB16 == 4) {
         if (p.pjw) {
-            if (p.s1) rows_epilogue_proj<R, true>(p, acc, biasv, b, y0, x0, ct, wave, lane, px, q);
-            else rows_epilogue_proj<R, false>(p, acc, biasv, b, y0, x0, ct, wave, lane, px, q);
+            if (p.s1) rows_epilogue_as<NB16, R, 7>(p, acc, biasv, b, y0, x0, ct, wave, px, q);
+            else rows_epilogue_as<NB16, R, 6>(p, acc, biasv, b, y0, x0, ct, wave, px, q);
             STAMP_AT(15);
             return;
         }
diff --git a/super-resolution-images-for-3d-printing-defect-detection_amd/csrc/conv_rows_epi.h b/super-resolution-images-for-3d-printing-defect-detection_amd/csrc/conv_rows_epi.h
--- a/super-resolution-images-for-3d-printing-defect-detection_amd/csrc/conv_rows_epi.h
+++ b/super-resolution-images-for-3d-printing-defect-detection_amd/csrc/conv_rows_epi.h
@@ -110,10 +110,104 @@
     }
 }
 
+template <int R, bool HAS1>
+__device__ __forceinline__ void rows_epilogue_proj(const ConvParams& p, f32x4 (&acc)[R][4], const f32x4 (&biasv)[4], int b, int y0, int x0, int ct,
+                                                   int wave, int lane, int px, int q) {
+    typedef unsigned u32x2 __attribute__((ext_vector_type(2)));
+    typedef unsigned u32x4 __attribute__((ext_vector_type(4)));
+    const int H = p.H, W = p.W, ox = x0 + px, oyw = y0 + wave * R;
+    const int rows = min(R, H - oyw);
+    if (rows <= 0) return;
+    const bool col_ok = ox < W;
+    const int oxc = col_ok ? ox : 0;
+    const float slope = p.act == SR_ACT_RELU ? 0.f : (p.act == SR_ACT_LRELU ? 0.2f : 1.f);
+    const float alpha = p.alpha, beta1 = p.beta1;
+    const int rr = p.r, nblk = p.pj_nblk;
+    const int si = rr > 1 ? ct / rr : 0, sj = rr > 1 ? ct - si * rr : 0;
+    const int lane_c = (q & 1) * 16 + 4 * (q & ~1);
+    const int64_t orow0 = ((int64_t)b * H + oyw) * rr + si;
+    const int ooff = (ox * rr + sj) * (int)p.out_cs + p.out_coff + (rr > 1 ? 0 : ct * 64) + lane_c;
+    const int poff = (ox * rr + sj) * (int)p.pj_cs + p.pj_coff + 4 * q;
+    {
+        bf16x4 k1[HAS1 ? R : 1][4];
+        if (HAS1) {
+#pragma unroll
+            for (int r = 0; r < R; ++r) {
+                const int64_t row = (int64_t)b * H + (oyw + (r < rows ? r : 0));
+#pragma unroll
+                for (int n = 0; n < 4; ++n)
+                    k1[r][n] = *reinterpret_cast<const bf16x4*>(reinterpret_cast<const bf16_t*>(p.s1) + row * p.s1_rs + (oxc * (int)p.s1_cs + choff(p.s1_coff + ct * 64 + n * 16 + 4 * q, p.s1_ps)));
+            }
+        }
+#pragma unroll
+        for (int r = 0; r < R; ++r)
+#pragma unroll
+            for (int n = 0; n < 4; ++n) {
+                f32x4 v = acc[r][n] + biasv[n];
+#pragma unroll
+                for (int e = 0; e < 4; ++e) v[e] = fmaxf(v[e], v[e] * slope) * alpha;
+                if (HAS1) {
+#pragma unroll
+                    for (int e = 0; e < 4; ++e) v[e] += beta1 * (float)k1[r][n][e];
+                }
+                acc[r][n] = v;
+            }
+        __builtin_amdgcn_sched_barrier(0);
+    }
+    bf16x8 wa[3][2];
+    f32x4 pjb[3];
+#pragma unroll
+    for (int nb = 0; nb < 3; ++nb) {
+        const int nbc = nb < nblk ? nb : 0;
+#pragma unroll
+        for (int hf = 0; hf < 2; ++hf) wa[nb][hf] = *reinterpret_cast<const bf16x8*>(p.pjw + ((nbc * 2 + hf) * 64 + lane) * 16);
+        pjb[nb] = *reinterpret_cast<const f32x4*>(p.pjbias + nbc * 16 + 4 * q);
+    }
+#pragma unroll
+    for (int r = 0; r < R; ++r) {
+        if (r >= rows) break;
+        bf16x4 o[4];
+#pragma unroll
+        for (int n = 0; n < 4; ++n) o[n] = bf16x4{(bf16_t)acc[r][n][0], (bf16_t)acc[r][n][1], (bf16_t)acc[r][n][2], (bf16_t)acc[r][n][3]};
+        bf16_t* const orow = reinterpret_cast<bf16_t*>(p.out) + (orow0 + (int64_t)r * rr) * p.out_rs;
+#pragma unroll
+        for (int s = 0; s < 2; ++s) {
+            const u32x2 au = __builtin_bit_cast(u32x2, o[2 * s]), cu = __builtin_bit_cast(u32x2, o[2 * s + 1]);
+            const auto s0 = __builtin_amdgcn_permlane16_swap(au[0], cu[0], false, false);
+            const auto s1 = __builtin_amdgcn_permlane16_swap(au[1], cu[1], false, false);
+            const u32x4 ov = {(unsigned)s0[0], (unsigned)s1[0], (unsigned)s0[1], (unsigned)s1[1]};
+            if (col_ok) *reinterpret_cast<u32x4*>(orow + ooff + 32 * s) = ov;
+        }
+        bf16x8 hb[2];
+#pragma unroll
+        for (int hf = 0; hf < 2; ++hf)
+#pragma unroll
+            for (int e = 0; e < 4; ++e) { hb[hf][e] = o[2 * hf][e]; hb[hf][4 + e] = o[2 * hf + 1][e]; }
+        bf16_t* const prow = reinterpret_cast<bf16_t*>(p.pjout) + (orow0 + (int64_t)r * rr) * p.pj_rs;
+#pragma unroll
+        for (int nb = 0; nb < 3; ++nb) {
+            if (nb >= nblk) break;
+            f32x4 z = __builtin_amdgcn_mfma_f32_16x16x32_bf16(wa[nb][0], hb[0], pjb[nb], 0, 0, 0);
+            z = __builtin_amdgcn_mfma_f32_16x16x32_bf16(wa[nb][1], hb[1], z, 0, 0, 0);
+            const bf16x4 zo = {(bf16_t)z[0], (bf16_t)z[1], (bf16_t)z[2], (bf16_t)z[3]};
+            if (col_ok) *reinterpret_cast<bf16x4*>(prow + poff + 16 * nb) = zo;
+            if (nb == 0 && p.pjkn) {
+                const float k0 = (float)zo[0], k1v = (float)zo[1], k2 = (float)zo[2], k3 = (float)zo[3];
+                const float n2 = (k0 * k0 + k1v * k1v) + (k2 * k2 + k3 * k3);
+                const auto sw = __builtin_amdgcn_permlane16_swap(__builtin_bit_cast(unsigned, n2), __builtin_bit_cast(unsigned, n2), false, false);
+                const float kn = n2 + __builtin_bit_cast(float, (unsigned)sw[1]);
+                if (col_ok && q == 0) p.pjkn[(orow0 + (int64_t)r * rr) * ((int64_t)W * rr) + (ox * rr + sj)] = kn;
+            }
+        }
+        __builtin_amdgcn_sched_barrier(0);
+    }
+}
+
 template <int NB16>
 __device__ __forceinline__ int rows_epilogue_kind(const ConvParams& p) {
     const int Cd = p.Cd, rr_ = p.r;
     const bool has1 = p.s1 != nullptr, has2 = p.s2 != nullptr;
+    if (NB16 == 4 && p.pjw) return has1 ? 7 : 6;
     const bool fast = p.vec != 0 && (p.Cout & 3) == 0 && p.act != SR_ACT_TANH && (rr_ <= 1 || (Cd & 15) == 0) && (has1 || !has2);
     if (!fast) return -1;
     const bool pair_ok = NB16 >= 2 && p.out_f32 == 0 && (rr_ <= 1 || (Cd & 31) == 0) && (p.Cout & 31) == 0;
@@ -139,6 +233,9 @@
                 }
             }
         }
+    } else if constexpr (KIND >= 6) {
+        static_assert(KIND < 6 || NB16 == 4, "the fused projection needs all 64 channels of a pixel in one workgroup");
+        rows_epilogue_proj<R, KIND == 7>(p, acc, biasv, b, y0, x0, ct, wave, q * 16 + px, px, q);
     } else {
         constexpr bool PAIR = (KIND & 1) != 0 && NB16 >= 2;
         rows_epilogue_fast<NB16, R, (KIND >> 1) >= 1, (KIND >> 1) >= 2, PAIR>(p, acc, biasv, b, y0, x0, ct, wave, px, q);
diff --git a/super-resolution-images-for-3d-printing-defect-detection_amd/csrc/conv_stream.hip b/super-resolution-images-for-3d-printing-defect-detection_amd/csrc/conv_stream.hip
--- a/super-resolution-images-for-3d-printing-defect-detection_amd/csrc/conv_stream.hip
+++ b/super-resolution-images-for-3d-printing-defect-detection_amd/csrc/conv_stream.hip
@@ -42,7 +42,12 @@
     const ConvParams& p = sp.c;
     const int tid = threadIdx.x, lane = tid & 63, px = lane & 15, q = lane >> 4;
     const int wave = __builtin_amdgcn_readfirstlane(tid >> 6);
-    const int ct = blockIdx.x % sp.nct, wgs = blockIdx.x / sp.nct;
+    int ct, wgs;
+    {
+        const int sb = 8 * sp.nct, nfull = (int)(gridDim.x / sb) * sb, bi = blockIdx.x;
+        if (bi < nfull) { const int rem = bi % sb; ct = rem >> 3; wgs = (bi / sb) * 8 + (rem & 7); }
+        else { const int rem = bi - nfull; ct = rem % sp.nct; wgs = nfull / sp.nct + rem / sp.nct; }
+    }
     const int t0 = wgs * sp.tiles_per_wg, t1 = min(sp.ntiles, t0 + sp.tiles_per_wg);
     if (t0 >= t1) return;
     const int nunits = 2 * (t1 - t0);
@@ -77,7 +82,7 @@
                 const int c = k & 1;
                 int b, y0, x0;
                 tile_of(min(t0 + (k >> 1), t1 - 1), b, y0, x0);
-                const char* const img = p.in + ((int64_t)b * H * W * p.in_cs + p.in_coff) * 2 + c * 64;
+                const char* const img = p.in + ((int64_t)b * H * p.in_rs + choff(p.in_coff, p.in_ps) + c * p.in_ps) * 2;
                 char* const dst = stg + (k % S_NBUF) * S_BUF;
 #pragma unroll
                 for (int i = 0; i < NP; ++i) {
@@ -85,7 +90,7 @@
                     const int gy = y0 + (rel[i] >> 16) - 1, gx = x0 + (rel[i] & 0xffff) - 1;
                     const bool inside = rel[i] >= 0 && (unsigned)gy < (unsigned)H && (unsigned)gx < (unsigned)W;
                     const int sl = slot ^ ((t & 4) >> 1);
-                    const char* src = inside ? img + ((int64_t)gy * W + gx) * (p.in_cs * 2) + sl * 16 : sp.zero + sl * 16;
+                    const char* src = inside ? img + ((int64_t)gy * p.in_rs + gx * (int)p.in_cs) * 2 + sl * 16 : sp.zero + sl * 16;
                     if (rel[i] >= 0)
                         __builtin_amdgcn_global_load_lds((const __attribute__((address_space(1))) void*)src,
                                                          (__attribute__((address_space(3))) void*)(dst + (LW + 4 * i) * 1024), 16, 0, 0);
@@ -156,13 +161,17 @@
         f32x4 biasv[4];
 #pragma unroll
         for (int n = 0; n < 4; ++n) biasv[n] = *reinterpret_cast<const f32x4*>(lbias + n * 16 + 4 * q);
-        rows_epilogue_as<4, S_R, KIND>(p, acc, biasv, b, y0, x0, ct, wave, px, q);
+        int pxe = px, qe = q;
+        if constexpr (KIND >= 6) asm volatile("" : "+v"(pxe), "+v"(qe));
+        rows_epilogue_as<4, S_R, KIND>(p, acc, biasv, b, y0, x0, ct, wave, pxe, qe);
     }
     };
     switch (rows_epilogue_kind<4>(p)) {
         case 0: tiles(std::integral_constant<int, 0>{}); break;
         case 1: tiles(std::integral_constant<int, 1>{}); break;
         case 2: tiles(std::integral_constant<int, 2>{}); break;
+        case 6: tiles(std::integral_constant<int, 6>{}); break;
+        case 7: tiles(std::integral_constant<int, 7>{}); break;
         default: tiles(std::integral_constant<int, 3>{}); break;
     }
 }
@@ -170,8 +179,10 @@
 }
 
 bool conv_stream_supported(const ConvWeights& w, const convk::ConvParams& p) {
-    return w.rows && w.dtype == SR_DTYPE_BF16 && w.NT == 4 && w.nchunks == 2 && w.Cin == 64 && w.CoutP == w.Cout && p.in_ps == 32 && p.in_cs >= 64 && p.in_cs % 8 == 0 &&
-           p.in_coff % 8 == 0 && p.H % S_TH == 0 && p.W % S_TW == 0 && p.skip_lds == 0 && !p.f2w && !p.pjw && !p.plout && !p.dbg && p.cell_h == 0 && p.cell_w == 0 &&
+    const bool in_ok = p.in_ps == 32 ? (p.in_cs >= 64 && p.in_cs % 8 == 0 && p.in_coff % 8 == 0) : (p.in_cs == 32 && p.in_coff % 32 == 0 && p.in_ps % 8 == 0);
+    const bool pj_ok = !p.pjw || (p.Cd == 64 && p.out_ps == 32 && !p.out_f32 && !p.s2 && !p.clip && p.pj_nblk >= 1 && p.pj_nblk <= 3);
+    return w.rows && w.dtype == SR_DTYPE_BF16 && w.NT == 4 && w.nchunks == 2 && w.Cin == 64 && w.CoutP == w.Cout && in_ok && pj_ok &&
+           p.H % S_TH == 0 && p.W % S_TW == 0 && p.skip_lds == 0 && !p.f2w && !p.plout && !p.dbg && p.cell_h == 0 && p.cell_w == 0 &&
            p.vec != 0 && (p.Cout & 3) == 0 && p.act != SR_ACT_TANH && (p.r <= 1 || (p.Cd & 15) == 0) && !p.s2;
 }
 
@@ -186,7 +197,8 @@
     const int64_t ntiles = (int64_t)p0.B * sp.tilesX * sp.tilesY;
     if (ntiles >= (1ll << 30)) return ctx->fail(SR_ERR_INVALID, "conv_stream: too many tiles for one launch");
     sp.ntiles = (int)ntiles;
-    const int ncu = ctx->cu_count();
+    int ncu = ctx->cu_count();
+    if (ctx->chain_max_wgs > 0 && ctx->chain_max_wgs < ncu) ncu = ctx->chain_max_wgs;
     const int groups = (int)std::max<int64_t>(1, std::min<int64_t>(ntiles, ncu / sp.nct > 0 ? ncu / sp.nct : 1));
     sp.tiles_per_wg = (int)((ntiles + groups - 1) / groups);
     const int ngroups = (int)((ntiles + sp.tiles_per_wg - 1) / sp.tiles_per_wg);
diff --git a/super-resolution-images-for-3d-printing-defect-detection_amd/sr355/_lib.py b/super-resolution-images-for-3d-printing-defect-detection_amd/sr355/_lib.py
--- a/super-resolution-images-for-3d-printing-defect-detection_amd/sr355/_lib.py
+++ b/super-resolution-images-for-3d-printing-defect-detection_amd/sr355/_lib.py
@@ -58,6 +58,7 @@
     "sr_debug_set_chain_stamp_buffer": (_i, [_vp, _vp, _i64]),
     "sr_debug_set_fused": (_i, [_vp, _i, _i]),
     "sr_debug_set_alloc_cap": (_i, [_vp, _i64]),
+    "sr_debug_attn_key_norms": (_i, [_vp, _vp, _i64, _i64p]),
     "sr_debug_conv_routes": (_i, [_vp, _i, C.c_char_p, _i64]),
     "sr_profile_begin": (_i, [_vp]),
     "sr_profile_end": (_i, [_vp, C.c_char_p, _i64]),
diff --git a/super-resolution-images-for-3d-printing-defect-detection_amd/sr355/runtime.py b/super-resolution-images-for-3d-printing-defect-detection_amd/sr355/runtime.py
--- a/super-resolution-images-for-3d-printing-defect-detection_amd/sr355/runtime.py
+++ b/super-resolution-images-for-3d-printing-defect-detection_amd/sr355/runtime.py
@@ -122,6 +122,15 @@
 
     def set_alloc_cap(self, nbytes):
         self.check(self.lib.sr_debug_set_alloc_cap(self.h, int(nbytes)))
+
+    def attn_key_norms(self):
+        n = C.c_int64(0)
+        self.check(self.lib.sr_debug_attn_key_norms(self.h, None, 0, C.byref(n)))
+        if n.value == 0:
+            return None
+        out = torch.empty(n.value, dtype=torch.float32, device=self.torch_device)
+        self.check(self.lib.sr_debug_attn_key_norms(self.h, out.data_ptr(), n.value, C.byref(n)))
+        return out
 
     def conv_routes(self, enable=True):
         buf = C.create_string_buffer(1 << 16)
```

New measurement: 112.9, median of 6. No clear change (+0.4%).
